# Arlo0o/StereoScene

Hardware: AMD Instinct MI355X
Metric: voxels/sec fwd+bwd, 256x256x32 grid D=192 (higher is better)
Workload: dtype f32; 1 GPU; kitti_d192: stereo pair features 2x[B,640,48,160] -> 256x256x32 occupancy, D=192, fwd+bwd incl. 4 losses; batch_per_gpu=1, global_batch=1, parallelism=dp1, train_mode=True

## Files before the change

include/ssbev.h:

```cpp
#ifndef SSBEV_H
#define SSBEV_H

#include <stddef.h>
#include <stdint.h>

#ifdef __cplusplus
extern "C" {
#endif

#define SSBEV_OK 0
#define SSBEV_EINVAL (-1)
#define SSBEV_EWORKSPACE (-2)
#define SSBEV_ELAUNCH (-3)

typedef void* ssbev_stream_t;

int ssbev_version(void);
const char* ssbev_build_arch(void);
void ssbev_env_refresh(void);

typedef struct {
  int B;
  int P;
  int C;
// ... 132 lines not shown
                         const ssbev_norm2_dims* d, void* ws, size_t ws_bytes, ssbev_stream_t stream);

typedef struct { float* running_mean_a; float* running_var_a; float momentum_a;
                 float* running_mean_b; float* running_var_b; float momentum_b; } ssbev_norm2_ext;
int ssbev_groupnorm2_fwd_ext(const float* xa, const float* gamma_a, const float* beta_a, float* mean_a, float* rstd_a,
                             const float* xb, const float* gamma_b, const float* beta_b, float* mean_b, float* rstd_b, float* y,
                             uint64_t* relu_mask, const ssbev_norm2_dims* d, const ssbev_norm2_ext* ext, void* ws, size_t ws_bytes,
                             ssbev_stream_t stream);
int ssbev_groupnorm2_bwd_ext(const float* gy, const uint64_t* relu_mask, const float* xa, const float* gamma_a, const float* mean_a,
                             const float* rstd_a, const float* xb, const float* gamma_b, const float* mean_b, const float* rstd_b,
                             float* gxa, float* gxb, float* ggamma_a, float* gbeta_a, float* ggamma_b, float* gbeta_b,
                             const ssbev_norm2_dims* d, const ssbev_norm2_ext* ext, void* ws, size_t ws_bytes,
                             ssbev_stream_t stream);

typedef struct {
  int vw;
  int slab_q;
  int slabs;
  int chunks;
  int64_t chunk_len;
  int64_t blocks;
  int fixed;
  int chunks_b;
  int64_t chunk_len_b;
  int chunks2;
  int64_t chunk_len2;
} ssbev_groupnorm_plan;
int ssbev_groupnorm_plan_query(const ssbev_norm_dims* d, const ssbev_norm2_dims* d2, int aligned16, ssbev_groupnorm_plan* out);

typedef struct { int B, D, H, W, C; } ssbev_upsample_dims;
int ssbev_trilinear2x_fwd(const float* x, float* y, const ssbev_upsample_dims* d, ssbev_stream_t stream);
int ssbev_trilinear2x_bwd(const float* gy, float* gx, const ssbev_upsample_dims* d, ssbev_stream_t stream);

typedef struct { float lr, beta1, beta2, eps, weight_decay, max_grad_norm; int step; } ssbev_adamw_cfg;
size_t ssbev_grad_norm_workspace(void);
int ssbev_grad_norm(const float* g, int64_t n, float* norm_out, void* ws, size_t ws_bytes,
                    ssbev_stream_t stream);
int ssbev_adamw_step(float* p, const float* g, float* m, float* v, int64_t n,
                     const ssbev_adamw_cfg* c, const float* grad_norm, ssbev_stream_t stream);

typedef struct { int B, D, H, W, C; } ssbev_occloss_dims;
int ssbev_occ_loss_num_sums(void);
size_t ssbev_occ_loss_workspace(const ssbev_occloss_dims* d);
int ssbev_occ_loss_fwd(const float* logits, const uint8_t* label, const float* class_weight, double* sums,
                       const ssbev_occloss_dims* d, void* ws, size_t ws_bytes, ssbev_stream_t stream);
int ssbev_bri_shell_chunks(void);
int ssbev_bri_shell_pre_fwd(const float* q, const float* kv, const float* conf, const float* wq, const float* bq,
                            const float* wk, const float* bk, const float* wv, const float* bv, float* Q, float* K, float* Vc,
                            int B, int D, int T, ssbev_stream_t stream);
int ssbev_bri_shell_post_fwd(const float* out, const float* kv, const float* gamma, float* y, int B, int D, int T,
                             ssbev_stream_t stream);
int ssbev_bri_shell_post_bwd(const float* gy, const float* out, const float* gamma, float* gout, float* delta_part, double* part,
                             int B, int D, int T, ssbev_stream_t stream);
int ssbev_bri_shell_pre_bwd(const float* gQ, const float* gK, const float* gVc, const float* q, const float* kv, const float* conf,
                            const float* gres, const float* wq, const float* wk, const float* wv, const float* bv, float* gq,
                            float* gkv, float* gconf_part, double* part, int B, int D, int T, ssbev_stream_t stream);

int ssbev_occ_loss_tail(const double* sums, float w_ce, float w_sem, float w_geo, float* out5, double* jac,
                        ssbev_stream_t stream);
size_t ssbev_occ_loss_bwd_workspace(const ssbev_occloss_dims* d);
int ssbev_occ_loss_bwd(const float* logits, const uint8_t* label, const float* class_weight,
                       const float* coef, float* grad_logits, const ssbev_occloss_dims* d, void* ws,
                       size_t ws_bytes, ssbev_stream_t stream);

size_t ssbev_occ_predict_workspace(const ssbev_upsample_dims* d);
int ssbev_occ_predict(const float* logits, const uint8_t* label, const uint16_t* remap, uint8_t* pred, uint16_t* raw,
                      int64_t* conf, int64_t* n_ignored, const ssbev_upsample_dims* d, void* ws, size_t ws_bytes,
                      ssbev_stream_t stream);

typedef struct { int B, D, H, W, C, ignore, upsample; } ssbev_lovasz_dims;
int ssbev_lovasz_num_counts(void);
size_t ssbev_lovasz_workspace(const ssbev_lovasz_dims* d);
int ssbev_lovasz_fwd(const float* logits, const uint8_t* label, float* loss, float* dj, int32_t* counts,
                     const ssbev_lovasz_dims* d, void* ws, size_t ws_bytes, ssbev_stream_t stream);
size_t ssbev_lovasz_bwd_workspace(const ssbev_lovasz_dims* d);
int ssbev_lovasz_bwd(const float* logits, const uint8_t* label, const float* dj, const int32_t* counts,
                     const float* grad_out, float* grad_logits, const ssbev_lovasz_dims* d, void* ws, size_t ws_bytes,
                     ssbev_stream_t stream);

typedef struct { int B, D, H, W, C, ignore, upsample; double top_k; } ssbev_ohem_dims;
size_t ssbev_ohem_ce_workspace(const ssbev_ohem_dims* d);
int ssbev_ohem_ce_fwd(const float* logits, const uint8_t* label, const float* class_weight, float* loss, uint8_t* mask,
                      float* inv_wsum, const ssbev_ohem_dims* d, void* ws, size_t ws_bytes, ssbev_stream_t stream);
size_t ssbev_ohem_ce_bwd_workspace(const ssbev_ohem_dims* d);
int ssbev_ohem_ce_bwd(const float* logits, const uint8_t* label, const float* class_weight, const uint8_t* mask,
                      const float* inv_wsum, const float* grad_out, float* grad_logits, const ssbev_ohem_dims* d, void* ws,
                      size_t ws_bytes, ssbev_stream_t stream);

int ssbev_bn_update_running(const float* mean, const float* rstd, float* running_mean, float* running_var, int C,
                            float momentum, float eps, int64_t n, ssbev_stream_t stream);

int ssbev_softmax_axis_fwd(const float* x, float* y, int64_t outer, int C, int64_t inner, ssbev_stream_t stream);
int ssbev_softmax_axis_bwd(const float* y, const float* gy, float* gx, int64_t outer, int C, int64_t inner,
                           ssbev_stream_t stream);
int ssbev_softmax_rows_fwd(const float* x, float* y, int64_t rows, int C, ssbev_stream_t stream);
int ssbev_softmax_rows_bwd(const float* y, const float* gy, float* gx, int64_t rows, int C, ssbev_stream_t stream);

typedef struct { int B, C, H, W, G, k, pad, dil; } ssbev_dcn_dims;
int ssbev_dcn_im2col(const float* x, const float* offset, float* cols, const ssbev_dcn_dims* d, ssbev_stream_t stream);
size_t ssbev_dcn_col2im_workspace(const ssbev_dcn_dims* d);
int ssbev_dcn_col2im(const float* x, const float* offset, const float* gcols, float* gx, float* goffset,
                     const ssbev_dcn_dims* d, void* ws, size_t ws_bytes, ssbev_stream_t stream);

int ssbev_resize_pil_u8(const uint8_t* src, int Hs, int Ws, int C, const int32_t* kk_h, const int32_t* bounds_h, int ksize_h,
                        const int32_t* kk_v, const int32_t* bounds_v, int ksize_v, uint8_t* tmp, uint8_t* dst, int Hd, int Wd,
                        ssbev_stream_t stream);
int ssbev_crop_normalize_u8(const uint8_t* src, int Hs, int Ws, float* dst, int x0, int y0, int w, int h, int flip,
                            const float* mean, const float* stdinv, int swap_rb, ssbev_stream_t stream);
int ssbev_crop_rotate_normalize_u8(const uint8_t* src, int Hs, int Ws, float* dst, int x0, int y0, int w, int h, int flip,
                                   const int32_t* affine6, const float* mean, const float* stdinv, int swap_rb,
                                   ssbev_stream_t stream);
#define SSBEV_JITTER_BRIGHTNESS 1
#define SSBEV_JITTER_CONTRAST 2
#define SSBEV_JITTER_SATURATION 4
#define SSBEV_JITTER_HUE 8
#define SSBEV_JITTER_SWAP 16
typedef struct { int flags, mode; float delta, alpha, saturation, hue; int perm[3]; } ssbev_jitter_params;
int ssbev_crop_rotate_jitter_normalize_u8(const uint8_t* src, int Hs, int Ws, float* dst, int x0, int y0, int w, int h, int flip,
                                          const int32_t* affine6, const ssbev_jitter_params* jitter, const float* mean,
                                          const float* stdinv, int swap_rb, ssbev_stream_t stream);
size_t ssbev_depth_bce_workspace(int BN, int fH, int fW);
int ssbev_depth_bce_fwd(const float* gt_depths, const float* depth_pred, float* out2, int BN, int D, int fH, int fW, int ds,
                        float c0, float dd, float weight, void* ws, size_t ws_bytes, ssbev_stream_t stream);
int ssbev_depth_bce_bwd(const float* depth_pred, const float* grad_loss, const float* out2, float* grad_pred, int BN, int D, int fH,
                        int fW, int ds, float c0, float dd, float weight, const void* ws, ssbev_stream_t stream);

size_t ssbev_depth_kld_workspace(int BN, int fH, int fW);
int ssbev_depth_kld_fwd(const float* gt_depths, const float* depth_pred, float* out2, int BN, int D, int fH, int fW, int ds,
                        double d0, double d1, double dd, float sigma, float edge_scale, float weight, void* ws, size_t ws_bytes,
                        ssbev_stream_t stream);
int ssbev_depth_kld_bwd(const float* depth_pred, const float* grad_loss, const float* out2, float* grad_pred, int BN, int D, int fH,
                        int fW, int ds, double d0, double d1, double dd, float sigma, float edge_scale, float weight, const void* ws,
                        size_t ws_bytes, ssbev_stream_t stream);

size_t ssbev_lidar_depth_workspace(int H, int W);
int ssbev_lidar_depth_map(const float* points, int n_points, const float* cam, const float* labels, float* uvd,
                          unsigned char* valid, float* depth, float* seg, int H, int W, void* ws, size_t ws_bytes,
                          ssbev_stream_t stream);

typedef struct { int B, C, Hi, Wi, Ho, Wo, k, stride, pad_t, pad_l; } ssbev_dw_dims;
int ssbev_dwconv2d_fwd(const float* x, const float* w, float* y, const ssbev_dw_dims* d, ssbev_stream_t stream);
int ssbev_dwconv2d_bwd_data(const float* gy, const float* w, float* gx, const ssbev_dw_dims* d, ssbev_stream_t stream);
size_t ssbev_dwconv2d_bwd_weight_workspace(const ssbev_dw_dims* d);
int ssbev_dwconv2d_bwd_weight(const float* x, const float* gy, float* gw, const ssbev_dw_dims* d, float* ws,
                              size_t ws_elems, ssbev_stream_t stream);
int ssbev_swish_fwd(const float* x, float* y, int64_t n, ssbev_stream_t stream);
int ssbev_swish_bwd(const float* x, const float* gy, float* gx, int64_t n, ssbev_stream_t stream);
size_t ssbev_chan_sum_workspace(int B, int64_t S, int C);
int ssbev_chan_sum(const float* a, const float* bmul, float* out, int B, int64_t S, int C, float scale, float* ws,
                   size_t ws_elems, ssbev_stream_t stream);
int ssbev_chan_scale(const float* x, const float* gate, float* y, int B, int64_t S, int C, float scale,
                     ssbev_stream_t stream);

typedef struct { int B, D, H, W, C; } ssbev_wino_dims;
int ssbev_wino_input_transform(const float* x, float* V, const ssbev_wino_dims* d, ssbev_stream_t stream);
int ssbev_wino_output_transform(const float* M, float* y, const ssbev_wino_dims* d, ssbev_stream_t stream);
int ssbev_wino_output_adjoint(const float* gy, float* Z, const ssbev_wino_dims* d, ssbev_stream_t stream);
int ssbev_wino2d_input_transform(const float* x, float* V, const ssbev_wino_dims* d, ssbev_stream_t stream);
int ssbev_wino2d_output_transform(const float* M, float* y, const ssbev_wino_dims* d, ssbev_stream_t stream);
int ssbev_wino2d_output_adjoint(const float* gy, float* Z, const ssbev_wino_dims* d, ssbev_stream_t stream);
int ssbev_wino_input_transform_bf16(const float* x, uint16_t* V, const ssbev_wino_dims* d, ssbev_stream_t stream);
int ssbev_wino_output_transform_bf16(const uint16_t* M, float* y, const ssbev_wino_dims* d, ssbev_stream_t stream);
int ssbev_wino_output_adjoint_bf16(const float* gy, uint16_t* Z, const ssbev_wino_dims* d, ssbev_stream_t stream);
int ssbev_wino2d_input_transform_bf16(const float* x, uint16_t* V, const ssbev_wino_dims* d, ssbev_stream_t stream);
int ssbev_wino2d_output_transform_bf16(const uint16_t* M, float* y, const ssbev_wino_dims* d, ssbev_stream_t stream);
int ssbev_wino2d_output_adjoint_bf16(const float* gy, uint16_t* Z, const ssbev_wino_dims* d, ssbev_stream_t stream);
int ssbev_wino_input_transform_bf16a(const uint16_t* x, uint16_t* V, const ssbev_wino_dims* d, ssbev_stream_t stream);
int ssbev_wino_output_transform_bf16a(const uint16_t* M, uint16_t* y, const ssbev_wino_dims* d, ssbev_stream_t stream);
int ssbev_wino_output_adjoint_bf16a(const uint16_t* gy, uint16_t* Z, const ssbev_wino_dims* d, ssbev_stream_t stream);
int ssbev_wino2d_input_transform_bf16a(const uint16_t* x, uint16_t* V, const ssbev_wino_dims* d, ssbev_stream_t stream);
int ssbev_wino2d_output_transform_bf16a(const uint16_t* M, uint16_t* y, const ssbev_wino_dims* d, ssbev_stream_t stream);
int ssbev_wino2d_output_adjoint_bf16a(const uint16_t* gy, uint16_t* Z, const ssbev_wino_dims* d, ssbev_stream_t stream);
int ssbev_wino43_input_transform(const float* x, float* V, const ssbev_wino_dims* d, ssbev_stream_t stream);
int ssbev_wino43_output_transform(const float* M, float* y, const ssbev_wino_dims* d, ssbev_stream_t stream);
int ssbev_wino43_output_adjoint(const float* gy, float* Z, const ssbev_wino_dims* d, ssbev_stream_t stream);
int ssbev_wino43_2d_input_transform(const float* x, float* V, const ssbev_wino_dims* d, ssbev_stream_t stream);
int ssbev_wino43_2d_output_transform(const float* M, float* y, const ssbev_wino_dims* d, ssbev_stream_t stream);
int ssbev_wino43_2d_output_transform_acc(const float* M, float* y, const ssbev_wino_dims* d, ssbev_stream_t stream);
int ssbev_wino2d_output_transform_acc(const float* M, float* y, const ssbev_wino_dims* d, ssbev_stream_t stream);
int ssbev_wino43_2d_output_adjoint(const float* gy, float* Z, const ssbev_wino_dims* d, ssbev_stream_t stream);
int ssbev_wino43_input_transform_bf16(const float* x, uint16_t* V, const ssbev_wino_dims* d, ssbev_stream_t stream);
int ssbev_wino43_output_transform_bf16(const uint16_t* M, float* y, const ssbev_wino_dims* d, ssbev_stream_t stream);
int ssbev_wino43_output_adjoint_bf16(const float* gy, uint16_t* Z, const ssbev_wino_dims* d, ssbev_stream_t stream);
int ssbev_wino43_2d_input_transform_bf16(const float* x, uint16_t* V, const ssbev_wino_dims* d, ssbev_stream_t stream);
int ssbev_wino43_2d_output_transform_bf16(const uint16_t* M, float* y, const ssbev_wino_dims* d, ssbev_stream_t stream);
int ssbev_wino43_2d_output_adjoint_bf16(const float* gy, uint16_t* Z, const ssbev_wino_dims* d, ssbev_stream_t stream);
int ssbev_wino444_input_transform(const float* x, float* V, const ssbev_wino_dims* d, ssbev_stream_t stream);
int ssbev_wino444_output_transform(const float* M, float* y, const ssbev_wino_dims* d, ssbev_stream_t stream);
int ssbev_wino444_output_adjoint(const float* gy, float* Z, const ssbev_wino_dims* d, ssbev_stream_t stream);
int ssbev_wino43_weight_transform(const float* w, float* U, int Cout, int Cin, int ndim, int mode, ssbev_stream_t stream);
int ssbev_wino43_weight_grad(const float* gU, float* gw, int Cout, int Cin, int ndim, ssbev_stream_t stream);
int ssbev_wino_weight_transform(const float* w, float* U, int Cout, int Cin, int ndim, int mode, ssbev_stream_t stream);
int ssbev_wino_weight_grad(const float* gU, float* gw, int Cout, int Cin, int ndim, ssbev_stream_t stream);
size_t ssbev_wino_dgemm_packed_elems(int Cout, int Cin);
int ssbev_wino_dgemm_pack(const float* w, float* Wp, int Cout, int Cin, int mode, ssbev_stream_t stream);
int ssbev_wino_dgemm(const float* P, const float* Wp, float* Mo, const ssbev_wino_dims* d, int N, ssbev_stream_t stream);
int ssbev_wino_bgemm(const float* A, const float* Wp, float* Cm, int64_t T, int K, int N, ssbev_stream_t stream);

typedef struct {
  int M, N, K, batch;
  int64_t lda, ldb, ldc, sa, sb, sc;
  int relu;
  int d2s_D, d2s_H, d2s_W, d2s_kd, d2s_kh, d2s_kw, d2s_Co;
  const int64_t* d2s_rowoff;
  const float* ep_mul;
  const float* ep_rowsub;
} ssbev_gemm_dims;
int ssbev_gemm_d2s_rowoff(int64_t* rowoff, int M, int D, int H, int W, int kd, int kh, int kw, int Co, ssbev_stream_t stream);
size_t ssbev_gemm_nn_workspace(const ssbev_gemm_dims* d);
size_t ssbev_gemm_nt_workspace(const ssbev_gemm_dims* d);
int ssbev_gemm_nn(const float* A, const float* B, const float* bias, float* C, const ssbev_gemm_dims* d, void* workspace,
                  size_t ws_bytes, ssbev_stream_t stream);
int ssbev_gemm_nt(const float* A, const float* W, const float* bias, float* C, const ssbev_gemm_dims* d, void* workspace,
                  size_t ws_bytes, ssbev_stream_t stream);
size_t ssbev_gemm_tn_workspace(const ssbev_gemm_dims* d);
int ssbev_gemm_tn(const float* A, const float* B, float* C, const ssbev_gemm_dims* d, void* workspace, size_t ws_bytes,
                  ssbev_stream_t stream);
typedef struct {
  int kernel;
  int bm, bn, bk;
  int nchunk;
  int per_chunk;
  int64_t grid;
  size_t workspace;
} ssbev_gemm_plan;
int ssbev_gemm_plan_query(const ssbev_gemm_dims* d, int form, ssbev_gemm_plan* out);

int ssbev_wino43_df_supported(const ssbev_wino_dims* d, int N);
int ssbev_wino43_df_instance(const ssbev_wino_dims* d, int N);
size_t ssbev_wino43_df_packed_elems(int Cout, int Cin);
int ssbev_wino43_df_pack(const float* w, float* Wp, int Cout, int Cin, int mode, ssbev_stream_t stream);
int ssbev_wino43_df_gemm(const float* P, const float* Wp, float* Mo, const ssbev_wino_dims* d, int N, ssbev_stream_t stream);
size_t ssbev_wino43_df_wgrad_workspace(const ssbev_wino_dims* d, int N);
int ssbev_wino43_df_wgrad(const float* P, const float* Z, float* gw, const ssbev_wino_dims* d, int N, void* workspace,
                          size_t ws_bytes, ssbev_stream_t stream);
typedef struct {
  int mt, nw;
  int ncolgrp, nrowgrp;
  int nst;
  int64_t grid;
  size_t lds_bytes;
  int w_kw, w_nt, w_br;
  int w_nkb, w_nnb;
  int w_nchunk;
  int w_stages_per_chunk;
  int w_total_stages;
  int64_t w_grid;
  size_t w_lds_bytes;
  size_t w_workspace;
} ssbev_wino43_df_plan;
int ssbev_wino43_df_plan_query(const ssbev_wino_dims* d, int N, ssbev_wino43_df_plan* out);

#ifdef __cplusplus
}
#endif
#endif
```

stereoscene_amd/capi.py:

```python
import ctypes as C
import os

import torch

_HERE = os.path.dirname(os.path.abspath(__file__))
LIB_PATH = os.path.join(_HERE, "_lib", "libssbev_hip.so")

OK, EINVAL, EWORKSPACE, ELAUNCH = 0, -1, -2, -3
_ERR = {EINVAL: "SSBEV_EINVAL (bad dims / null pointer / unsupported configuration)",
        EWORKSPACE: "SSBEV_EWORKSPACE (workspace too small)",
        ELAUNCH: "SSBEV_ELAUNCH (HIP launch failure)"}


class SsbevError(RuntimeError):
    pass


class PoolDims(C.Structure):
    _fields_ = [("B", C.c_int), ("P", C.c_int), ("C", C.c_int), ("nx", C.c_int), ("ny", C.c_int), ("nz", C.c_int),
                ("origin", C.c_float * 3), ("dx", C.c_float * 3)]


class LiftDims(C.Structure):
    _fields_ = [("N", C.c_int), ("D", C.c_int), ("HW", C.c_int)]


class GwcDims(C.Structure):
    _fields_ = [("B", C.c_int), ("C", C.c_int), ("G", C.c_int), ("D", C.c_int), ("H", C.c_int), ("W", C.c_int),
                ("down", C.c_float), ("align_corners", C.c_int)]


class ConvDims(C.Structure):
    _fields_ = [(n, C.c_int) for n in (
        "B", "Cin", "Cout", "Di", "Hi", "Wi", "Do", "Ho", "Wo", "kd", "kh", "kw", "sd", "sh", "sw",
        "pd", "ph", "pw", "dd", "dh", "dw", "transposed", "relu", "accumulate", "tile_hint", "precision")]


class GeomDims(C.Structure):
    _fields_ = [(n, C.c_int) for n in ("B", "N", "D", "H", "W")]


class NormDims(C.Structure):
    _fields_ = [("B", C.c_int), ("C", C.c_int), ("G", C.c_int), ("S", C.c_int64), ("eps", C.c_float),
                ("relu", C.c_int), ("stats_given", C.c_int), ("pre_act", C.c_int), ("ld_y", C.c_int64), ("ld_gy", C.c_int64),
                ("io_dtype", C.c_int)]


class Norm2Dims(C.Structure):
    _fields_ = [("B", C.c_int), ("C", C.c_int), ("Ga", C.c_int), ("Gb", C.c_int), ("S", C.c_int64), ("eps_a", C.c_float),
                ("eps_b", C.c_float), ("relu", C.c_int), ("a_batch", C.c_int), ("b_batch", C.c_int), ("io_dtype", C.c_int)]


class Gemm16Dims(C.Structure):
    _fields_ = [("M", C.c_int), ("N", C.c_int), ("K", C.c_int), ("batch", C.c_int), ("out_fp32", C.c_int)]


class NormExt(C.Structure):
    _fields_ = [("running_mean", C.c_void_p), ("running_var", C.c_void_p), ("momentum", C.c_float),
                ("n", C.c_int64)]


class Norm2Ext(C.Structure):
    _fields_ = [("running_mean_a", C.c_void_p), ("running_var_a", C.c_void_p), ("momentum_a", C.c_float),
                ("running_mean_b", C.c_void_p), ("running_var_b", C.c_void_p), ("momentum_b", C.c_float)]


class DcnDims(C.Structure):
    _fields_ = [(n, C.c_int) for n in ("B", "C", "H", "W", "G", "k", "pad", "dil")]


class DwDims(C.Structure):
    _fields_ = [(n, C.c_int) for n in ("B", "C", "Hi", "Wi", "Ho", "Wo", "k", "stride", "pad_t", "pad_l")]


class WinoDims(C.Structure):
    _fields_ = [(n, C.c_int) for n in ("B", "D", "H", "W", "C")]


class UpsampleDims(C.Structure):
    _fields_ = [("B", C.c_int), ("D", C.c_int), ("H", C.c_int), ("W", C.c_int), ("C", C.c_int)]


class LovaszDims(C.Structure):
    _fields_ = [(n, C.c_int) for n in ("B", "D", "H", "W", "C", "ignore", "upsample")]


class OhemDims(C.Structure):
    _fields_ = LovaszDims._fields_ + [("top_k", C.c_double)]


class GemmDims(C.Structure):
    _fields_ = [("M", C.c_int), ("N", C.c_int), ("K", C.c_int), ("batch", C.c_int),
                ("lda", C.c_int64), ("ldb", C.c_int64), ("ldc", C.c_int64), ("sa", C.c_int64), ("sb", C.c_int64), ("sc", C.c_int64),
                ("relu", C.c_int),
                ("d2s_D", C.c_int), ("d2s_H", C.c_int), ("d2s_W", C.c_int), ("d2s_kd", C.c_int), ("d2s_kh", C.c_int),
                ("d2s_kw", C.c_int), ("d2s_Co", C.c_int), ("d2s_rowoff", C.c_void_p),
                ("ep_mul", C.c_void_p), ("ep_rowsub", C.c_void_p)]


class GroupnormPlan(C.Structure):
    _fields_ = [("vw", C.c_int), ("slab_q", C.c_int), ("slabs", C.c_int), ("chunks", C.c_int), ("chunk_len", C.c_int64),
                ("blocks", C.c_int64), ("fixed", C.c_int), ("chunks_b", C.c_int), ("chunk_len_b", C.c_int64), ("chunks2", C.c_int),
                ("chunk_len2", C.c_int64)]


class GemmPlan(C.Structure):
    _fields_ = [("kernel", C.c_int), ("bm", C.c_int), ("bn", C.c_int), ("bk", C.c_int), ("nchunk", C.c_int), ("per_chunk", C.c_int),
                ("grid", C.c_int64), ("workspace", C.c_size_t)]


class Wino43DfPlan(C.Structure):
    _fields_ = [("mt", C.c_int), ("nw", C.c_int), ("ncolgrp", C.c_int), ("nrowgrp", C.c_int), ("nst", C.c_int), ("grid", C.c_int64),
                ("lds_bytes", C.c_size_t), ("w_kw", C.c_int), ("w_nt", C.c_int), ("w_br", C.c_int), ("w_nkb", C.c_int),
                ("w_nnb", C.c_int), ("w_nchunk", C.c_int), ("w_stages_per_chunk", C.c_int), ("w_total_stages", C.c_int),
                ("w_grid", C.c_int64), ("w_lds_bytes", C.c_size_t), ("w_workspace", C.c_size_t)]


class JitterParams(C.Structure):
    _fields_ = [("flags", C.c_int), ("mode", C.c_int), ("delta", C.c_float), ("alpha", C.c_float), ("saturation", C.c_float),
                ("hue", C.c_float), ("perm", C.c_int * 3)]


JITTER_BRIGHTNESS, JITTER_CONTRAST, JITTER_SATURATION, JITTER_HUE, JITTER_SWAP = 1, 2, 4, 8, 16


class AdamWCfg(C.Structure):
    _fields_ = [("lr", C.c_float), ("beta1", C.c_float), ("beta2", C.c_float), ("eps", C.c_float),
                ("weight_decay", C.c_float), ("max_grad_norm", C.c_float), ("step", C.c_int)]


_P = C.c_void_p
SIGNATURES = {
    "ssbev_version": (C.c_int, []),
    "ssbev_build_arch": (C.c_char_p, []),
    "ssbev_env_refresh": (None, []),
    "ssbev_voxel_index": (C.c_int, [_P, _P, _P, C.POINTER(PoolDims), _P]),
    "ssbev_coords_to_vox": (C.c_int, [_P, C.c_int, _P, C.POINTER(PoolDims), _P]),
    "ssbev_pool_prepare_workspace": (C.c_size_t, [C.c_int, C.POINTER(PoolDims)]),
    "ssbev_pool_prepare": (C.c_int, [_P, C.c_int, _P, _P, C.POINTER(PoolDims), _P, C.c_size_t, _P]),
    "ssbev_pool_long_list_elems": (C.c_size_t, [C.c_int]),
    "ssbev_pool_prepare2": (C.c_int, [_P, C.c_int, _P, _P, _P, C.POINTER(PoolDims), _P, C.c_size_t, _P]),
    "ssbev_bev_pool_fwd": (C.c_int, [_P, _P, _P, _P, C.POINTER(PoolDims), _P]),
    "ssbev_bev_pool_bwd": (C.c_int, [_P, _P, C.c_int, _P, C.POINTER(PoolDims), _P]),
    "ssbev_lift_splat_fwd": (C.c_int, [_P, _P, _P, _P, _P, C.POINTER(PoolDims), C.POINTER(LiftDims), _P]),
    "ssbev_lift_splat_fwd2": (C.c_int, [_P, _P, _P, _P, _P, _P, C.POINTER(PoolDims), C.POINTER(LiftDims), _P]),
    "ssbev_lift_splat_bwd": (C.c_int, [_P, _P, _P, _P, _P, _P, C.POINTER(PoolDims), C.POINTER(LiftDims), _P]),
    "ssbev_gwc_warp_fwd": (C.c_int, [_P, _P, _P, _P, C.POINTER(GwcDims), _P]),
    "ssbev_gwc_warp_bwd": (C.c_int, [_P, _P, _P, _P, _P, _P, C.POINTER(GwcDims), _P]),
    "ssbev_gwc_warp_bwd_workspace": (C.c_size_t, [C.POINTER(GwcDims)]),
    "ssbev_gwc_warp_bwd_fused": (C.c_int, [_P, _P, _P, _P, _P, _P, C.POINTER(GwcDims), _P, C.c_size_t, _P]),
    "ssbev_conv_packed_weight_elems": (C.c_size_t, [C.POINTER(ConvDims)]),
    "ssbev_conv_kernel_class": (C.c_int, [C.POINTER(ConvDims), C.c_int]),
    "ssbev_conv_chunk_groups": (C.c_int, [C.POINTER(ConvDims), C.c_int]),
    "ssbev_frustum_geometry": (C.c_int, [_P] * 9 + [C.POINTER(GeomDims), _P]),
    "ssbev_conv_pack_weight": (C.c_int, [_P, _P, C.POINTER(ConvDims), C.c_int, _P]),
    "ssbev_conv_thin_workspace": (C.c_size_t, [C.POINTER(ConvDims), C.c_int]),
    "ssbev_conv_thin_packed_elems": (C.c_size_t, [C.POINTER(ConvDims), C.c_int]),
    "ssbev_conv_thin_pack": (C.c_int, [_P, _P, C.POINTER(ConvDims), C.c_int, _P]),
    "ssbev_conv_thin_run": (C.c_int, [_P, _P, _P, _P, C.POINTER(ConvDims), C.c_int, _P, C.c_size_t, _P]),
    "ssbev_conv_fwd": (C.c_int, [_P, _P, _P, _P, C.POINTER(ConvDims), _P]),
    "ssbev_conv_bwd_data": (C.c_int, [_P, _P, _P, C.POINTER(ConvDims), _P]),
    "ssbev_conv_fwd_bf16": (C.c_int, [_P, _P, _P, _P, C.POINTER(ConvDims), _P]),
    "ssbev_conv_bwd_data_bf16": (C.c_int, [_P, _P, _P, C.POINTER(ConvDims), _P]),
    "ssbev_conv_bwd_weight_bf16": (C.c_int, [_P, _P, _P, C.POINTER(ConvDims), _P, C.c_size_t, _P]),
    "ssbev_conv_bwd_weight_workspace": (C.c_size_t, [C.POINTER(ConvDims)]),
    "ssbev_conv_bwd_weight": (C.c_int, [_P, _P, _P, C.POINTER(ConvDims), _P, C.c_size_t, _P]),
    "ssbev_gemm16_packed_elems": (C.c_size_t, [C.POINTER(Gemm16Dims)]),
    "ssbev_gemm16_pack": (C.c_int, [_P, _P, C.POINTER(Gemm16Dims), _P]),
    "ssbev_gemm16_nn": (C.c_int, [_P, _P, _P, C.POINTER(Gemm16Dims), _P]),
    "ssbev_gemm16_tn_workspace": (C.c_size_t, [C.POINTER(Gemm16Dims)]),
    "ssbev_gemm16_tn": (C.c_int, [_P, _P, _P, C.POINTER(Gemm16Dims), _P, C.c_size_t, _P]),
    "ssbev_groupnorm_workspace": (C.c_size_t, [C.POINTER(NormDims)]),
    "ssbev_groupnorm_fwd": (C.c_int, [_P] * 7 + [C.POINTER(NormDims), _P, C.c_size_t, _P]),
    "ssbev_groupnorm_bwd": (C.c_int, [_P] * 10 + [C.POINTER(NormDims), _P, C.c_size_t, _P]),
    "ssbev_groupnorm_mask_words": (C.c_size_t, [C.POINTER(NormDims)]),
    "ssbev_groupnorm_fwd_mask": (C.c_int, [_P] * 8 + [C.POINTER(NormDims), _P, C.c_size_t, _P]),
    "ssbev_groupnorm_bwd_mask": (C.c_int, [_P] * 10 + [C.POINTER(NormDims), _P, C.c_size_t, _P]),
    "ssbev_groupnorm_fwd_ext": (C.c_int, [_P] * 8 + [C.POINTER(NormDims), C.POINTER(NormExt), _P, C.c_size_t, _P]),
    "ssbev_groupnorm_bwd_ext": (C.c_int, [_P] * 11 + [C.POINTER(NormDims), C.POINTER(NormExt), _P, C.c_size_t, _P]),
    "ssbev_groupnorm2_fwd_ext": (C.c_int, [_P] * 12 + [C.POINTER(Norm2Dims), C.POINTER(Norm2Ext), _P, C.c_size_t, _P]),
    "ssbev_groupnorm2_bwd_ext": (C.c_int, [_P] * 16 + [C.POINTER(Norm2Dims), C.POINTER(Norm2Ext), _P, C.c_size_t, _P]),
    "ssbev_groupnorm2_workspace": (C.c_size_t, [C.POINTER(Norm2Dims)]),
    "ssbev_groupnorm2_fwd": (C.c_int, [_P] * 12 + [C.POINTER(Norm2Dims), _P, C.c_size_t, _P]),
    "ssbev_groupnorm2_bwd": (C.c_int, [_P] * 16 + [C.POINTER(Norm2Dims), _P, C.c_size_t, _P]),
    "ssbev_groupnorm_plan_query": (C.c_int, [C.POINTER(NormDims), C.POINTER(Norm2Dims), C.c_int, C.POINTER(GroupnormPlan)]),
    "ssbev_trilinear2x_fwd": (C.c_int, [_P, _P, C.POINTER(UpsampleDims), _P]),
    "ssbev_trilinear2x_bwd": (C.c_int, [_P, _P, C.POINTER(UpsampleDims), _P]),
    "ssbev_dcn_im2col": (C.c_int, [_P, _P, _P, C.POINTER(DcnDims), _P]),
    "ssbev_dcn_col2im_workspace": (C.c_size_t, [C.POINTER(DcnDims)]),
    "ssbev_dcn_col2im": (C.c_int, [_P, _P, _P, _P, _P, C.POINTER(DcnDims), _P, C.c_size_t, _P]),
    "ssbev_bn_update_running": (C.c_int, [_P, _P, _P, _P, C.c_int, C.c_float, C.c_float, C.c_int64, _P]),
    "ssbev_resize_pil_u8": (C.c_int, [_P, C.c_int, C.c_int, C.c_int, _P, _P, C.c_int, _P, _P, C.c_int, _P, _P, C.c_int, C.c_int, _P]),
    "ssbev_crop_normalize_u8": (C.c_int, [_P, C.c_int, C.c_int, _P, C.c_int, C.c_int, C.c_int, C.c_int, C.c_int, _P, _P, C.c_int, _P]),
    "ssbev_crop_rotate_normalize_u8": (C.c_int, [_P, C.c_int, C.c_int, _P, C.c_int, C.c_int, C.c_int, C.c_int, C.c_int, _P, _P, _P,
                                                C.c_int, _P]),
    "ssbev_crop_rotate_jitter_normalize_u8": (C.c_int, [_P, C.c_int, C.c_int, _P, C.c_int, C.c_int, C.c_int, C.c_int, C.c_int, _P,
                                                       C.POINTER(JitterParams), _P, _P, C.c_int, _P]),
    "ssbev_depth_bce_workspace": (C.c_size_t, [C.c_int, C.c_int, C.c_int]),
    "ssbev_depth_bce_fwd": (C.c_int, [_P, _P, _P] + [C.c_int] * 5 + [C.c_float] * 3 + [_P, C.c_size_t, _P]),
    "ssbev_depth_bce_bwd": (C.c_int, [_P, _P, _P, _P] + [C.c_int] * 5 + [C.c_float] * 3 + [_P, _P]),
    "ssbev_depth_kld_workspace": (C.c_size_t, [C.c_int, C.c_int, C.c_int]),
    "ssbev_depth_kld_fwd": (C.c_int, [_P, _P, _P] + [C.c_int] * 5 + [C.c_double] * 3 + [C.c_float] * 3 + [_P, C.c_size_t, _P]),
    "ssbev_depth_kld_bwd": (C.c_int, [_P, _P, _P, _P] + [C.c_int] * 5 + [C.c_double] * 3 + [C.c_float] * 3 + [_P, C.c_size_t, _P]),
    "ssbev_lidar_depth_workspace": (C.c_size_t, [C.c_int, C.c_int]),
    "ssbev_lidar_depth_map": (C.c_int, [_P, C.c_int, _P, _P, _P, _P, _P, _P, C.c_int, C.c_int, _P, C.c_size_t, _P]),
    "ssbev_dwconv2d_fwd": (C.c_int, [_P, _P, _P, C.POINTER(DwDims), _P]),
    "ssbev_dwconv2d_bwd_data": (C.c_int, [_P, _P, _P, C.POINTER(DwDims), _P]),
    "ssbev_dwconv2d_bwd_weight_workspace": (C.c_size_t, [C.POINTER(DwDims)]),
    "ssbev_dwconv2d_bwd_weight": (C.c_int, [_P, _P, _P, C.POINTER(DwDims), _P, C.c_size_t, _P]),
    "ssbev_swish_fwd": (C.c_int, [_P, _P, C.c_int64, _P]),
    "ssbev_swish_bwd": (C.c_int, [_P, _P, _P, C.c_int64, _P]),
    "ssbev_chan_sum_workspace": (C.c_size_t, [C.c_int, C.c_int64, C.c_int]),
    "ssbev_chan_sum": (C.c_int, [_P, _P, _P, C.c_int, C.c_int64, C.c_int, C.c_float, _P, C.c_size_t, _P]),
    "ssbev_chan_scale": (C.c_int, [_P, _P, _P, C.c_int, C.c_int64, C.c_int, C.c_float, _P]),
    "ssbev_wino_input_transform": (C.c_int, [_P, _P, C.POINTER(WinoDims), _P]),
    "ssbev_wino_output_transform": (C.c_int, [_P, _P, C.POINTER(WinoDims), _P]),
    "ssbev_wino_output_adjoint": (C.c_int, [_P, _P, C.POINTER(WinoDims), _P]),
    "ssbev_wino_weight_transform": (C.c_int, [_P, _P, C.c_int, C.c_int, C.c_int, C.c_int, _P]),
    "ssbev_wino_weight_grad": (C.c_int, [_P, _P, C.c_int, C.c_int, C.c_int, _P]),
    "ssbev_wino_dgemm_packed_elems": (C.c_size_t, [C.c_int, C.c_int]),
    "ssbev_wino_dgemm_pack": (C.c_int, [_P, _P, C.c_int, C.c_int, C.c_int, _P]),
    "ssbev_wino_dgemm": (C.c_int, [_P, _P, _P, C.POINTER(WinoDims), C.c_int, _P]),
    "ssbev_wino_bgemm": (C.c_int, [_P, _P, _P, C.c_int64, C.c_int, C.c_int, _P]),
    "ssbev_gemm_d2s_rowoff": (C.c_int, [_P, C.c_int, C.c_int, C.c_int, C.c_int, C.c_int, C.c_int, C.c_int, C.c_int, _P]),
    "ssbev_gemm_nn_workspace": (C.c_size_t, [C.POINTER(GemmDims)]),
    "ssbev_gemm_nt_workspace": (C.c_size_t, [C.POINTER(GemmDims)]),
    "ssbev_gemm_nn": (C.c_int, [_P, _P, _P, _P, C.POINTER(GemmDims), _P, C.c_size_t, _P]),
    "ssbev_gemm_nt": (C.c_int, [_P, _P, _P, _P, C.POINTER(GemmDims), _P, C.c_size_t, _P]),
    "ssbev_gemm_tn_workspace": (C.c_size_t, [C.POINTER(GemmDims)]),
    "ssbev_gemm_tn": (C.c_int, [_P, _P, _P, C.POINTER(GemmDims), _P, C.c_size_t, _P]),
    "ssbev_gemm_plan_query": (C.c_int, [C.POINTER(GemmDims), C.c_int, C.POINTER(GemmPlan)]),
    "ssbev_wino43_df_supported": (C.c_int, [C.POINTER(WinoDims), C.c_int]),
    "ssbev_wino43_df_instance": (C.c_int, [C.POINTER(WinoDims), C.c_int]),
    "ssbev_wino43_df_packed_elems": (C.c_size_t, [C.c_int, C.c_int]),
    "ssbev_wino43_df_pack": (C.c_int, [_P, _P, C.c_int, C.c_int, C.c_int, _P]),
    "ssbev_wino43_df_gemm": (C.c_int, [_P, _P, _P, C.POINTER(WinoDims), C.c_int, _P]),
    "ssbev_wino43_df_wgrad_workspace": (C.c_size_t, [C.POINTER(WinoDims), C.c_int]),
    "ssbev_wino43_df_wgrad": (C.c_int, [_P, _P, _P, C.POINTER(WinoDims), C.c_int, _P, C.c_size_t, _P]),
    "ssbev_wino43_df_plan_query": (C.c_int, [C.POINTER(WinoDims), C.c_int, C.POINTER(Wino43DfPlan)]),
    "ssbev_wino2d_input_transform": (C.c_int, [_P, _P, C.POINTER(WinoDims), _P]),
    "ssbev_wino2d_output_transform": (C.c_int, [_P, _P, C.POINTER(WinoDims), _P]),
    "ssbev_wino2d_output_adjoint": (C.c_int, [_P, _P, C.POINTER(WinoDims), _P]),
    "ssbev_wino43_input_transform": (C.c_int, [_P, _P, C.POINTER(WinoDims), _P]),
    "ssbev_wino43_input_transform_bf16": (C.c_int, [_P, _P, C.POINTER(WinoDims), _P]),
    "ssbev_wino43_output_transform": (C.c_int, [_P, _P, C.POINTER(WinoDims), _P]),
    "ssbev_wino43_output_transform_bf16": (C.c_int, [_P, _P, C.POINTER(WinoDims), _P]),
    "ssbev_wino43_output_adjoint": (C.c_int, [_P, _P, C.POINTER(WinoDims), _P]),
    "ssbev_wino43_output_adjoint_bf16": (C.c_int, [_P, _P, C.POINTER(WinoDims), _P]),
    "ssbev_wino43_2d_input_transform": (C.c_int, [_P, _P, C.POINTER(WinoDims), _P]),
    "ssbev_wino43_2d_input_transform_bf16": (C.c_int, [_P, _P, C.POINTER(WinoDims), _P]),
    "ssbev_wino43_2d_output_transform": (C.c_int, [_P, _P, C.POINTER(WinoDims), _P]),
    "ssbev_wino43_2d_output_transform_acc": (C.c_int, [_P, _P, C.POINTER(WinoDims), _P]),
    "ssbev_wino2d_output_transform_acc": (C.c_int, [_P, _P, C.POINTER(WinoDims), _P]),
    "ssbev_wino43_2d_output_transform_bf16": (C.c_int, [_P, _P, C.POINTER(WinoDims), _P]),
    "ssbev_wino43_2d_output_adjoint": (C.c_int, [_P, _P, C.POINTER(WinoDims), _P]),
    "ssbev_wino43_2d_output_adjoint_bf16": (C.c_int, [_P, _P, C.POINTER(WinoDims), _P]),
    "ssbev_wino444_input_transform": (C.c_int, [_P, _P, C.POINTER(WinoDims), _P]),
    "ssbev_wino444_output_transform": (C.c_int, [_P, _P, C.POINTER(WinoDims), _P]),
    "ssbev_wino444_output_adjoint": (C.c_int, [_P, _P, C.POINTER(WinoDims), _P]),
    "ssbev_wino43_weight_transform": (C.c_int, [_P, _P, C.c_int, C.c_int, C.c_int, C.c_int, _P]),
    "ssbev_wino43_weight_grad": (C.c_int, [_P, _P, C.c_int, C.c_int, C.c_int, _P]),
    "ssbev_wino_input_transform_bf16": (C.c_int, [_P, _P, C.POINTER(WinoDims), _P]),
    "ssbev_wino_output_transform_bf16": (C.c_int, [_P, _P, C.POINTER(WinoDims), _P]),
    "ssbev_wino_output_adjoint_bf16": (C.c_int, [_P, _P, C.POINTER(WinoDims), _P]),
    "ssbev_wino2d_input_transform_bf16": (C.c_int, [_P, _P, C.POINTER(WinoDims), _P]),
    "ssbev_wino2d_output_transform_bf16": (C.c_int, [_P, _P, C.POINTER(WinoDims), _P]),
    "ssbev_wino2d_output_adjoint_bf16": (C.c_int, [_P, _P, C.POINTER(WinoDims), _P]),
    "ssbev_wino_input_transform_bf16a": (C.c_int, [_P, _P, C.POINTER(WinoDims), _P]),
    "ssbev_wino_output_transform_bf16a": (C.c_int, [_P, _P, C.POINTER(WinoDims), _P]),
    "ssbev_wino_output_adjoint_bf16a": (C.c_int, [_P, _P, C.POINTER(WinoDims), _P]),
    "ssbev_wino2d_input_transform_bf16a": (C.c_int, [_P, _P, C.POINTER(WinoDims), _P]),
    "ssbev_wino2d_output_transform_bf16a": (C.c_int, [_P, _P, C.POINTER(WinoDims), _P]),
    "ssbev_wino2d_output_adjoint_bf16a": (C.c_int, [_P, _P, C.POINTER(WinoDims), _P]),
    "ssbev_softmax_axis_fwd": (C.c_int, [_P, _P, C.c_int64, C.c_int, C.c_int64, _P]),
    "ssbev_softmax_axis_bwd": (C.c_int, [_P, _P, _P, C.c_int64, C.c_int, C.c_int64, _P]),
    "ssbev_softmax_rows_fwd": (C.c_int, [_P, _P, C.c_int64, C.c_int, _P]),
    "ssbev_softmax_rows_bwd": (C.c_int, [_P, _P, _P, C.c_int64, C.c_int, _P]),
    "ssbev_occ_loss_num_sums": (C.c_int, []),
    "ssbev_occ_loss_workspace": (C.c_size_t, [C.POINTER(UpsampleDims)]),
    "ssbev_occ_loss_fwd": (C.c_int, [_P, _P, _P, _P, C.POINTER(UpsampleDims), _P, C.c_size_t, _P]),
    "ssbev_occ_loss_tail": (C.c_int, [_P, C.c_float, C.c_float, C.c_float, _P, _P, _P]),
    "ssbev_bri_shell_chunks": (C.c_int, []),
    "ssbev_bri_shell_pre_fwd": (C.c_int, [_P] * 12 + [C.c_int] * 3 + [_P]),
    "ssbev_bri_shell_post_fwd": (C.c_int, [_P] * 4 + [C.c_int] * 3 + [_P]),
    "ssbev_bri_shell_post_bwd": (C.c_int, [_P] * 6 + [C.c_int] * 3 + [_P]),
    "ssbev_bri_shell_pre_bwd": (C.c_int, [_P] * 15 + [C.c_int] * 3 + [_P]),
    "ssbev_occ_loss_bwd_workspace": (C.c_size_t, [C.POINTER(UpsampleDims)]),
    "ssbev_occ_loss_bwd": (C.c_int, [_P, _P, _P, _P, _P, C.POINTER(UpsampleDims), _P, C.c_size_t, _P]),
    "ssbev_occ_predict_workspace": (C.c_size_t, [C.POINTER(UpsampleDims)]),
    "ssbev_occ_predict": (C.c_int, [_P] * 7 + [C.POINTER(UpsampleDims), _P, C.c_size_t, _P]),
    "ssbev_lovasz_num_counts": (C.c_int, []),
    "ssbev_lovasz_workspace": (C.c_size_t, [C.POINTER(LovaszDims)]),
    "ssbev_lovasz_fwd": (C.c_int, [_P] * 5 + [C.POINTER(LovaszDims), _P, C.c_size_t, _P]),
    "ssbev_lovasz_bwd_workspace": (C.c_size_t, [C.POINTER(LovaszDims)]),
    "ssbev_lovasz_bwd": (C.c_int, [_P] * 6 + [C.POINTER(LovaszDims), _P, C.c_size_t, _P]),
    "ssbev_ohem_ce_workspace": (C.c_size_t, [C.POINTER(OhemDims)]),
    "ssbev_ohem_ce_fwd": (C.c_int, [_P] * 6 + [C.POINTER(OhemDims), _P, C.c_size_t, _P]),
    "ssbev_ohem_ce_bwd_workspace": (C.c_size_t, [C.POINTER(OhemDims)]),
    "ssbev_ohem_ce_bwd": (C.c_int, [_P] * 7 + [C.POINTER(OhemDims), _P, C.c_size_t, _P]),
    "ssbev_grad_norm_workspace": (C.c_size_t, []),
    "ssbev_grad_norm": (C.c_int, [_P, C.c_int64, _P, _P, C.c_size_t, _P]),
    "ssbev_adamw_step": (C.c_int, [_P, _P, _P, _P, C.c_int64, C.POINTER(AdamWCfg), _P, _P]),
}

_lib = None


def load():
    global _lib
    if _lib is None:
        if not os.path.exists(LIB_PATH):
            raise SsbevError(f"{LIB_PATH} is missing: run `python -m stereoscene_amd.build` "
                             "(there is no CPU / PyTorch fallback for the HIP operators)")
        lib = C.CDLL(LIB_PATH)
        for name, (res, args) in SIGNATURES.items():
            fn = getattr(lib, name)
            fn.restype, fn.argtypes = res, args
        _lib = lib
    return _lib


def check(code, what):
    if code != OK:
        raise SsbevError(f"{what}: {_ERR.get(code, code)}")


def ptr(t):
    if t is None:
        return None
    if not t.is_cuda:
        raise SsbevError("ssbev operators run on the MI355X only: got a CPU tensor (no CPU fallback exists)")
    if not t.is_contiguous():
        raise SsbevError("ssbev operators need contiguous buffers")
    return C.c_void_p(t.data_ptr())


_raw_stream = getattr(torch._C, "_cuda_getCurrentRawStream", None)


def stream():
    if _raw_stream is not None:
        return C.c_void_p(_raw_stream(torch.cuda.current_device()))
    return C.c_void_p(torch.cuda.current_stream().cuda_stream)
```

stereoscene_amd/csrc/capi.hip:

```cpp
#include "common.h"

#include <cstdlib>
#include <mutex>
#include <string>
#include <unordered_map>

namespace {
struct EnvTable {
  std::mutex mu;
  std::unordered_map<std::string, std::pair<bool, std::string>> seen;
};
EnvTable& env_table() {
  static EnvTable* t = new EnvTable();
  return *t;
}
}

const char* ssbev_env(const char* name) {
  EnvTable& t = env_table();
  std::lock_guard<std::mutex> lock(t.mu);
  auto it = t.seen.find(name);
  if (it == t.seen.end()) {
    const char* v = std::getenv(name);
    it = t.seen.emplace(name, std::make_pair(v != nullptr, std::string(v ? v : ""))).first;
  }
  return it->second.first ? it->second.second.c_str() : nullptr;
}

extern "C" {
int ssbev_version(void) { return 110;  }
const char* ssbev_build_arch(void) { return "gfx950"; }

void ssbev_env_refresh(void) {
  EnvTable& t = env_table();
  std::lock_guard<std::mutex> lock(t.mu);
  t.seen.clear();
}
}
```

stereoscene_amd/csrc/winograd.hip:

```cpp
#include "common.h"

#include <algorithm>
#include <cstdlib>

namespace {

struct WinoGeom { int B, D, H, W, C; int acc = 0; };
__device__ const float kWinoZeros[4] = {0.f, 0.f, 0.f, 0.f};

typedef unsigned short bf16_bits;
__device__ __forceinline__ float fload(const float* p) { return *p; }
__device__ __forceinline__ float fload(const bf16_bits* p) { return __uint_as_float((unsigned)*p << 16); }
__device__ __forceinline__ void fstore(float* p, float v) { *p = v; }
__device__ __forceinline__ void fstore(bf16_bits* p, float v) { *p = __builtin_bit_cast(bf16_bits, (__bf16)v); }

__device__ __forceinline__ void bt4(float* v, int s) {
  const float d0 = v[0], d1 = v[s], d2 = v[2 * s], d3 = v[3 * s];
  v[0] = d0 - d2; v[s] = d1 + d2; v[2 * s] = d2 - d1; v[3 * s] = d1 - d3;
}
__device__ __forceinline__ void a4(float* v, int s) {
  const float g0 = v[0], g1 = v[s];
  v[0] = g0; v[s] = g0 + g1; v[2 * s] = g0 - g1; v[3 * s] = -g1;
}

template <int NV, typename T>
__device__ __forceinline__ void ldv(const T* p, float (&o)[NV]) {
  if constexpr (NV == 1) {
    o[0] = ld1(p);
  } else if constexpr (sizeof(T) == 2) {
    const unsigned u = *reinterpret_cast<const unsigned*>(p);
    o[0] = __uint_as_float(u << 16); o[1] = __uint_as_float(u & 0xffff0000u);
  } else {
    const float2 f = *reinterpret_cast<const float2*>(p);
    o[0] = f.x; o[1] = f.y;
  }
}
template <int NV, typename T>
__device__ __forceinline__ void stv(T* p, const float (&v)[NV]) {
  if constexpr (NV == 1) {
    st1(p, v[0]);
  } else if constexpr (sizeof(T) == 2) {
    *reinterpret_cast<unsigned*>(p) = pack_bf2(v[0], v[1]);
  } else {
    *reinterpret_cast<float2*>(p) = make_float2(v[0], v[1]);
  }
}

template <int NV>
__device__ __forceinline__ void wino_decode3(long i, const WinoGeom& g, int& c, long& tile, int& tw, int& th, int& td, int& b) {
  const int cq = g.C / NV;
  c = NV * (int)(i % cq);
  long t = i / cq;
  tile = t;
  tw = (int)(t % (g.W / 2)); t /= g.W / 2;
  th = (int)(t % (g.H / 2)); t /= g.H / 2;
  td = (int)(t % (g.D / 2));
  b = (int)(t / (g.D / 2));
}
template <int NV>
__device__ __forceinline__ void wino_decode2(long i, const WinoGeom& g, int& c, long& tile, int& tw, int& th, long& bd) {
  const int cq = g.C / NV;
  c = NV * (int)(i % cq);
  long t = i / cq;
  tile = t;
  tw = (int)(t % (g.W / 2)); t /= g.W / 2;
  th = (int)(t % (g.H / 2));
  bd = t / (g.H / 2);
}

template <typename TF, typename TA = float, int NV = 1>
__global__ void __launch_bounds__(256)
wino_input_kernel(const TA* __restrict__ x, TF* __restrict__ V, WinoGeom g, long total) {
  const long i = (long)blockIdx.x * 256 + threadIdx.x;
  if (i >= total) return;
  int c, tw, th, td, b;
  long tile;
  wino_decode3<NV>(i, g, c, tile, tw, th, td, b);
  float v[NV][64];
#pragma unroll
  for (int a = 0; a < 4; ++a) {
    const int d = 2 * td - 1 + a;
#pragma unroll
    for (int e = 0; e < 4; ++e) {
      const int h = 2 * th - 1 + e;
#pragma unroll
      for (int f = 0; f < 4; ++f) {
        const int w = 2 * tw - 1 + f;
        const bool ok = d >= 0 && d < g.D && h >= 0 && h < g.H && w >= 0 && w < g.W;
        float t[NV];
#pragma unroll
        for (int n = 0; n < NV; ++n) t[n] = 0.0f;
        if (ok) ldv<NV>(x + ((((long)b * g.D + d) * g.H + h) * g.W + w) * g.C + c, t);
#pragma unroll
        for (int n = 0; n < NV; ++n) v[n][(a * 4 + e) * 4 + f] = t[n];
      }
    }
  }
#pragma unroll
  for (int n = 0; n < NV; ++n) {
#pragma unroll
    for (int p = 0; p < 16; ++p) bt4(v[n] + p * 4, 1);
#pragma unroll
    for (int a = 0; a < 4; ++a)
#pragma unroll
      for (int f = 0; f < 4; ++f) bt4(v[n] + a * 16 + f, 4);
#pragma unroll
    for (int p = 0; p < 16; ++p) bt4(v[n] + p, 16);
  }
  const long T = total / (g.C / NV);
#pragma unroll
  for (int xi = 0; xi < 64; ++xi) {
    float t[NV];
#pragma unroll
    for (int n = 0; n < NV; ++n) t[n] = v[n][xi];
    stv<NV>(V + ((long)xi * T + tile) * g.C + c, t);
  }
}

template <typename TF, typename TA = float, int NV = 1>
__global__ void __launch_bounds__(256)
wino_output_kernel(const TF* __restrict__ M, TA* __restrict__ y, WinoGeom g, long total) {
  const long i = (long)blockIdx.x * 256 + threadIdx.x;
  if (i >= total) return;
  int c, tw, th, td, b;
  long tile;
  wino_decode3<NV>(i, g, c, tile, tw, th, td, b);
  const long T = total / (g.C / NV);
  float m[NV][64];
#pragma unroll
  for (int xi = 0; xi < 64; ++xi) {
    float t[NV];
    ldv<NV>(M + ((long)xi * T + tile) * g.C + c, t);
#pragma unroll
    for (int n = 0; n < NV; ++n) m[n][xi] = t[n];
  }
  float out[NV][8];
#pragma unroll
  for (int n = 0; n < NV; ++n) {
    float r1[32];
#pragma unroll
    for (int p = 0; p < 16; ++p) {
      r1[p * 2 + 0] = m[n][p * 4] + m[n][p * 4 + 1] + m[n][p * 4 + 2];
      r1[p * 2 + 1] = m[n][p * 4 + 1] - m[n][p * 4 + 2] - m[n][p * 4 + 3];
    }
    float r2[16];
#pragma unroll
    for (int a = 0; a < 4; ++a)
#pragma unroll
      for (int f = 0; f < 2; ++f) {
        const float m0 = r1[(a * 4 + 0) * 2 + f], m1 = r1[(a * 4 + 1) * 2 + f], m2 = r1[(a * 4 + 2) * 2 + f],
                    m3 = r1[(a * 4 + 3) * 2 + f];
        r2[(a * 2 + 0) * 2 + f] = m0 + m1 + m2;
        r2[(a * 2 + 1) * 2 + f] = m1 - m2 - m3;
      }
#pragma unroll
    for (int e = 0; e < 2; ++e)
#pragma unroll
      for (int f = 0; f < 2; ++f) {
        const float m0 = r2[(0 * 2 + e) * 2 + f], m1 = r2[(1 * 2 + e) * 2 + f], m2 = r2[(2 * 2 + e) * 2 + f],
                    m3 = r2[(3 * 2 + e) * 2 + f];
        out[n][(0 * 2 + e) * 2 + f] = m0 + m1 + m2;
        out[n][(1 * 2 + e) * 2 + f] = m1 - m2 - m3;
      }
  }
#pragma unroll
  for (int dz = 0; dz < 2; ++dz)
#pragma unroll
    for (int e = 0; e < 2; ++e)
#pragma unroll
      for (int f = 0; f < 2; ++f) {
        float t[NV];
#pragma unroll
        for (int n = 0; n < NV; ++n) t[n] = out[n][(dz * 2 + e) * 2 + f];
        stv<NV>(y + ((((long)b * g.D + 2 * td + dz) * g.H + 2 * th + e) * g.W + 2 * tw + f) * g.C + c, t);
      }
}

template <typename TF, typename TA = float, int NV = 1>
__global__ void __launch_bounds__(256)
wino_output_adjoint_kernel(const TA* __restrict__ gy, TF* __restrict__ Z, WinoGeom g, long total) {
  const long i = (long)blockIdx.x * 256 + threadIdx.x;
  if (i >= total) return;
  int c, tw, th, td, b;
  long tile;
  wino_decode3<NV>(i, g, c, tile, tw, th, td, b);
  float v[NV][64];
#pragma unroll
  for (int a = 0; a < 2; ++a)
#pragma unroll
    for (int e = 0; e < 2; ++e)
#pragma unroll
      for (int f = 0; f < 2; ++f) {
        float t[NV];
        ldv<NV>(gy + ((((long)b * g.D + 2 * td + a) * g.H + 2 * th + e) * g.W + 2 * tw + f) * g.C + c, t);
#pragma unroll
        for (int n = 0; n < NV; ++n) v[n][(a * 4 + e) * 4 + f] = t[n];
      }
#pragma unroll
  for (int n = 0; n < NV; ++n) {
#pragma unroll
    for (int a = 0; a < 2; ++a)
#pragma unroll
      for (int e = 0; e < 2; ++e) a4(v[n] + (a * 4 + e) * 4, 1);
#pragma unroll
    for (int a = 0; a < 2; ++a)
#pragma unroll
      for (int f = 0; f < 4; ++f) a4(v[n] + a * 16 + f, 4);
#pragma unroll
    for (int p = 0; p < 16; ++p) a4(v[n] + p, 16);
  }
  const long T = total / (g.C / NV);
#pragma unroll
  for (int xi = 0; xi < 64; ++xi) {
    float t[NV];
#pragma unroll
    for (int n = 0; n < NV; ++n) t[n] = v[n][xi];
    stv<NV>(Z + ((long)xi * T + tile) * g.C + c, t);
  }
}

template <typename TF, typename TA = float, int NV = 1>
__global__ void __launch_bounds__(256)
wino2d_input_kernel(const TA* __restrict__ x, TF* __restrict__ V, WinoGeom g, long total) {
  const long i = (long)blockIdx.x * 256 + threadIdx.x;
  if (i >= total) return;
  int c, tw, th;
  long tile, bd;
  wino_decode2<NV>(i, g, c, tile, tw, th, bd);
  float v[NV][16];
#pragma unroll
  for (int e = 0; e < 4; ++e) {
    const int h = 2 * th - 1 + e;
#pragma unroll
    for (int f = 0; f < 4; ++f) {
      const int w = 2 * tw - 1 + f;
      const bool ok = h >= 0 && h < g.H && w >= 0 && w < g.W;
      float t[NV];
#pragma unroll
      for (int n = 0; n < NV; ++n) t[n] = 0.0f;
      if (ok) ldv<NV>(x + ((bd * g.H + h) * g.W + w) * g.C + c, t);
#pragma unroll
      for (int n = 0; n < NV; ++n) v[n][e * 4 + f] = t[n];
    }
  }
#pragma unroll
  for (int n = 0; n < NV; ++n) {
#pragma unroll
    for (int e = 0; e < 4; ++e) bt4(v[n] + e * 4, 1);
#pragma unroll
    for (int f = 0; f < 4; ++f) bt4(v[n] + f, 4);
  }
  const long T = total / (g.C / NV);
#pragma unroll
  for (int xi = 0; xi < 16; ++xi) {
    float t[NV];
#pragma unroll
    for (int n = 0; n < NV; ++n) t[n] = v[n][xi];
    stv<NV>(V + ((long)xi * T + tile) * g.C + c, t);
  }
}

template <typename TF, typename TA = float, int NV = 1>
__global__ void __launch_bounds__(256)
wino2d_output_kernel(const TF* __restrict__ M, TA* __restrict__ y, WinoGeom g, long total) {
  const long i = (long)blockIdx.x * 256 + threadIdx.x;
  if (i >= total) return;
  int c, tw, th;
  long tile, bd;
  wino_decode2<NV>(i, g, c, tile, tw, th, bd);
  const long T = total / (g.C / NV);
  float m[NV][16];
#pragma unroll
  for (int xi = 0; xi < 16; ++xi) {
    float t[NV];
    ldv<NV>(M + ((long)xi * T + tile) * g.C + c, t);
#pragma unroll
    for (int n = 0; n < NV; ++n) m[n][xi] = t[n];
  }
  float oldv[NV][4];
#pragma unroll
  for (int n = 0; n < NV; ++n)
#pragma unroll
    for (int k = 0; k < 4; ++k) oldv[n][k] = 0.0f;
  if (g.acc) {
#pragma unroll
    for (int f = 0; f < 2; ++f) {
      const long base = ((bd * g.H + 2 * th) * g.W + 2 * tw + f) * g.C + c;
      float t0[NV], t1[NV];
      ldv<NV>(y + base, t0);
      ldv<NV>(y + base + (long)g.W * g.C, t1);
#pragma unroll
      for (int n = 0; n < NV; ++n) { oldv[n][2 * f] = t0[n]; oldv[n][2 * f + 1] = t1[n]; }
    }
  }
#pragma unroll
  for (int f = 0; f < 2; ++f) {
    float y0[NV], y1[NV];
#pragma unroll
    for (int n = 0; n < NV; ++n) {
      float r[8];
#pragma unroll
      for (int e = 0; e < 4; ++e) {
        r[e * 2 + 0] = m[n][e * 4] + m[n][e * 4 + 1] + m[n][e * 4 + 2];
        r[e * 2 + 1] = m[n][e * 4 + 1] - m[n][e * 4 + 2] - m[n][e * 4 + 3];
      }
      y0[n] = r[0 * 2 + f] + r[1 * 2 + f] + r[2 * 2 + f] + oldv[n][2 * f];
      y1[n] = r[1 * 2 + f] - r[2 * 2 + f] - r[3 * 2 + f] + oldv[n][2 * f + 1];
    }
    const long base = ((bd * g.H + 2 * th) * g.W + 2 * tw + f) * g.C + c;
    stv<NV>(y + base, y0);
    stv<NV>(y + base + (long)g.W * g.C, y1);
  }
}

template <typename TF, typename TA = float, int NV = 1>
__global__ void __launch_bounds__(256)
wino2d_output_adjoint_kernel(const TA* __restrict__ gy, TF* __restrict__ Z, WinoGeom g, long total) {
  const long i = (long)blockIdx.x * 256 + threadIdx.x;
  if (i >= total) return;
  int c, tw, th;
  long tile, bd;
  wino_decode2<NV>(i, g, c, tile, tw, th, bd);
  float v[NV][16];
#pragma unroll
  for (int e = 0; e < 2; ++e)
#pragma unroll
    for (int f = 0; f < 2; ++f) {
      float t[NV];
      ldv<NV>(gy + ((bd * g.H + 2 * th + e) * g.W + 2 * tw + f) * g.C + c, t);
#pragma unroll
      for (int n = 0; n < NV; ++n) v[n][e * 4 + f] = t[n];
    }
#pragma unroll
  for (int n = 0; n < NV; ++n) {
#pragma unroll
    for (int e = 0; e < 2; ++e) a4(v[n] + e * 4, 1);
#pragma unroll
    for (int f = 0; f < 4; ++f) a4(v[n] + f, 4);
  }
  const long T = total / (g.C / NV);
#pragma unroll
  for (int xi = 0; xi < 16; ++xi) {
    float t[NV];
#pragma unroll
    for (int n = 0; n < NV; ++n) t[n] = v[n][xi];
    stv<NV>(Z + ((long)xi * T + tile) * g.C + c, t);
  }
}

bool wino2d_ok(const ssbev_wino_dims* d) {
  return d && d->B > 0 && d->C > 0 && d->D > 0 && d->H > 0 && d->W > 0 && d->H % 2 == 0 && d->W % 2 == 0;
}

__device__ __forceinline__ void g4(const float* g, int s, float* o, int so) {
  const float g0 = g[0], g1 = g[s], g2 = g[2 * s];
  o[0] = g0; o[so] = 0.5f * (g0 + g1 + g2); o[2 * so] = 0.5f * (g0 - g1 + g2); o[3 * so] = g2;
}
__device__ __forceinline__ void gt3(const float* u, int s, float* o, int so) {
  const float u0 = u[0], u1 = u[s], u2 = u[2 * s], u3 = u[3 * s];
  o[0] = u0 + 0.5f * (u1 + u2); o[so] = 0.5f * (u1 - u2); o[2 * so] = 0.5f * (u1 + u2) + u3;
}

template <int ND>
__global__ void __launch_bounds__(256)
wino_weight_kernel(const float* __restrict__ w, float* __restrict__ U, int Cout, int Cin, int mode) {
  constexpr int TAPS = ND == 3 ? 27 : 9, NF = ND == 3 ? 64 : 16;
  const int i = blockIdx.x * 256 + threadIdx.x;
  if (i >= Cout * Cin) return;
  const int co = mode == 0 ? i % Cout : i / Cin, ci = mode == 0 ? i / Cout : i % Cin;
  float g[TAPS];
#pragma unroll
  for (int t = 0; t < TAPS; ++t) g[t] = w[((size_t)co * Cin + ci) * TAPS + (mode == 0 ? t : TAPS - 1 - t)];
  float u[NF];
  if (ND == 3) {
    float a[36], b[48];
#pragma unroll
    for (int p = 0; p < 9; ++p) g4(g + p * 3, 1, a + p * 4, 1);
#pragma unroll
    for (int d = 0; d < 3; ++d)
#pragma unroll
      for (int f = 0; f < 4; ++f) g4(a + d * 12 + f, 4, b + d * 16 + f, 4);
#pragma unroll
    for (int p = 0; p < 16; ++p) g4(b + p, 16, u + p, 16);
  } else {
    float a[12];
#pragma unroll
    for (int p = 0; p < 3; ++p) g4(g + p * 3, 1, a + p * 4, 1);
#pragma unroll
    for (int f = 0; f < 4; ++f) g4(a + f, 4, u + f, 4);
  }
  const size_t plane = (size_t)Cout * Cin;
  const size_t pos = mode == 0 ? (size_t)ci * Cout + co : (size_t)co * Cin + ci;
#pragma unroll
  for (int xi = 0; xi < NF; ++xi) U[xi * plane + pos] = u[xi];
}

template <int ND>
__global__ void __launch_bounds__(256)
wino_weight_grad_kernel(const float* __restrict__ gU, float* __restrict__ gw, int Cout, int Cin) {
  constexpr int TAPS = ND == 3 ? 27 : 9, NF = ND == 3 ? 64 : 16;
  const int i = blockIdx.x * 256 + threadIdx.x;
  if (i >= Cout * Cin) return;
  const int co = i % Cout, ci = i / Cout;
  const size_t plane = (size_t)Cout * Cin;
  float u[NF];
#pragma unroll
  for (int xi = 0; xi < NF; ++xi) u[xi] = gU[xi * plane + (size_t)ci * Cout + co];
  float g[TAPS];
  if (ND == 3) {
    float a[48], b[36];
#pragma unroll
    for (int p = 0; p < 16; ++p) gt3(u + p * 4, 1, a + p * 3, 1);
#pragma unroll
    for (int d = 0; d < 4; ++d)
#pragma unroll
      for (int f = 0; f < 3; ++f) gt3(a + d * 12 + f, 3, b + d * 9 + f, 3);
#pragma unroll
    for (int p = 0; p < 9; ++p) gt3(b + p, 9, g + p, 9);
  } else {
    float a[12];
#pragma unroll
    for (int p = 0; p < 4; ++p) gt3(u + p * 4, 1, a + p * 3, 1);
#pragma unroll
    for (int f = 0; f < 3; ++f) gt3(a + f, 3, g + f, 3);
  }
#pragma unroll
  for (int t = 0; t < TAPS; ++t) gw[((size_t)co * Cin + ci) * TAPS + t] = g[t];
}

__device__ __forceinline__ void bt6(float* v, int s) {
  const float d0 = v[0], d1 = v[s], d2 = v[2 * s], d3 = v[3 * s], d4 = v[4 * s], d5 = v[5 * s];
  v[0] = 4.0f * d0 - 5.0f * d2 + d4;
  v[s] = -4.0f * d1 - 4.0f * d2 + d3 + d4;
  v[2 * s] = 4.0f * d1 - 4.0f * d2 - d3 + d4;
  v[3 * s] = -2.0f * d1 - d2 + 2.0f * d3 + d4;
  v[4 * s] = 2.0f * d1 - d2 - 2.0f * d3 + d4;
  v[5 * s] = 4.0f * d1 - 5.0f * d3 + d5;
}
__device__ __forceinline__ void at6(const float* m, int s, float* o, int so) {
  const float m0 = m[0], m1 = m[s], m2 = m[2 * s], m3 = m[3 * s], m4 = m[4 * s], m5 = m[5 * s];
  const float p = m1 + m2, q = m1 - m2, r = m3 + m4, t = m3 - m4;
  o[0] = m0 + p + r;
  o[so] = q + 2.0f * t;
  o[2 * so] = p + 4.0f * r;
  o[3 * so] = q + 8.0f * t + m5;
}
__device__ __forceinline__ void a6(const float* g, int s, float* o, int so) {
  const float g0 = g[0], g1 = g[s], g2 = g[2 * s], g3 = g[3 * s];
  o[0] = g0;
  o[so] = g0 + g1 + g2 + g3;
  o[2 * so] = g0 - g1 + g2 - g3;
  o[3 * so] = g0 + 2.0f * g1 + 4.0f * g2 + 8.0f * g3;
  o[4 * so] = g0 - 2.0f * g1 + 4.0f * g2 - 8.0f * g3;
  o[5 * so] = g3;
}
__device__ __forceinline__ void g6(const float* g, int s, float* o, int so) {
  const float g0 = g[0], g1 = g[s], g2 = g[2 * s];
  o[0] = 0.25f * g0;
  o[so] = -(g0 + g1 + g2) * (1.0f / 6.0f);
  o[2 * so] = -(g0 - g1 + g2) * (1.0f / 6.0f);
  o[3 * so] = g0 * (1.0f / 24.0f) + g1 * (1.0f / 12.0f) + g2 * (1.0f / 6.0f);
  o[4 * so] = g0 * (1.0f / 24.0f) - g1 * (1.0f / 12.0f) + g2 * (1.0f / 6.0f);
  o[5 * so] = g2;
}
__device__ __forceinline__ void gt6(const float* u, int s, float* o, int so) {
  const float u0 = u[0], u1 = u[s], u2 = u[2 * s], u3 = u[3 * s], u4 = u[4 * s], u5 = u[5 * s];
  o[0] = 0.25f * u0 - (u1 + u2) * (1.0f / 6.0f) + (u3 + u4) * (1.0f / 24.0f);
  o[so] = (u2 - u1) * (1.0f / 6.0f) + (u3 - u4) * (1.0f / 12.0f);
  o[2 * so] = -(u1 + u2) * (1.0f / 6.0f) + (u3 + u4) * (1.0f / 6.0f) + u5;
}

template <int DA>
__device__ __forceinline__ void tile43(long t, const WinoGeom& g, int& b_or_bd, int& td, int& th, int& tw) {
  tw = (int)(t % (g.W / 4)); t /= g.W / 4;
  th = (int)(t % (g.H / 4)); t /= g.H / 4;
  if (DA) { td = (int)(t % (g.D / DA)); b_or_bd = (int)(t / (g.D / DA)); }
  else { td = 0; b_or_bd = (int)t; }
}

template <int DA, typename TF>
__global__ void __launch_bounds__(256) __attribute__((amdgpu_waves_per_eu(1, DA == 4 ? 1 : (DA == 2 ? 2 : 8))))
wino43_input_kernel(const float* __restrict__ x, TF* __restrict__ V, WinoGeom g, long total) {
  constexpr int NA = DA ? DA + 2 : 1, NF = NA * 36;
  const long i = (long)blockIdx.x * 256 + threadIdx.x;
  if (i >= total) return;
  const int c = (int)(i % g.C);
  const long tile = i / g.C;
  int b, td, th, tw;
  tile43<DA>(tile, g, b, td, th, tw);
  float v[NF];
#pragma unroll
  for (int a = 0; a < NA; ++a) {
    const int d = DA ? DA * td - 1 + a : 0;
    const long plane = DA ? (long)b * g.D + d : (long)b;
    const bool dok = !DA || (d >= 0 && d < g.D);
#pragma unroll
    for (int e = 0; e < 6; ++e) {
      const int h = 4 * th - 1 + e;
#pragma unroll
      for (int f = 0; f < 6; ++f) {
        const int w = 4 * tw - 1 + f;
        const bool ok = dok && h >= 0 && h < g.H && w >= 0 && w < g.W;
        v[(a * 6 + e) * 6 + f] = ok ? x[((plane * g.H + h) * g.W + w) * g.C + c] : 0.0f;
      }
// ... 34 lines not shown
  float r1[NA * 6 * 4];
#pragma unroll
  for (int p = 0; p < NA * 6; ++p) at6(m + p * 6, 1, r1 + p * 4, 1);
  float r2[NA * 4 * 4];
#pragma unroll
  for (int a = 0; a < NA; ++a)
#pragma unroll
    for (int f = 0; f < 4; ++f) at6(r1 + a * 24 + f, 4, r2 + a * 16 + f, 4);
  if (DA == 0 && g.acc) {
    float oldv[16];
#pragma unroll
    for (int e = 0; e < 4; ++e)
#pragma unroll
      for (int f = 0; f < 4; ++f) oldv[e * 4 + f] = y[(((long)b * g.H + 4 * th + e) * g.W + 4 * tw + f) * g.C + c];
#pragma unroll
    for (int k = 0; k < 16; ++k) r2[k] += oldv[k];
  }
#pragma unroll
  for (int e = 0; e < 4; ++e)
#pragma unroll
    for (int f = 0; f < 4; ++f) {
      if (DA == 2) {
        const float m0 = r2[0 * 16 + e * 4 + f], m1 = r2[1 * 16 + e * 4 + f], m2 = r2[2 * 16 + e * 4 + f], m3 = r2[3 * 16 + e * 4 + f];
        const long base = ((((long)b * g.D + 2 * td) * g.H + 4 * th + e) * g.W + 4 * tw + f) * g.C + c;
        y[base] = m0 + m1 + m2;
        y[base + (long)g.H * g.W * g.C] = m1 - m2 - m3;
      } else if (DA == 4) {
        float o[4];
        at6(r2 + e * 4 + f, 16, o, 1);
        const long base = ((((long)b * g.D + 4 * td) * g.H + 4 * th + e) * g.W + 4 * tw + f) * g.C + c;
#pragma unroll
        for (int a = 0; a < 4; ++a) y[base + (long)a * g.H * g.W * g.C] = o[a];
      } else {
        y[(((long)b * g.H + 4 * th + e) * g.W + 4 * tw + f) * g.C + c] = r2[e * 4 + f];
      }
    }
}

template <int DA, typename TF>
__global__ void __launch_bounds__(256) __attribute__((amdgpu_waves_per_eu(1, DA == 4 ? 1 : (DA == 2 ? 2 : 8))))
wino43_output_adjoint_kernel(const float* __restrict__ gy, TF* __restrict__ Z, WinoGeom g, long total) {
  constexpr int NA = DA ? DA + 2 : 1, NG = DA ? DA : 1, NF = NA * 36;
  const long i = (long)blockIdx.x * 256 + threadIdx.x;
  if (i >= total) return;
  const int c = (int)(i % g.C);
  const long tile = i / g.C;
  int b, td, th, tw;
  tile43<DA>(tile, g, b, td, th, tw);
  float gin[NG * 16];
#pragma unroll
  for (int a = 0; a < NG; ++a) {
    const long plane = DA ? (long)b * g.D + DA * td + a : (long)b;
#pragma unroll
    for (int e = 0; e < 4; ++e)
#pragma unroll
      for (int f = 0; f < 4; ++f) gin[(a * 4 + e) * 4 + f] = gy[((plane * g.H + 4 * th + e) * g.W + 4 * tw + f) * g.C + c];
  }
  float r1[NG * 4 * 6];
#pragma unroll
  for (int p = 0; p < NG * 4; ++p) a6(gin + p * 4, 1, r1 + p * 6, 1);
  float v[NF];
#pragma unroll
  for (int a = 0; a < NG; ++a)
#pragma unroll
    for (int f = 0; f < 6; ++f) a6(r1 + a * 24 + f, 6, v + a * 36 + f, 6);
  if (DA == 2) {
#pragma unroll
    for (int p = 0; p < 36; ++p) a4(v + p, 36);
  } else if (DA == 4) {
#pragma unroll
    for (int p = 0; p < 36; ++p) {
      float t6[6];
      a6(v + p, 36, t6, 1);
#pragma unroll
      for (int a = 0; a < 6; ++a) v[a * 36 + p] = t6[a];
    }
  }
  const long T = total / g.C;
#pragma unroll
  for (int xi = 0; xi < NF; ++xi) fstore(Z + ((long)xi * T + tile) * g.C + c, v[xi]);
}

template <int DA>
__global__ void __launch_bounds__(256)
wino43_weight_kernel(const float* __restrict__ w, float* __restrict__ U, int Cout, int Cin, int mode) {
  constexpr int ND_ = DA ? 3 : 1, TAPS = ND_ * 9, NA = DA ? DA + 2 : 1, NF = NA * 36;
  const int i = blockIdx.x * 256 + threadIdx.x;
  if (i >= Cout * Cin) return;
  const int co = mode == 0 ? i % Cout : i / Cin, ci = mode == 0 ? i / Cout : i % Cin;
  float g[TAPS];
#pragma unroll
  for (int t = 0; t < TAPS; ++t) g[t] = w[((size_t)co * Cin + ci) * TAPS + (mode == 0 ? t : TAPS - 1 - t)];
  float a1[ND_ * 3 * 6];
#pragma unroll
  for (int p = 0; p < ND_ * 3; ++p) g6(g + p * 3, 1, a1 + p * 6, 1);
  float a2[ND_ * 36];
#pragma unroll
  for (int d = 0; d < ND_; ++d)
#pragma unroll
    for (int f = 0; f < 6; ++f) g6(a1 + d * 18 + f, 6, a2 + d * 36 + f, 6);
  float u[NF];
  if (DA == 2) {
#pragma unroll
    for (int p = 0; p < 36; ++p) g4(a2 + p, 36, u + p, 36);
  } else if (DA == 4) {
#pragma unroll
    for (int p = 0; p < 36; ++p) g6(a2 + p, 36, u + p, 36);
  } else {
#pragma unroll
    for (int p = 0; p < 36; ++p) u[p] = a2[p];
  }
  const size_t plane = (size_t)Cout * Cin;
  const size_t pos = mode == 0 ? (size_t)ci * Cout + co : (size_t)co * Cin + ci;
#pragma unroll
  for (int xi = 0; xi < NF; ++xi) U[xi * plane + pos] = u[xi];
}

template <int DA>
__global__ void __launch_bounds__(256)
wino43_weight_grad_kernel(const float* __restrict__ gU, float* __restrict__ gw, int Cout, int Cin) {
  constexpr int ND_ = DA ? 3 : 1, TAPS = ND_ * 9, NA = DA ? DA + 2 : 1, NF = NA * 36;
  const int i = blockIdx.x * 256 + threadIdx.x;
  if (i >= Cout * Cin) return;
  const int co = i % Cout, ci = i / Cout;
  const size_t plane = (size_t)Cout * Cin;
  float u[NF];
#pragma unroll
  for (int xi = 0; xi < NF; ++xi) u[xi] = gU[xi * plane + (size_t)ci * Cout + co];
  float a1[NA * 6 * 3];
#pragma unroll
  for (int p = 0; p < NA * 6; ++p) gt6(u + p * 6, 1, a1 + p * 3, 1);
  float a2[NA * 9];
#pragma unroll
  for (int a = 0; a < NA; ++a)
#pragma unroll
    for (int f = 0; f < 3; ++f) gt6(a1 + a * 18 + f, 3, a2 + a * 9 + f, 3);
  float g[TAPS];
  if (DA == 2) {
#pragma unroll
    for (int p = 0; p < 9; ++p) gt3(a2 + p, 9, g + p, 9);
  } else if (DA == 4) {
#pragma unroll
    for (int p = 0; p < 9; ++p) gt6(a2 + p, 9, g + p, 9);
  } else {
#pragma unroll
    for (int p = 0; p < 9; ++p) g[p] = a2[p];
  }
#pragma unroll
  for (int t = 0; t < TAPS; ++t) gw[((size_t)co * Cin + ci) * TAPS + t] = g[t];
}

bool wino43_ok(const ssbev_wino_dims* d, int da) {
  return d && d->B > 0 && d->C > 0 && d->D > 0 && d->H > 0 && d->W > 0 && d->H % 4 == 0 && d->W % 4 == 0 &&
         (da == 0 || d->D % da == 0);
}

typedef float wf32x16 __attribute__((ext_vector_type(16)));

struct WinoGemmGeom { int B, D, Thw, Cin, Cout, CoutPad; };

template <int MT, int NT>
__global__ void __launch_bounds__(256)
wino_dgemm_kernel(const float* __restrict__ P, const float* __restrict__ Wp, float* __restrict__ Mo, WinoGemmGeom g) {
  const int lane = threadIdx.x & 63, wave = threadIdx.x >> 6;
  const int li = lane & 31, lk = lane >> 5;
  const int tgroups = (g.Thw + 32 * MT - 1) / (32 * MT), tg4 = ((tgroups + 3) >> 2) << 2;
  const int tg = (blockIdx.x * 4 + wave) % tg4;
  const int bi = (blockIdx.x * 4 + wave) / tg4;
  if (tg >= tgroups) return;
  const int i = bi % (g.D / 2), b = bi / (g.D / 2);
  const int xhw = blockIdx.z, n0 = blockIdx.y * (NT * 32);
  const long R = (long)g.B * g.D * g.Thw;
  const float* pa[4][MT];
#pragma unroll
  for (int mt = 0; mt < MT; ++mt) {
    const int tq = (tg * MT + mt) * 32 + li;
#pragma unroll
    for (int a = 0; a < 4; ++a) {
      const int d = 2 * i - 1 + a;
      pa[a][mt] = (tq < g.Thw && d >= 0 && d < g.D)
                      ? P + ((long)xhw * R + ((long)b * g.D + d) * g.Thw + tq) * g.Cin + 4 * lk : nullptr;
    }
  }
  wf32x16 acc[4][MT][NT];
#pragma unroll
  for (int f = 0; f < 4; ++f)
#pragma unroll
    for (int mt = 0; mt < MT; ++mt)
#pragma unroll
      for (int nt = 0; nt < NT; ++nt)
#pragma unroll
        for (int r = 0; r < 16; ++r) acc[f][mt][nt][r] = 0.0f;
  const int Q = (g.Cin + 7) >> 3;
  const size_t fstride = (size_t)Q * 2 * g.CoutPad * 4;
  const float* wl = Wp + ((size_t)lk * g.CoutPad + n0 + li) * 4 + (size_t)xhw * fstride;
  for (int q = 0; q < Q; ++q) {
    const bool cok = (8 * q + 4 * lk) < g.Cin;
    float4 v[4][MT];
#pragma unroll
    for (int mt = 0; mt < MT; ++mt) {
      float4 p[4];
#pragma unroll
      for (int a = 0; a < 4; ++a)
        p[a] = (pa[a][mt] && cok) ? *reinterpret_cast<const float4*>(pa[a][mt] + 8 * q) : make_float4(0.f, 0.f, 0.f, 0.f);
      v[0][mt] = make_float4(p[0].x - p[2].x, p[0].y - p[2].y, p[0].z - p[2].z, p[0].w - p[2].w);
      v[1][mt] = make_float4(p[1].x + p[2].x, p[1].y + p[2].y, p[1].z + p[2].z, p[1].w + p[2].w);
      v[2][mt] = make_float4(p[2].x - p[1].x, p[2].y - p[1].y, p[2].z - p[1].z, p[2].w - p[1].w);
      v[3][mt] = make_float4(p[1].x - p[3].x, p[1].y - p[3].y, p[1].z - p[3].z, p[1].w - p[3].w);
    }
    float4 wv[4][NT];
#pragma unroll
    for (int f = 0; f < 4; ++f)
#pragma unroll
      for (int nt = 0; nt < NT; ++nt)
        wv[f][nt] = (n0 + nt * 32 < g.CoutPad)
                        ? *reinterpret_cast<const float4*>(wl + (size_t)f * 16 * fstride + ((size_t)q * 2 * g.CoutPad + nt * 32) * 4)
                        : make_float4(0.f, 0.f, 0.f, 0.f);
#define SSBEV_WG_COMP(COMP)                                                                   \
    _Pragma("unroll") for (int f = 0; f < 4; ++f)                                             \
    _Pragma("unroll") for (int mt = 0; mt < MT; ++mt)                                         \
    _Pragma("unroll") for (int nt = 0; nt < NT; ++nt)                                         \
      acc[f][mt][nt] = __builtin_amdgcn_mfma_f32_32x32x2f32(v[f][mt].COMP, wv[f][nt].COMP, acc[f][mt][nt], 0, 0, 0);
    SSBEV_WG_COMP(x) SSBEV_WG_COMP(y) SSBEV_WG_COMP(z) SSBEV_WG_COMP(w)
#undef SSBEV_WG_COMP
  }
#pragma unroll
  for (int mt = 0; mt < MT; ++mt) {
    const int t0 = (tg * MT + mt) * 32;
    float* o0 = Mo + ((long)xhw * R + ((long)b * g.D + 2 * i) * g.Thw + t0) * g.Cout;
    float* o1 = o0 + (long)g.Thw * g.Cout;
#pragma unroll
    for (int nt = 0; nt < NT; ++nt) {
      const int co = n0 + nt * 32 + li;
      if (co >= g.Cout) continue;
#pragma unroll
      for (int r = 0; r < 16; ++r) {
        const int row = (r & 3) + 8 * (r >> 2) + 4 * lk;
        if (t0 + row < g.Thw) {
          const float m0 = acc[0][mt][nt][r], m1 = acc[1][mt][nt][r], m2 = acc[2][mt][nt][r], m3 = acc[3][mt][nt][r];
          o0[(long)row * g.Cout + co] = m0 + m1 + m2;
          o1[(long)row * g.Cout + co] = m1 - m2 - m3;
        }
      }
    }
  }
}

struct WinoBgemmGeom { long T; int K, N, NPad; };

constexpr int kBgBM = 64, kBgBK = 64, kBgStages = 3;

template <int NT>
__global__ void __launch_bounds__(256)
wino_bgemm_kernel(const float* __restrict__ A, const float* __restrict__ Wp, float* __restrict__ Cm, WinoBgemmGeom g) {
  extern __shared__ __align__(16) float al[];
  const int tid = threadIdx.x, lane = tid & 63, wave = tid >> 6;
  const int li = lane & 31, lk = lane >> 5;
  const int xi = blockIdx.z;
  const int n0 = (blockIdx.y * 4 + wave) * (NT * 32);
  const bool col_active = n0 < g.N;
  const float* Ax = A + (long)xi * g.T * g.K;
  float* Cx = Cm + (long)xi * g.T * g.N;
  const int Q = (g.K + 7) >> 3, nstage = (g.K + kBgBK - 1) / kBgBK;
  const size_t fstride = (size_t)Q * 2 * g.NPad * 4;
  const float* wl = Wp + (size_t)xi * fstride + ((size_t)lk * g.NPad + n0 + li) * 4;
  const long nrb = (g.T + kBgBM - 1) / kBgBM;
  const long rb_per = (nrb + gridDim.x - 1) / gridDim.x;
  const long rb_begin = (long)blockIdx.x * rb_per, rb_end = min(nrb, rb_begin + rb_per);
  const long total = (rb_end - rb_begin) * nstage;
  if (total <= 0) return;

  auto issue = [&](long s) {
    const long rb = rb_begin + s / nstage;
    const int k0 = (int)(s % nstage) * kBgBK, buf = (int)(s % kBgStages);
#pragma unroll
    for (int e = 0; e < 4; ++e) {
      const int jbase = (wave + 4 * e) * 64;
      const int j = jbase + lane, row = j >> 4, slot = j & 15;
      const int src_slot = (slot & 8) | ((slot & 7) ^ (row & 7));
      const long r = rb * kBgBM + row;
      const int k = k0 + src_slot * 4;
      const float* src = (r < g.T && k < g.K) ? Ax + r * g.K + k : kWinoZeros;
      __builtin_amdgcn_global_load_lds(src, al + buf * (kBgBM * kBgBK) + jbase * 4, 16, 0, 0);
    }
  };
  wf32x16 acc[2][NT];
  float4 bvA[kBgBK / 8][NT], bvB[kBgBK / 8][NT];
  auto load_b = [&](long s, float4 (&bv)[kBgBK / 8][NT]) {
    const int st = (int)(s % nstage);
#pragma unroll
    for (int qq = 0; qq < kBgBK / 8; ++qq) {
      const int q = st * (kBgBK / 8) + qq;
#pragma unroll
      for (int nt = 0; nt < NT; ++nt)
        bv[qq][nt] = (col_active && q < Q && n0 + nt * 32 < g.NPad)
                         ? *reinterpret_cast<const float4*>(wl + ((size_t)q * 2 * g.NPad + nt * 32) * 4)
                         : make_float4(0.f, 0.f, 0.f, 0.f);
    }
  };
  issue(0);
  load_b(0, bvA);
  if (total > 1) issue(1);
  for (long s = 0; s < total; ++s) {
    const int st = (int)(s % nstage), buf = (int)(s % kBgStages);
    float4 (&bv)[kBgBK / 8][NT] = (s & 1) ? bvB : bvA;
    if (st == 0) {
#pragma unroll
      for (int mt = 0; mt < 2; ++mt)
#pragma unroll
        for (int nt = 0; nt < NT; ++nt)
#pragma unroll
          for (int r = 0; r < 16; ++r) acc[mt][nt][r] = 0.0f;
    }
    if (s + 1 < total) asm volatile("s_waitcnt vmcnt(4)" ::: "memory");
    else asm volatile("s_waitcnt vmcnt(0)" ::: "memory");
    __syncthreads();
    if (s + 1 < total) { if (s & 1) load_b(s + 1, bvA); else load_b(s + 1, bvB); }
    if (s + 2 < total) issue(s + 2);
    if (col_active) {
      const float* ab = al + buf * (kBgBM * kBgBK);
#pragma unroll
      for (int qq = 0; qq < kBgBK / 8; ++qq) {
        float4 av[2];
#pragma unroll
        for (int mt = 0; mt < 2; ++mt) {
          const int row = mt * 32 + li;
          const int slot = 2 * qq + lk;
          av[mt] = *reinterpret_cast<const float4*>(ab + row * kBgBK + (((slot & 8) | ((slot & 7) ^ (row & 7))) << 2));
        }
#define SSBEV_BG_COMP(COMP)                                                                 \
        _Pragma("unroll") for (int mt = 0; mt < 2; ++mt)                                    \
        _Pragma("unroll") for (int nt = 0; nt < NT; ++nt)                                   \
          acc[mt][nt] = __builtin_amdgcn_mfma_f32_32x32x2f32(av[mt].COMP, bv[qq][nt].COMP, acc[mt][nt], 0, 0, 0);
        SSBEV_BG_COMP(x) SSBEV_BG_COMP(y) SSBEV_BG_COMP(z) SSBEV_BG_COMP(w)
#undef SSBEV_BG_COMP
      }
      if (st == nstage - 1) {
        const long r0 = (rb_begin + s / nstage) * kBgBM;
#pragma unroll
        for (int mt = 0; mt < 2; ++mt)
#pragma unroll
          for (int nt = 0; nt < NT; ++nt) {
            const int co = n0 + nt * 32 + li;
            if (co >= g.N) continue;
#pragma unroll
            for (int r = 0; r < 16; ++r) {
              const long row = r0 + mt * 32 + (r & 3) + 8 * (r >> 2) + 4 * lk;
              if (row < g.T) Cx[row * g.N + co] = acc[mt][nt][r];
            }
          }
      }
    }
  }
}

__global__ void __launch_bounds__(256)
wino_weight_packed_kernel(const float* __restrict__ w, float* __restrict__ Wp, int Cout, int Cin, int mode) {
  const int K = mode == 0 ? Cin : Cout, N = mode == 0 ? Cout : Cin;
  const int KPad = (K + 7) & ~7, NPad = (N + 31) & ~31;
  const int i = blockIdx.x * 256 + threadIdx.x;
  if (i >= KPad * NPad) return;
  const int n = i % NPad, k = i / NPad;
  float u[64];
  if (k < K && n < N) {
    float gk[27];
    const int co = mode == 0 ? n : k, ci = mode == 0 ? k : n;
#pragma unroll
    for (int t = 0; t < 27; ++t) gk[t] = w[((size_t)co * Cin + ci) * 27 + (mode == 0 ? t : 26 - t)];
    float a[36], bb[48];
#pragma unroll
    for (int p = 0; p < 9; ++p) g4(gk + p * 3, 1, a + p * 4, 1);
#pragma unroll
    for (int d = 0; d < 3; ++d)
#pragma unroll
      for (int f = 0; f < 4; ++f) g4(a + d * 12 + f, 4, bb + d * 16 + f, 4);
#pragma unroll
    for (int p = 0; p < 16; ++p) g4(bb + p, 16, u + p, 16);
  } else {
#pragma unroll
    for (int xi = 0; xi < 64; ++xi) u[xi] = 0.0f;
  }
  const int Q = KPad >> 3, q = k >> 3, kh = (k >> 2) & 1, t = k & 3;
#pragma unroll
  for (int xi = 0; xi < 64; ++xi) Wp[((((size_t)xi * Q + q) * 2 + kh) * NPad + n) * 4 + t] = u[xi];
}

bool wino_ok(const ssbev_wino_dims* d) {
  return d && d->B > 0 && d->C > 0 && d->D > 0 && d->H > 0 && d->W > 0 && d->D % 2 == 0 && d->H % 2 == 0 && d->W % 2 == 0;
}

}

extern "C" {

#define SSBEV_WINO_ENTRY(NAME, KERNEL, TSRC, TDST)                                                                 \
  int NAME(const TSRC* src, TDST* dst, const ssbev_wino_dims* d, ssbev_stream_t stream) {                         \
    if (!wino_ok(d) || !src || !dst) return SSBEV_EINVAL;                                                          \
    const long total = (long)d->B * (d->D / 2) * (d->H / 2) * (d->W / 2) * d->C;                                   \
    const WinoGeom g{d->B, d->D, d->H, d->W, d->C};                                                                \
    hipLaunchKernelGGL(KERNEL, dim3(cdiv((size_t)total, 256)), dim3(256), 0, as_stream(stream), src, dst, g, total); \
    return ssbev_launch_status();                                                                                  \
  }

#define SSBEV_WINO2D_ENTRY(NAME, KERNEL, TSRC, TDST)                                                               \
  int NAME(const TSRC* src, TDST* dst, const ssbev_wino_dims* d, ssbev_stream_t stream) {                         \
    if (!wino2d_ok(d) || !src || !dst) return SSBEV_EINVAL;                                                        \
    const long total = (long)d->B * d->D * (d->H / 2) * (d->W / 2) * d->C;                                         \
    const WinoGeom g{d->B, d->D, d->H, d->W, d->C};                                                                \
    hipLaunchKernelGGL(KERNEL, dim3(cdiv((size_t)total, 256)), dim3(256), 0, as_stream(stream), src, dst, g, total); \
    return ssbev_launch_status();                                                                                  \
  }

int ssbev_wino_weight_transform(const float* w, float* U, int Cout, int Cin, int ndim, int mode, ssbev_stream_t stream) {
  if (!w || !U || Cout <= 0 || Cin <= 0 || (ndim != 2 && ndim != 3) || (mode != 0 && mode != 1)) return SSBEV_EINVAL;
  const dim3 grid(cdiv((size_t)Cout * Cin, 256)), block(256);
  if (ndim == 3) hipLaunchKernelGGL(wino_weight_kernel<3>, grid, block, 0, as_stream(stream), w, U, Cout, Cin, mode);
  else hipLaunchKernelGGL(wino_weight_kernel<2>, grid, block, 0, as_stream(stream), w, U, Cout, Cin, mode);
  return ssbev_launch_status();
}

int ssbev_wino_weight_grad(const float* gU, float* gw, int Cout, int Cin, int ndim, ssbev_stream_t stream) {
  if (!gU || !gw || Cout <= 0 || Cin <= 0 || (ndim != 2 && ndim != 3)) return SSBEV_EINVAL;
  const dim3 grid(cdiv((size_t)Cout * Cin, 256)), block(256);
  if (ndim == 3) hipLaunchKernelGGL(wino_weight_grad_kernel<3>, grid, block, 0, as_stream(stream), gU, gw, Cout, Cin);
  else hipLaunchKernelGGL(wino_weight_grad_kernel<2>, grid, block, 0, as_stream(stream), gU, gw, Cout, Cin);
  return ssbev_launch_status();
}

size_t ssbev_wino_dgemm_packed_elems(int Cout, int Cin) {
  const size_t a = (size_t)((Cin + 7) & ~7) * ((Cout + 31) & ~31), b = (size_t)((Cout + 7) & ~7) * ((Cin + 31) & ~31);
  return 64 * (a > b ? a : b);
}

int ssbev_wino_dgemm_pack(const float* w, float* Wp, int Cout, int Cin, int mode, ssbev_stream_t stream) {
  if (!w || !Wp || Cout <= 0 || Cin <= 0 || (mode != 0 && mode != 1)) return SSBEV_EINVAL;
  const int K = mode == 0 ? Cin : Cout, N = mode == 0 ? Cout : Cin;
  const size_t total = (size_t)((K + 7) & ~7) * ((N + 31) & ~31);
  hipLaunchKernelGGL(wino_weight_packed_kernel, dim3(cdiv(total, 256)), dim3(256), 0, as_stream(stream), w, Wp, Cout, Cin,
                     mode);
  return ssbev_launch_status();
}

int ssbev_wino_dgemm(const float* P, const float* Wp, float* Mo, const ssbev_wino_dims* d, int N, ssbev_stream_t stream) {
  if (!wino_ok(d) || !P || !Wp || !Mo || N <= 0 || d->C % 4 != 0) return SSBEV_EINVAL;
  const WinoGemmGeom g{d->B, d->D, (d->H / 2) * (d->W / 2), d->C, N, (N + 31) & ~31};
  static const int forced = [] { const char* e = ssbev_tune("SSBEV_WINO_TILE"); return e ? atoi(e) : 0; }();
  int mt = 1, nt = 2;
  if (forced) { mt = forced / 10; nt = forced % 10; }
  const int tgroups = (g.Thw + 32 * mt - 1) / (32 * mt), tg4 = (tgroups + 3) >> 2;
  dim3 grid((unsigned)((long)g.B * (g.D / 2) * tg4), cdiv(N, nt * 32), 16), block(256);
  hipStream_t st = as_stream(stream);
#define SSBEV_WG_LAUNCH(M_, N_) hipLaunchKernelGGL((wino_dgemm_kernel<M_, N_>), grid, block, 0, st, P, Wp, Mo, g)
  switch (mt * 10 + nt) {
    case 14: SSBEV_WG_LAUNCH(1, 4); break;
    case 13: SSBEV_WG_LAUNCH(1, 3); break;
    case 12: SSBEV_WG_LAUNCH(1, 2); break;
    case 22: SSBEV_WG_LAUNCH(2, 2); break;
    case 21: SSBEV_WG_LAUNCH(2, 1); break;
    case 11: SSBEV_WG_LAUNCH(1, 1); break;
    default: return SSBEV_EINVAL;
  }
#undef SSBEV_WG_LAUNCH
  return ssbev_launch_status();
}

int ssbev_wino_bgemm(const float* A, const float* Wp, float* Cm, int64_t T, int K, int N, ssbev_stream_t stream) {
  if (!A || !Wp || !Cm || T <= 0 || K <= 0 || N <= 0 || K % 4 != 0) return SSBEV_EINVAL;
  const WinoBgemmGeom g{(long)T, K, N, (N + 31) & ~31};
  const int nt = N > 128 ? 2 : 1;
  const long nrb = ((long)T + kBgBM - 1) / kBgBM;
  const int ycols = cdiv(N, 4 * nt * 32);
  long gx = std::max(1L, (768L + 64 * ycols - 1) / (64 * ycols));
  gx = std::min(gx, std::max(1L, nrb / 4));
  dim3 grid((unsigned)gx, ycols, 64), block(256);
  const size_t lds = (size_t)kBgStages * kBgBM * kBgBK * sizeof(float);
  hipStream_t st = as_stream(stream);
  if (nt == 2) hipLaunchKernelGGL(wino_bgemm_kernel<2>, grid, block, lds, st, A, Wp, Cm, g);
  else hipLaunchKernelGGL(wino_bgemm_kernel<1>, grid, block, lds, st, A, Wp, Cm, g);
  return ssbev_launch_status();
}

SSBEV_WINO2D_ENTRY(ssbev_wino2d_input_transform, wino2d_input_kernel<float>, float, float)
SSBEV_WINO2D_ENTRY(ssbev_wino2d_output_transform, wino2d_output_kernel<float>, float, float)
SSBEV_WINO2D_ENTRY(ssbev_wino2d_output_adjoint, wino2d_output_adjoint_kernel<float>, float, float)

SSBEV_WINO_ENTRY(ssbev_wino_input_transform, wino_input_kernel<float>, float, float)
SSBEV_WINO_ENTRY(ssbev_wino_output_transform, wino_output_kernel<float>, float, float)
SSBEV_WINO_ENTRY(ssbev_wino_output_adjoint, wino_output_adjoint_kernel<float>, float, float)

#define SSBEV_WINO43_ENTRY(NAME, KERNEL, DA, TF, TSRC, TDST)                                                        \
  int NAME(const TSRC* src, TDST* dst, const ssbev_wino_dims* d, ssbev_stream_t stream) {                         \
    if (!wino43_ok(d, DA) || !src || !dst) return SSBEV_EINVAL;                                                     \
    const long total = (long)d->B * (DA ? d->D / DA : d->D) * (d->H / 4) * (d->W / 4) * d->C;                      \
    const WinoGeom g{d->B, d->D, d->H, d->W, d->C};                                                                \
    hipLaunchKernelGGL((KERNEL<DA, TF>), dim3(cdiv((size_t)total, 256)), dim3(256), 0, as_stream(stream), src, dst, g, \
                       total);                                                                                     \
    return ssbev_launch_status();                                                                                  \
  }

SSBEV_WINO43_ENTRY(ssbev_wino43_input_transform, wino43_input_kernel, 2, float, float, float)
SSBEV_WINO43_ENTRY(ssbev_wino43_output_transform, wino43_output_kernel, 2, float, float, float)
SSBEV_WINO43_ENTRY(ssbev_wino43_output_adjoint, wino43_output_adjoint_kernel, 2, float, float, float)
SSBEV_WINO43_ENTRY(ssbev_wino43_2d_input_transform, wino43_input_kernel, 0, float, float, float)
SSBEV_WINO43_ENTRY(ssbev_wino43_2d_output_transform, wino43_output_kernel, 0, float, float, float)
SSBEV_WINO43_ENTRY(ssbev_wino43_2d_output_adjoint, wino43_output_adjoint_kernel, 0, float, float, float)
SSBEV_WINO43_ENTRY(ssbev_wino43_input_transform_bf16, wino43_input_kernel, 2, bf16_bits, float, uint16_t)
SSBEV_WINO43_ENTRY(ssbev_wino43_output_transform_bf16, wino43_output_kernel, 2, bf16_bits, uint16_t, float)
SSBEV_WINO43_ENTRY(ssbev_wino43_output_adjoint_bf16, wino43_output_adjoint_kernel, 2, bf16_bits, float, uint16_t)
SSBEV_WINO43_ENTRY(ssbev_wino43_2d_input_transform_bf16, wino43_input_kernel, 0, bf16_bits, float, uint16_t)
SSBEV_WINO43_ENTRY(ssbev_wino43_2d_output_transform_bf16, wino43_output_kernel, 0, bf16_bits, uint16_t, float)
SSBEV_WINO43_ENTRY(ssbev_wino43_2d_output_adjoint_bf16, wino43_output_adjoint_kernel, 0, bf16_bits, float, uint16_t)

SSBEV_WINO43_ENTRY(ssbev_wino444_input_transform, wino43_input_kernel, 4, float, float, float)
SSBEV_WINO43_ENTRY(ssbev_wino444_output_transform, wino43_output_kernel, 4, float, float, float)
SSBEV_WINO43_ENTRY(ssbev_wino444_output_adjoint, wino43_output_adjoint_kernel, 4, float, float, float)

int ssbev_wino43_2d_output_transform_acc(const float* src, float* dst, const ssbev_wino_dims* d, ssbev_stream_t stream) {
  if (!wino43_ok(d, 0) || !src || !dst) return SSBEV_EINVAL;
  const long total = (long)d->B * d->D * (d->H / 4) * (d->W / 4) * d->C;
  WinoGeom g{d->B, d->D, d->H, d->W, d->C};
  g.acc = 1;
  hipLaunchKernelGGL((wino43_output_kernel<0, float>), dim3(cdiv((size_t)total, 256)), dim3(256), 0, as_stream(stream), src, dst, g, total);
  return ssbev_launch_status();
}

int ssbev_wino2d_output_transform_acc(const float* src, float* dst, const ssbev_wino_dims* d, ssbev_stream_t stream) {
  if (!wino2d_ok(d) || !src || !dst) return SSBEV_EINVAL;
  const long total = (long)d->B * d->D * (d->H / 2) * (d->W / 2) * d->C;
  WinoGeom g{d->B, d->D, d->H, d->W, d->C};
  g.acc = 1;
  hipLaunchKernelGGL(wino2d_output_kernel<float>, dim3(cdiv((size_t)total, 256)), dim3(256), 0, as_stream(stream), src, dst, g, total);
  return ssbev_launch_status();
}

int ssbev_wino43_weight_transform(const float* w, float* U, int Cout, int Cin, int ndim, int mode, ssbev_stream_t stream) {
  if (!w || !U || Cout <= 0 || Cin <= 0 || (ndim != 2 && ndim != 3 && ndim != 4) || (mode != 0 && mode != 1)) return SSBEV_EINVAL;
  const dim3 grid(cdiv((size_t)Cout * Cin, 256)), block(256);
  if (ndim == 4) hipLaunchKernelGGL(wino43_weight_kernel<4>, grid, block, 0, as_stream(stream), w, U, Cout, Cin, mode);
  else if (ndim == 3) hipLaunchKernelGGL(wino43_weight_kernel<2>, grid, block, 0, as_stream(stream), w, U, Cout, Cin, mode);
  else hipLaunchKernelGGL(wino43_weight_kernel<0>, grid, block, 0, as_stream(stream), w, U, Cout, Cin, mode);
  return ssbev_launch_status();
}

int ssbev_wino43_weight_grad(const float* gU, float* gw, int Cout, int Cin, int ndim, ssbev_stream_t stream) {
  if (!gU || !gw || Cout <= 0 || Cin <= 0 || (ndim != 2 && ndim != 3 && ndim != 4)) return SSBEV_EINVAL;
  const dim3 grid(cdiv((size_t)Cout * Cin, 256)), block(256);
  if (ndim == 4) hipLaunchKernelGGL(wino43_weight_grad_kernel<4>, grid, block, 0, as_stream(stream), gU, gw, Cout, Cin);
  else if (ndim == 3) hipLaunchKernelGGL(wino43_weight_grad_kernel<2>, grid, block, 0, as_stream(stream), gU, gw, Cout, Cin);
  else hipLaunchKernelGGL(wino43_weight_grad_kernel<0>, grid, block, 0, as_stream(stream), gU, gw, Cout, Cin);
  return ssbev_launch_status();
}

SSBEV_WINO2D_ENTRY(ssbev_wino2d_input_transform_bf16, wino2d_input_kernel<bf16_bits>, float, uint16_t)
SSBEV_WINO2D_ENTRY(ssbev_wino2d_output_transform_bf16, wino2d_output_kernel<bf16_bits>, uint16_t, float)
SSBEV_WINO2D_ENTRY(ssbev_wino2d_output_adjoint_bf16, wino2d_output_adjoint_kernel<bf16_bits>, float, uint16_t)

#define SSBEV_WINO16_ENTRY(NAME, KERNEL, DIV_D, OK)                                                                   \
  int NAME(const uint16_t* src, uint16_t* dst, const ssbev_wino_dims* d, ssbev_stream_t stream) {                    \
    if (!OK(d) || !src || !dst) return SSBEV_EINVAL;                                                                  \
    const int nv = d->C % 2 == 0 ? 2 : 1;                                                                             \
    const long total = (long)d->B * (d->D / DIV_D) * (d->H / 2) * (d->W / 2) * (d->C / nv);                           \
    const WinoGeom g{d->B, d->D, d->H, d->W, d->C};                                                                   \
    if (nv == 2)                                                                                                      \
      hipLaunchKernelGGL((KERNEL<bf16_bits, bf16_bits, 2>), dim3(cdiv((size_t)total, 256)), dim3(256), 0, as_stream(stream), src, dst, g, total); \
    else                                                                                                              \
      hipLaunchKernelGGL((KERNEL<bf16_bits, bf16_bits, 1>), dim3(cdiv((size_t)total, 256)), dim3(256), 0, as_stream(stream), src, dst, g, total); \
    return ssbev_launch_status();                                                                                     \
  }
SSBEV_WINO16_ENTRY(ssbev_wino_input_transform_bf16a, wino_input_kernel, 2, wino_ok)
SSBEV_WINO16_ENTRY(ssbev_wino_output_transform_bf16a, wino_output_kernel, 2, wino_ok)
SSBEV_WINO16_ENTRY(ssbev_wino_output_adjoint_bf16a, wino_output_adjoint_kernel, 2, wino_ok)
SSBEV_WINO16_ENTRY(ssbev_wino2d_input_transform_bf16a, wino2d_input_kernel, 1, wino2d_ok)
SSBEV_WINO16_ENTRY(ssbev_wino2d_output_transform_bf16a, wino2d_output_kernel, 1, wino2d_ok)
SSBEV_WINO16_ENTRY(ssbev_wino2d_output_adjoint_bf16a, wino2d_output_adjoint_kernel, 1, wino2d_ok)

SSBEV_WINO_ENTRY(ssbev_wino_input_transform_bf16, wino_input_kernel<bf16_bits>, float, uint16_t)
SSBEV_WINO_ENTRY(ssbev_wino_output_transform_bf16, wino_output_kernel<bf16_bits>, uint16_t, float)
SSBEV_WINO_ENTRY(ssbev_wino_output_adjoint_bf16, wino_output_adjoint_kernel<bf16_bits>, float, uint16_t)

}
```

stereoscene_amd/csrc/winograd_fused.hip:

```cpp
#include "common.h"

#include <cstdio>
#include <vector>

#include <algorithm>
#include <cstdlib>
#include <type_traits>

namespace {

typedef float wf32x16 __attribute__((ext_vector_type(16)));
__device__ const float kDfZeros[4] = {0.f, 0.f, 0.f, 0.f};

constexpr int DF_BK = 32;

struct DfGeom {
  int B, D, Thw, K, N, NPad;
  int ND;
  int nrowgrp;
  int ncolgrp;
  int NU;
  int nxi;
  unsigned long long* dbg = nullptr;
};
// ... 248 lines not shown
  const int total_stages = g.B * g.ND * g.nrowstage;
  const int s_begin = chunk * g.stages_per_chunk, s_end = min(total_stages, s_begin + g.stages_per_chunk);

  auto issue = [&](int sidx, int buf) {
    const int i = sidx % g.ND, br = sidx / g.ND;
    const int rs = br % g.nrowstage, b = br / g.nrowstage;
    const int t0 = rs * DFW_BR;
#pragma unroll
    for (int e = 0; e < (PI + 3) / 4; ++e) {
      const int j = wave + 4 * e;
      if (PI % 4 != 0 && j >= PI) break;
      const int a = j / PIP, jj = j % PIP, item = jj * 64 + lane;
      const int row = item / PSL, slot = item % PSL;
      const int d = 2 * i - 1 + a, t = t0 + row;
      const int kk = k0 + slot * 4;
      const bool ok = d >= 0 && d < g.D && t < g.Thw && kk < g.K;
      const int off = ((b * g.D + d) * g.Thw + t) * g.K + kk;
      const float* src = ok ? Px + off : kDfZeros;
      __builtin_amdgcn_global_load_lds(src, lds + buf * SF + a * (DFW_BR * PC) + jj * 256, 16, 0, 0);
    }
#pragma unroll
    for (int e = 0; e < (ZI + 3) / 4; ++e) {
      const int j = wave + 4 * e;
      if (ZI % 4 != 0 && j >= ZI) break;
      const int a = j / ZIP, jj = j % ZIP, item = jj * 64 + lane;
      const int row = item / ZSL, slot = item % ZSL;
      const int t = t0 + row, nn = n0 + slot * 4;
      const bool ok = t < g.Thw && nn < g.N;
      const int off = ((b * g.D + 2 * i + a) * g.Thw + t) * g.N + nn;
      const float* src = ok ? Zx + off : kDfZeros;
      __builtin_amdgcn_global_load_lds(src, lds + buf * SF + PF + a * (DFW_BR * ZC) + jj * 256, 16, 0, 0);
    }
  };

  wf32x16 acc[4][NT];
#pragma unroll
  for (int f = 0; f < 4; ++f)
#pragma unroll
    for (int nt = 0; nt < NT; ++nt)
#pragma unroll
      for (int rr = 0; rr < 16; ++rr) acc[f][nt][rr] = 0.0f;

  const bool tile_active = k0 + kw * 32 < g.K && n0 + nw * NT * 32 < g.N;
  if (s_begin < s_end) issue(s_begin, 0);
  for (int sidx = s_begin; sidx < s_end; ++sidx) {
    const int buf = (sidx - s_begin) & 1;
    asm volatile("s_waitcnt vmcnt(0)" ::: "memory");
    __builtin_amdgcn_s_barrier();
    const float* pb = lds + buf * SF;
    const float* zb = pb + PF;
    if (sidx + 1 < s_end) issue(sidx + 1, buf ^ 1);
    if (tile_active) {
      float pc[4], gc[NT][2], pn[4], gn[NT][2];
      auto fetch = [&](int rp, float (&pv)[4], float (&gz)[NT][2]) {
        const int row = 2 * rp + lk;
#pragma unroll
        for (int a = 0; a < 4; ++a) pv[a] = pb[a * (DFW_BR * PC) + row * PC + kw * 32 + li];
#pragma unroll
        for (int nt = 0; nt < NT; ++nt) {
          gz[nt][0] = zb[row * ZC + (nw * NT + nt) * 32 + li];
          gz[nt][1] = zb[DFW_BR * ZC + row * ZC + (nw * NT + nt) * 32 + li];
        }
      };
      fetch(0, pc, gc);
#pragma unroll
      for (int rp = 0; rp < DFW_BR / 2; ++rp) {
        if (rp + 1 < DFW_BR / 2) fetch(rp + 1, pn, gn);
        __builtin_amdgcn_sched_barrier(0);
        const float v0 = pc[0] - pc[2], v1 = pc[1] + pc[2], v2 = pc[2] - pc[1], v3 = pc[1] - pc[3];
#pragma unroll
        for (int nt = 0; nt < NT; ++nt) {
          const float g0 = gc[nt][0], g1 = gc[nt][1];
          acc[0][nt] = __builtin_amdgcn_mfma_f32_32x32x2f32(v0, g0, acc[0][nt], 0, 0, 0);
          acc[1][nt] = __builtin_amdgcn_mfma_f32_32x32x2f32(v1, g0 + g1, acc[1][nt], 0, 0, 0);
          acc[2][nt] = __builtin_amdgcn_mfma_f32_32x32x2f32(v2, g0 - g1, acc[2][nt], 0, 0, 0);
          acc[3][nt] = __builtin_amdgcn_mfma_f32_32x32x2f32(v3, -g1, acc[3][nt], 0, 0, 0);
        }
#pragma unroll
        for (int a = 0; a < 4; ++a) pc[a] = pn[a];
#pragma unroll
        for (int nt = 0; nt < NT; ++nt) { gc[nt][0] = gn[nt][0]; gc[nt][1] = gn[nt][1]; }
      }
    }
    asm volatile("s_waitcnt lgkmcnt(0)" ::: "memory");
  }
  const int kt = k0 + kw * 32;
#pragma unroll
  for (int f = 0; f < 4; ++f) {
    float* dst = part + ((((size_t)chunk * 4 + f) * g.nxi + xhw) * g.K) * g.N;
#pragma unroll
    for (int nt = 0; nt < NT; ++nt) {
      const int n = n0 + (nw * NT + nt) * 32 + li;
      if (n >= g.N) continue;
#pragma unroll
      for (int rr = 0; rr < 16; ++rr) {
        const int k = kt + (rr & 3) + 8 * (rr >> 2) + 4 * lk;
        if (k < g.K) dst[(size_t)k * g.N + n] = acc[f][nt][rr];
      }
    }
  }
}

__device__ __forceinline__ void g43t(const float* u, int s, float* o, int so) {
  const float u0 = u[0], u1 = u[s], u2 = u[2 * s], u3 = u[3 * s], u4 = u[4 * s], u5 = u[5 * s];
  o[0] = 0.25f * u0 - (u1 + u2) * (1.0f / 6.0f) + (u3 + u4) * (1.0f / 24.0f);
  o[so] = (u2 - u1) * (1.0f / 6.0f) + (u3 - u4) * (1.0f / 12.0f);
  o[2 * so] = -(u1 + u2) * (1.0f / 6.0f) + (u3 + u4) * (1.0f / 6.0f) + u5;
}
__device__ __forceinline__ void g23t(const float* u, int s, float* o, int so) {
  const float u0 = u[0], u1 = u[s], u2 = u[2 * s], u3 = u[3 * s];
  o[0] = u0 + 0.5f * (u1 + u2);
  o[so] = 0.5f * (u1 - u2);
  o[2 * so] = 0.5f * (u1 + u2) + u3;
}

__global__ void __launch_bounds__(256)
wino_dfw_sum_kernel(float* __restrict__ part, size_t n4, int nchunk) {
  const size_t i = (size_t)blockIdx.x * 256 + threadIdx.x;
  if (i >= n4) return;
  float4 a = reinterpret_cast<const float4*>(part)[i];
  for (int c = 1; c < nchunk; ++c) {
    const float4 o = reinterpret_cast<const float4*>(part)[(size_t)c * n4 + i];
    a.x += o.x; a.y += o.y; a.z += o.z; a.w += o.w;
  }
  reinterpret_cast<float4*>(part)[i] = a;
}

__global__ void __launch_bounds__(256)
wino_dfw_reduce_kernel(const float* __restrict__ gU, float* __restrict__ gw, int Cout, int Cin) {
  const int idx = blockIdx.x * 256 + threadIdx.x;
  if (idx >= Cin * Cout) return;
  const int co = idx % Cout, ci = idx / Cout;
  float u[144];
  const size_t slab = (size_t)Cin * Cout;
#pragma unroll
  for (int x = 0; x < 144; ++x) u[x] = gU[(size_t)x * slab + idx];
  float a1[72];
#pragma unroll
  for (int p = 0; p < 24; ++p) g43t(u + p * 6, 1, a1 + p * 3, 1);
  float a2[36];
#pragma unroll
  for (int fd = 0; fd < 4; ++fd)
#pragma unroll
    for (int f = 0; f < 3; ++f) g43t(a1 + fd * 18 + f, 3, a2 + fd * 9 + f, 3);
  float gk[27];
#pragma unroll
  for (int p = 0; p < 9; ++p) g23t(a2 + p, 9, gk + p, 9);
#pragma unroll
  for (int t = 0; t < 27; ++t) gw[((size_t)co * Cin + ci) * 27 + t] = gk[t];
}

bool df_dims_ok(const ssbev_wino_dims* d, int N) {
  return d && d->B > 0 && d->C > 0 && d->D > 0 && d->H > 0 && d->W > 0 && d->H % 4 == 0 && d->W % 4 == 0 && d->D % 2 == 0 &&
         d->C % DF_BK == 0 && N > 0 && N % 4 == 0;
}

int env_int(const char* name, int dflt) {
  const char* v = ssbev_tune(name);
  return v ? atoi(v) : dflt;
}

}

extern "C" {

int ssbev_wino43_df_supported(const ssbev_wino_dims* d, int N) { return df_dims_ok(d, N) ? 1 : 0; }

size_t ssbev_wino43_df_packed_elems(int Cout, int Cin) {
  const size_t a = (size_t)((Cin + 7) & ~7) * ((Cout + 31) & ~31), b = (size_t)((Cout + 7) & ~7) * ((Cin + 31) & ~31);
  return 144 * (a > b ? a : b);
}

int ssbev_wino43_df_pack(const float* w, float* Wp, int Cout, int Cin, int mode, ssbev_stream_t stream) {
  if (!w || !Wp || Cout <= 0 || Cin <= 0 || (mode != 0 && mode != 1)) return SSBEV_EINVAL;
  const int K = mode == 0 ? Cin : Cout, N = mode == 0 ? Cout : Cin;
  const int KPad = (K + 7) & ~7, NPad = (N + 31) & ~31;
  hipLaunchKernelGGL(wino_df_pack_kernel, dim3((unsigned)((KPad / 4) * ((NPad + 63) / 64))), dim3(256), 0, as_stream(stream), w,
                     Wp, Cout, Cin, mode);
  return ssbev_launch_status();
}

struct DfPlan { int mt, nw, ncolgrp, nrowgrp, nst; long grid; size_t lds; };

static DfPlan df_instance(const ssbev_wino_dims* d, int N) {
  int mt, nw;
  const int ntile = ((N + 31) & ~31) / 32, Thw = (d->H / 4) * (d->W / 4), ND = d->D / 2;
  static const int forced_nw = env_int("SSBEV_DF_NW", 0), forced_mt = env_int("SSBEV_DF_MT", 0);
  nw = ntile % 4 == 0 ? 4 : (ntile % 3 == 0 ? 3 : (ntile % 2 == 0 ? 2 : 4));
  if (forced_nw >= 2 && forced_nw <= 4) nw = forced_nw;
  const int ncolgrp = (ntile + nw - 1) / nw;
  mt = 2;
  if ((long)36 * d->B * ND * ((Thw + 63) / 64) * ncolgrp < 2048) mt = 1;
  if (((Thw + 63) / 64) * 64 * 10 > ((Thw + 31) / 32) * 32 * 11) mt = 1;
  if (nw == 3) mt = 1;
  static const int nw2_mt = env_int("SSBEV_DF_NW2_MT", 1);
  if (nw == 2) mt = nw2_mt == 2 ? 2 : 1;
  if (forced_mt == 1 || forced_mt == 2) mt = forced_mt;
  const int key = mt * 10 + nw;
  if (key != 24 && key != 23 && key != 22 && key != 14 && key != 13 && key != 12) { mt = 1; nw = 2; }
  DfPlan p;
  p.mt = mt; p.nw = nw;
  p.ncolgrp = (ntile + nw - 1) / nw;
  p.nrowgrp = (Thw + 32 * mt - 1) / (32 * mt);
  p.nst = d->C / DF_BK;
  p.grid = (long)36 * d->B * ND * p.nrowgrp * p.ncolgrp;
  p.lds = (size_t)2 * 4 * 32 * mt * DF_BK * sizeof(float);
  return p;
}

int ssbev_wino43_df_instance(const ssbev_wino_dims* d, int N) {
  if (!df_dims_ok(d, N)) return 0;
  const DfPlan p = df_instance(d, N);
  return p.mt * 10 + p.nw;
}

int ssbev_wino43_df_gemm(const float* P, const float* Wp, float* Mo, const ssbev_wino_dims* d, int N, ssbev_stream_t stream) {
  if (!df_dims_ok(d, N) || !P || !Wp || !Mo) return SSBEV_EINVAL;
  DfGeom g;
  g.B = d->B; g.D = d->D; g.Thw = (d->H / 4) * (d->W / 4); g.K = d->C; g.N = N; g.NPad = (N + 31) & ~31;
  g.ND = d->D / 2;
  const DfPlan pl = df_instance(d, N);
  const int mt = pl.mt, nw = pl.nw;
  g.ncolgrp = pl.ncolgrp;
  g.nrowgrp = pl.nrowgrp;
  g.NU = g.B * g.ND * g.nrowgrp;
  g.nxi = 36;
  const size_t lds = pl.lds;
  const long nwg = pl.grid;
  hipStream_t st = as_stream(stream);
#ifdef SSBEV_DF_CLOCKS
#define DF_CLOCKS_BEGIN(NW_)                                                                                               \
  unsigned long long* dbg_dev = nullptr;                                                                                   \
  const bool dbg_on = ssbev_tune("SSBEV_DF_TIMES") != nullptr;                                                                \
  if (dbg_on) { if (hipMalloc(&dbg_dev, (size_t)nwg * NW_ * 32) != hipSuccess) return SSBEV_ELAUNCH; g.dbg = dbg_dev; }
#define DF_CLOCKS_END(NW_)                                                                                                 \
  if (dbg_on) {                                                                                                            \
    std::vector<unsigned long long> h((size_t)nwg * NW_ * 4);                                                              \
    (void)hipStreamSynchronize(st); (void)hipMemcpy(h.data(), dbg_dev, h.size() * 8, hipMemcpyDeviceToHost); (void)hipFree(dbg_dev); \
    double ph[3] = {0, 0, 0}; unsigned long long t0 = ~0ull, t1 = 0;                                                       \
    for (size_t w = 0; w < (size_t)nwg * NW_; ++w) { for (int i = 0; i < 3; ++i) ph[i] += (double)h[w * 4 + i];            \
      t0 = std::min(t0, h[w * 4 + 3]); t1 = std::max(t1, h[w * 4 + 3] + h[w * 4] + h[w * 4 + 1] + h[w * 4 + 2]); }         \
    const double nw_ = (double)nwg * NW_;                                                                                  \
    fprintf(stderr, "wino_df<mt %d, %d> K=%d N=%d: clocks per wave: prologue %.0f stages %.0f (%d stages) epilogue %.0f | span %.0f, %ld workgroups\n", \
            mt, NW_, g.K, g.N, ph[0] / nw_, ph[1] / nw_, g.K / DF_BK, ph[2] / nw_, (double)(t1 - t0), nwg);                \
  }
#else
#define DF_CLOCKS_BEGIN(NW_)
#define DF_CLOCKS_END(NW_)
#endif
#define SSBEV_DF_LAUNCH(MT_, NW_)                                                                                          \
  do {                                                                                                                     \
    auto kern = wino_df_kernel<MT_, NW_>;                                                                                  \
    if (lds > 64 * 1024 - 1 &&                                                                                             \
        hipFuncSetAttribute(reinterpret_cast<const void*>(kern), hipFuncAttributeMaxDynamicSharedMemorySize, (int)lds) !=  \
            hipSuccess)                                                                                                    \
      return SSBEV_ELAUNCH;                                                                                                \
    DF_CLOCKS_BEGIN(NW_)                                                                                                    \
    hipLaunchKernelGGL(kern, dim3((unsigned)nwg), dim3(64 * NW_), lds, st, P, Wp, Mo, g);                                  \
    DF_CLOCKS_END(NW_)                                                                                                      \
  } while (0)
  switch (mt * 10 + nw) {
    case 24: SSBEV_DF_LAUNCH(2, 4); break;
    case 23: SSBEV_DF_LAUNCH(2, 3); break;
    case 22: SSBEV_DF_LAUNCH(2, 2); break;
    case 14: SSBEV_DF_LAUNCH(1, 4); break;
    case 13: SSBEV_DF_LAUNCH(1, 3); break;
    default: SSBEV_DF_LAUNCH(1, 2); break;
  }
#undef SSBEV_DF_LAUNCH
  return ssbev_launch_status();
}

struct DfwPlan { int kw, nt, br, pc, zc, nkb, nnb, nchunk, stages_per_chunk, total_stages; long grid; size_t lds, workspace; };

static DfwPlan dfw_plan(const ssbev_wino_dims* d, int N) {
  DfwPlan p;
  const int K = d->C;
  if (K <= 64) { p.kw = 2; p.nt = 1; p.br = 16; }
  else if (N % 96 == 0) { p.kw = 4; p.nt = 3; p.br = 8; }
  else { p.kw = 4; p.nt = 2; p.br = 16; }
  p.pc = p.kw * 32;
  p.zc = (4 / p.kw) * p.nt * 32;
  p.nkb = (K + p.pc - 1) / p.pc;
  p.nnb = (N + p.zc - 1) / p.zc;
  const int Thw = (d->H / 4) * (d->W / 4);
  p.total_stages = d->B * (d->D / 2) * ((Thw + p.br - 1) / p.br);
  static const int target = env_int("SSBEV_DFW_WGS", 1024);
  const int per = 36 * p.nkb * p.nnb;
  int nchunk = std::max(1, target / per);
  {
    double best = -1.0;
    int best_n = nchunk;
    for (int n = std::max(1, nchunk * 2 / 3); n <= nchunk * 2; ++n) {
      const long tot = (long)per * n, rounds = (tot + 511) / 512;
      const double eff = (double)tot / (double)(rounds * 512) - 0.002 * std::abs(n - nchunk);
      if (eff > best) { best = eff; best_n = n; }
    }
    nchunk = best_n;
  }
  p.nchunk = std::min(nchunk, std::max(1, p.total_stages / 8));
  p.stages_per_chunk = (p.total_stages + p.nchunk - 1) / p.nchunk;
  p.grid = (long)per * p.nchunk;
  p.lds = (size_t)2 * (4 * p.br * p.pc + 2 * p.br * p.zc) * sizeof(float);
  p.workspace = (size_t)p.nchunk * 144 * K * N * sizeof(float);
  return p;
}

// ... 56 lines not shown
```

stereoscene_amd/functional.py:

```python
import ctypes as C
import math

import os

import numpy as np
import torch

from . import capi, streams



class KernelTimer:

    def __init__(self, families=None):
        self.records = []
        self.counts = {}
        self.families = families

    def span(self, family, flops, nbytes=0.0, tag=None, executed=None):
        c = self.counts.setdefault(family, dict(launches=0, flops=0.0, bytes=0.0, executed=0.0))
        c["launches"] += 1
        c["flops"] += flops
        c["bytes"] += nbytes
        c["executed"] += flops if executed is None else executed
# ... 846 lines not shown
    R, K, N = a.shape[-2], a.shape[-1], b.shape[-1]
    out = torch.empty(*a.shape[:-2], K, N, dtype=torch.float32, device=a.device)
    g = _gdims(R, N, K, batch, lda, ldb, N, sa, sb, K * N)
    if ep_mul is not None:
        ep_mul, ep_rowsub = ep_mul.contiguous(), ep_rowsub.contiguous().float()
        if tuple(ep_mul.shape) != tuple(out.shape) or ep_rowsub.numel() != batch * K:
            raise capi.SsbevError("gemm_tn: epilogue operand shapes")
        g.ep_mul, g.ep_rowsub = ep_mul.data_ptr(), ep_rowsub.data_ptr()
    lib = capi.load()
    ws = _ws(lib.ssbev_gemm_tn_workspace(C.byref(g)), a.device)
    fl = 2.0 * batch * R * N * K
    with _span("gemm_own", fl, 4.0 * (a.numel() + b.numel() + out.numel() * (2 if ep_mul is not None else 1)),
               tag or f"tn {batch}x{R}x{K}x{N}"):
        capi.check(lib.ssbev_gemm_tn(_rawptr(a), _rawptr(b), capi.ptr(out), C.byref(g), capi.ptr(ws), ws.numel(), capi.stream()),
                   "ssbev_gemm_tn")
    return out


class _LinearCL(torch.autograd.Function):

    @staticmethod
    def forward(ctx, x2, w2, bias):
        ctx.save_for_backward(x2, w2)
        ctx.has_bias = bias is not None
        return gemm_nt(x2, w2, bias, tag=f"linear fwd {w2.shape[1]}->{w2.shape[0]} rows={x2.shape[0]}")

    @staticmethod
    def backward(ctx, gy):
        x2, w2 = ctx.saved_tensors
        gy = gy.contiguous()
        gx = gw = gb = None
        if ctx.needs_input_grad[0]:
            gx = gemm_nn(gy, w2, tag=f"linear dgrad {w2.shape[1]}->{w2.shape[0]} rows={x2.shape[0]}")
        if ctx.needs_input_grad[1]:
            gw = gemm_tn(gy, x2, tag=f"linear wgrad {w2.shape[1]}->{w2.shape[0]} rows={x2.shape[0]}")
        if ctx.has_bias and ctx.needs_input_grad[2]:
            gb = gy.sum(0)
        return gx, gw, gb


_D2S_TABLES = {}


def _d2s_table(B, D, H, W, k, Co, device):
    key = (B, D, H, W, k, Co, str(device))
    t = _D2S_TABLES.get(key)
    if t is None:
        t = torch.empty(B * D * H * W, dtype=torch.int64, device=device)
        capi.check(capi.load().ssbev_gemm_d2s_rowoff(capi.ptr(t), B * D * H * W, D, H, W, k[0], k[1], k[2], Co, capi.stream()),
                   "ssbev_gemm_d2s_rowoff")
        _D2S_TABLES[key] = t
    return t


class _DeconvKS(torch.autograd.Function):

    @staticmethod
    def forward(ctx, xcl, weight, bias, k):
        B, D, H, W, Ci = xcl.shape
        Co = weight.shape[1]
        kd, kh, kw = k
        taps = kd * kh * kw
        wk = weight.detach().permute(0, 2, 3, 4, 1).reshape(Ci, taps * Co).contiguous()
        table = _d2s_table(B, D, H, W, k, Co, xcl.device)
        y = torch.empty(B, D * kd, H * kh, W * kw, Co, dtype=torch.float32, device=xcl.device)
        x2 = xcl.reshape(-1, Ci)
        R = x2.shape[0]
        g = _gdims(R, taps * Co, Ci, 1, Ci, taps * Co, 0, 0, 0, 0, 0, ((D, H, W, kd, kh, kw, Co), table))
        fl = 2.0 * R * Ci * taps * Co
        with _span("gemm_own", fl, 4.0 * (x2.numel() + wk.numel() + y.numel()), f"deconv k=s fwd {Ci}->{Co} k{kd}{kh}{kw}"):
            capi.check(capi.load().ssbev_gemm_nn(capi.ptr(x2), capi.ptr(wk), capi.ptr(bias.detach().contiguous() if bias is not None else None),
                                                 capi.ptr(y), C.byref(g), None, 0, capi.stream()), "ssbev_gemm_nn")
        ctx.save_for_backward(x2, wk)
        ctx.meta = (B, D, H, W, Ci, Co, k, bias is not None)
        return y

    @staticmethod
    def backward(ctx, gy):
        x2, wk = ctx.saved_tensors
        B, D, H, W, Ci, Co, k, has_bias = ctx.meta
        kd, kh, kw = k
        taps = kd * kh * kw
        gy = gy.contiguous()
        table = _d2s_table(B, D, H, W, k, Co, gy.device)
        d2s = ((D, H, W, kd, kh, kw, Co), table)
        R = x2.shape[0]
        lib = capi.load()
        gx = gw = gb = None
        fl = 2.0 * R * Ci * taps * Co
        if ctx.needs_input_grad[0]:
            gx2 = torch.empty(R, Ci, dtype=torch.float32, device=gy.device)
            g = _gdims(R, Ci, taps * Co, 1, 0, taps * Co, Ci, 0, 0, 0, 0, d2s)
            ws = _ws(lib.ssbev_gemm_nt_workspace(C.byref(g)), gy.device)
            with _span("gemm_own", fl, 4.0 * (gy.numel() + wk.numel() + gx2.numel()), f"deconv k=s dgrad {Ci}->{Co} k{kd}{kh}{kw}"):
                capi.check(lib.ssbev_gemm_nt(capi.ptr(gy), capi.ptr(wk), None, capi.ptr(gx2), C.byref(g), capi.ptr(ws), ws.numel(),
                                             capi.stream()), "ssbev_gemm_nt")
            gx = gx2.view(B, D, H, W, Ci)
        if ctx.needs_input_grad[1]:
            gwk = torch.empty(Ci, taps * Co, dtype=torch.float32, device=gy.device)
            g = _gdims(R, taps * Co, Ci, 1, Ci, 0, taps * Co, 0, 0, Ci * taps * Co, 0, d2s)
            ws = _ws(lib.ssbev_gemm_tn_workspace(C.byref(g)), gy.device)
            with _span("gemm_own", fl, 4.0 * (gy.numel() + x2.numel() + gwk.numel()), f"deconv k=s wgrad {Ci}->{Co} k{kd}{kh}{kw}"):
                capi.check(lib.ssbev_gemm_tn(capi.ptr(x2), capi.ptr(gy), capi.ptr(gwk), C.byref(g), capi.ptr(ws), ws.numel(),
                                             capi.stream()), "ssbev_gemm_tn")
            gw = gwk.view(Ci, kd, kh, kw, Co).permute(0, 4, 1, 2, 3).contiguous()
        if has_bias and ctx.needs_input_grad[2]:
            gb = gy.reshape(-1, Co).sum(0)
        return gx, gw, gb, None


GEMM_LAYERS = os.environ.get("SSBEV_GEMM_LAYERS", "1") != "0"
GEMM_MIN_CIN = int(os.environ.get("SSBEV_GEMM_MIN_CIN", "512"))


def _deconv_k_eq_s_gemm(x, weight, bias, k):
    if tuple(k) == (1, 1, 1) and own_gemm_site("deconv") and own_gemm_site("linear") and weight.shape[1] % 4 == 0:
        return linear_cl(x, weight.reshape(weight.shape[0], weight.shape[1]).t(), bias)
    xcl = to_cl(_f32(x, "deconv_gemm"))
    B, D, H, W, Ci = xcl.shape
    Co = weight.shape[1]
    kd, kh, kw = k
    if own_gemm_site("deconv") and Co % 64 == 0 and Ci % 4 == 0:
        return from_cl(_DeconvKS.apply(xcl, weight, bias, (int(kd), int(kh), int(kw))))
    w2 = weight.permute(0, 2, 3, 4, 1).reshape(Ci, kd * kh * kw * Co)
    fl = 2.0 * B * D * H * W * Ci * kd * kh * kw * Co
    nby = 4.0 * (xcl.numel() + w2.numel() + B * D * H * W * kd * kh * kw * Co)
    mult = 3.0 if (torch.is_grad_enabled() and (x.requires_grad or weight.requires_grad)) else 1.0
    with _span("gemm_lib", fl * mult, nby * mult, f"fwd   deconv k=s {Ci}->{Co} k{kd}{kh}{kw}"):
        g = torch.mm(xcl.reshape(-1, Ci), w2).view(B, D, H, W, kd, kh, kw, Co)
    y = g.permute(0, 1, 4, 2, 5, 3, 6, 7).reshape(B, D * kd, H * kh, W * kw, Co)
    if bias is not None:
        y = y + bias
    return from_cl(y)


def conv_transpose3d(x, weight, bias=None, stride=1, padding=0, output_padding=0):
    st, pd, op = _triple(stride, 3), _triple(padding, 3), _triple(output_padding, 3)
    if storage_bf16() and x.is_cuda and TILE_HINT in (0, 9):
        y = _conv16_route(x, weight, bias, st, pd, (1, 1, 1), True, op)
        if y is not None:
            return y
        return _to_act(_ConvNd.apply(x, weight, bias, st, pd, (1, 1, 1), True, op))
    if (GEMM_LAYERS and TILE_HINT == 0 and PRECISION == "fp32" and x.is_cuda and tuple(weight.shape[2:]) == tuple(st)
            and pd == (0, 0, 0) and op == (0, 0, 0) and weight.shape[0] >= 128):
        return _deconv_k_eq_s_gemm(x, weight, bias, tuple(st))
    return _ConvNd.apply(x, weight, bias, _triple(stride, 3), _triple(padding, 3), (1, 1, 1), True,
                         _triple(output_padding, 3))


DILATED_POLYPHASE = os.environ.get("SSBEV_DILATED_POLYPHASE", "1") != "0"
POLYPHASE_MAX_PAD = float(os.environ.get("SSBEV_POLYPHASE_MAX_PAD", "1.35"))


def _dilated_polyphase(x, weight, d):
    B, Cc, H, W = x.shape
    Hp, Wp = -(-H // (2 * d)) * 2 * d, -(-W // (2 * d)) * 2 * d
    if Hp * Wp > POLYPHASE_MAX_PAD * H * W:
        return None
    xp = torch.nn.functional.pad(x, [0, Wp - W, 0, Hp - H]) if (Hp != H or Wp != W) else x
    xs = xp.reshape(B, Cc, Hp // d, d, Wp // d, d).permute(0, 3, 5, 1, 2, 4).reshape(B * d * d, Cc, Hp // d, Wp // d)
    ys = conv2d(xs, weight, None, 1, 1, 1)
    Co = weight.shape[0]
    y = ys.reshape(B, d, d, Co, Hp // d, Wp // d).permute(0, 3, 4, 1, 5, 2).reshape(B, Co, Hp, Wp)
    return y[:, :, :H, :W]


def conv2d(x, weight, bias=None, stride=1, padding=0, dilation=1):
    s, p, dl = _triple(stride, 2), _triple(padding, 2), _triple(dilation, 2)
    if storage_bf16() and x.is_cuda and TILE_HINT in (0, 9):
        x5, w5 = x.unsqueeze(2), weight.unsqueeze(2)
        if (DILATED_POLYPHASE and WINOGRAD and WINO_BF16S and tuple(weight.shape[2:]) == (3, 3) and s == (1, 1) and dl[0] == dl[1]
                and dl[0] > 1 and p == dl and min(weight.shape[0], weight.shape[1]) >= 64):
            y = _dilated_polyphase(x, weight, dl[0])
            if y is not None:
                return y if bias is None else y + _like_act(bias, y).view(1, -1, 1, 1)
        if WINOGRAD and WINO_BF16S and wino_conv3d_applicable(x5, w5, (1,) + s, (0,) + p, (1,) + dl):
            y = _WinoConv.apply(x5, w5, _slot_of(x)).squeeze(2)
            return y if bias is None else y + _like_act(bias, y).view(1, -1, 1, 1)
        y = _conv16_route(x5, w5, bias, (1,) + s, (0,) + p, (1,) + dl, False, (0, 0, 0))
        if y is None:
            y = _to_act(_ConvNd.apply(x5, w5, bias, (1,) + s, (0,) + p, (1,) + dl, False, (0, 0, 0)))
        return y.squeeze(2)
    if (GEMM_LAYERS and TILE_HINT == 0 and PRECISION == "fp32" and x.is_cuda and tuple(weight.shape[2:]) == (1, 1)
            and s == (1, 1) and p == (0, 0) and weight.shape[1] >= GEMM_MIN_CIN):
        return linear_cl(x, weight, bias)
    if (DILATED_POLYPHASE and WINOGRAD and TILE_HINT == 0 and x.is_cuda and tuple(weight.shape[2:]) == (3, 3) and s == (1, 1)
            and dl[0] == dl[1] and dl[0] > 1 and p == dl and min(weight.shape[0], weight.shape[1]) >= 64):
        y = _dilated_polyphase(x, weight, dl[0])
        if y is not None:
            return y if bias is None else y + bias.view(1, -1, 1, 1)
    x5, w5 = x.unsqueeze(2), weight.unsqueeze(2)
    if WINOGRAD and TILE_HINT == 0 and wino_conv3d_applicable(x5, w5, (1,) + s, (0,) + p, (1,) + dl):
        y = _WinoConv.apply(x5, w5, _slot_of(x)).squeeze(2)
        return y if bias is None else y + bias.view(1, -1, 1, 1)
    y = _ConvNd.apply(x5, w5, bias, (1,) + s, (0,) + p, (1,) + dl, False, (0, 0, 0), _slot_of(x))
    return y.squeeze(2)



_WINO_G = None


def _wino_g(device):
    global _WINO_G
    if _WINO_G is None or _WINO_G.device != device:
        _WINO_G = torch.tensor([[1.0, 0.0, 0.0], [0.5, 0.5, 0.5], [0.5, -0.5, 0.5], [0.0, 0.0, 1.0]], device=device)
    return _WINO_G


PRECISION = os.environ.get("SSBEV_PRECISION", "fp32")
_MODES = ("fp32", "bf16", "bf16_operands")


def set_precision(mode):
    global PRECISION
    if mode not in _MODES:
        raise ValueError(f"precision must be one of {_MODES}, got {mode!r}")
    PRECISION = mode


def storage_bf16():
    return PRECISION == "bf16"


def act_dtype():
    return torch.bfloat16 if PRECISION == "bf16" else torch.float32


def _like_act(y, ref):
    return y if y.dtype == ref.dtype else y.to(ref.dtype)


def _wino_call(name, src, dims, out_shape, dtype=torch.float32):
    lib = capi.load()
    dst = torch.empty(out_shape, dtype=dtype, device=src.device)
    capi.check(getattr(lib, name)(capi.ptr(src), capi.ptr(dst), C.byref(dims), capi.stream()), name)
    return dst


WINO_DEPTH_FUSED = os.environ.get("SSBEV_WINO_DEPTH_FUSED", "0") != "0"


WINO_OWN_GEMM = os.environ.get("SSBEV_WINO_OWN_GEMM", "0") != "0"


def gemm16_nn(a16, b32, out_fp32=False, tag=None):
    lib = capi.load()
    Bt, M, K = a16.shape
    N = b32.shape[2]
    d = capi.Gemm16Dims(M, N, K, Bt, int(out_fp32))
    n = lib.ssbev_gemm16_packed_elems(C.byref(d))
    if n == 0 or a16.dtype != torch.bfloat16 or b32.dtype != torch.float32 or tuple(b32.shape[:2]) != (Bt, K):
        return None
    a16, b32 = a16.contiguous(), b32.contiguous()
    packed = torch.empty(n, dtype=torch.int16, device=a16.device)
    out = torch.empty(Bt, M, N, dtype=torch.float32 if out_fp32 else torch.bfloat16, device=a16.device)
    with _span("gemm16", 2.0 * Bt * M * K * N, 2.0 * (a16.numel() + out.numel()) + 4.0 * b32.numel(), tag or f"gemm16 {Bt}x[{M}x{K}x{N}]"):
        capi.check(lib.ssbev_gemm16_pack(capi.ptr(b32), capi.ptr(packed), C.byref(d), capi.stream()), "ssbev_gemm16_pack")
        capi.check(lib.ssbev_gemm16_nn(capi.ptr(a16), capi.ptr(packed), capi.ptr(out), C.byref(d), capi.stream()), "ssbev_gemm16_nn")
    return out


GEMM16_OWN = os.environ.get("SSBEV_GEMM16_OWN", "1") != "0"


def _bmm16(V, U):
    if GEMM16_OWN and V.is_cuda:
        M = gemm16_nn(V, U, tag=f"wino16 gemm {V.shape[0]}x[{V.shape[1]}x{V.shape[2]}x{U.shape[2]}]")
        if M is not None:
            return M
    return torch.bmm(V, U.to(torch.bfloat16))


def gemm16_tn(a16, b16, tag=None):
    lib = capi.load()
    Bt, M, K = a16.shape
    N = b16.shape[2]
    d = capi.Gemm16Dims(M, N, K, Bt, 1)
    if (K % 8 or N % 8 or a16.dtype != torch.bfloat16 or b16.dtype != torch.bfloat16 or tuple(b16.shape[:2]) != (Bt, M)
            or Bt >= 65536):
        return None
    a16, b16 = a16.contiguous(), b16.contiguous()
    out = torch.empty(Bt, K, N, dtype=torch.float32, device=a16.device)
    ws = torch.empty(max(int(lib.ssbev_gemm16_tn_workspace(C.byref(d))), 4), dtype=torch.float32, device=a16.device)
    with _span("gemm16", 2.0 * Bt * M * K * N, 2.0 * (a16.numel() + b16.numel()) + 4.0 * out.numel(), tag or f"gemm16 tn {Bt}x[{K}x{M}x{N}]"):
        capi.check(lib.ssbev_gemm16_tn(capi.ptr(a16), capi.ptr(b16), capi.ptr(out), C.byref(d), capi.ptr(ws), ws.numel(),
                                       capi.stream()), "ssbev_gemm16_tn")
    return out


def _bmm16_tn(V, Z):
    if GEMM16_OWN and V.is_cuda:
        g = gemm16_tn(V, Z, tag=f"wino16 wgrad gemm {V.shape[0]}x[{V.shape[2]}x{V.shape[1]}x{Z.shape[2]}]")
        if g is not None:
            return g
    return torch.bmm(V.transpose(1, 2), Z, out_dtype=torch.float32)


def _wino_bgemm(V, w, Cout, Cin, mode):
    lib = capi.load()
    T, K = V.shape[1], V.shape[2]
    N = Cout if mode == 0 else Cin
    Wp = torch.empty(lib.ssbev_wino_dgemm_packed_elems(Cout, Cin), dtype=torch.float32, device=V.device)
    capi.check(lib.ssbev_wino_dgemm_pack(capi.ptr(w), capi.ptr(Wp), Cout, Cin, mode, capi.stream()), "ssbev_wino_dgemm_pack")
    M = torch.empty(64, T, N, dtype=torch.float32, device=V.device)
    capi.check(lib.ssbev_wino_bgemm(capi.ptr(V), capi.ptr(Wp), capi.ptr(M), T, K, N, capi.stream()), "ssbev_wino_bgemm")
    return M


def _wino_depth_fused(xcl, w, B, D, H, W, K, N, mode):
    lib = capi.load()
    Cout, Cin = (N, K) if mode == 0 else (K, N)
    R = B * D * (H // 2) * (W // 2)
    P = _wino_call("ssbev_wino2d_input_transform", xcl, capi.WinoDims(B, D, H, W, K), (16, R, K))
    Wp = torch.empty(lib.ssbev_wino_dgemm_packed_elems(Cout, Cin), dtype=torch.float32, device=xcl.device)
    capi.check(lib.ssbev_wino_dgemm_pack(capi.ptr(w), capi.ptr(Wp), Cout, Cin, mode, capi.stream()), "ssbev_wino_dgemm_pack")
    Mo = torch.empty(16, R, N, dtype=torch.float32, device=xcl.device)
    dims = capi.WinoDims(B, D, H, W, K)
    capi.check(lib.ssbev_wino_dgemm(capi.ptr(P), capi.ptr(Wp), capi.ptr(Mo), C.byref(dims), N, capi.stream()),
               "ssbev_wino_dgemm")
    del P
    return _wino_call("ssbev_wino2d_output_transform", Mo, capi.WinoDims(B, D, H, W, N), (B, D, H, W, N))


WINO_F43 = os.environ.get("SSBEV_WINO_F43", "1") != "0"
WINO_F43_2D = os.environ.get("SSBEV_WINO_F43_2D", "0") != "0"
WINO_F43_2D_DEPTHNET = os.environ.get("SSBEV_WINO_F43_2D_DEPTHNET", "0") != "0"
_F43_2D_SCOPE = 0


class wino_f43_2d_scope:

    def __enter__(self):
        global _F43_2D_SCOPE
        _F43_2D_SCOPE += 1 if WINO_F43_2D_DEPTHNET else 0
        return self

    def __exit__(self, *exc):
        global _F43_2D_SCOPE
        _F43_2D_SCOPE -= 1 if WINO_F43_2D_DEPTHNET else 0
        return False
WINO_F444 = os.environ.get("SSBEV_WINO_F444", "0") != "0"
WINO_F444_MIN_CIN = int(os.environ.get("SSBEV_WINO_F444_MIN_CIN", "0"))


WINO_DF = os.environ.get("SSBEV_WINO_DF", "1") != "0"
WINO_DF_MIN_ROWS = int(os.environ.get("SSBEV_WINO_DF_MIN_ROWS", "1024"))


def _wino_df_applicable(B, D, H, W, Cin, Cout):
    if not (WINO_DF and WINO_F43 and PRECISION == "fp32" and not (WINO_DEPTH_FUSED or WINO_OWN_GEMM or WINO_F444)):
        return False
    if B * D * (H // 4) * (W // 4) < WINO_DF_MIN_ROWS:
        return False
    lib = capi.load()
    return bool(lib.ssbev_wino43_df_supported(C.byref(capi.WinoDims(B, D, H, W, Cin)), Cout)) and \
        bool(lib.ssbev_wino43_df_supported(C.byref(capi.WinoDims(B, D, H, W, Cout)), Cin)) and Cout % 4 == 0


def _wino_df_gemm(xcl, w, B, D, H, W, K, N, mode, tag, fl, into=None):
    lib = capi.load()
    Cout, Cin = (N, K) if mode == 0 else (K, N)
    R = B * D * (H // 4) * (W // 4)
    with _span("wino_transform", 0.0, 4.0 * xcl.numel() * 3.25, tag + " in"):
        P = _wino_call("ssbev_wino43_2d_input_transform", xcl, capi.WinoDims(B, D, H, W, K), (36, R, K))
    Wp = torch.empty(lib.ssbev_wino43_df_packed_elems(Cout, Cin), dtype=torch.float32, device=xcl.device)
    capi.check(lib.ssbev_wino43_df_pack(capi.ptr(w), capi.ptr(Wp), Cout, Cin, mode, capi.stream()), "ssbev_wino43_df_pack")
    Mo = torch.empty(36, R, N, dtype=torch.float32, device=xcl.device)
    dims = capi.WinoDims(B, D, H, W, K)
    nby = 4.0 * (P.numel() + Mo.numel() + Wp.numel())
    with _span(f"conv_wino_fused:{lib.ssbev_wino43_df_instance(C.byref(dims), N)}" if KERNEL_TIMER is not None else "conv_wino_fused",
               fl, nby, tag, fl / 6.0):
        capi.check(lib.ssbev_wino43_df_gemm(capi.ptr(P), capi.ptr(Wp), capi.ptr(Mo), C.byref(dims), N, capi.stream()),
                   "ssbev_wino43_df_gemm")
    with _span("wino_transform", 0.0, 4.0 * B * D * H * W * N * (3.25 + (into is not None)), tag + " out"):
        if into is not None:
            odims = capi.WinoDims(B, D, H, W, N)
            capi.check(lib.ssbev_wino43_2d_output_transform_acc(capi.ptr(Mo), capi.ptr(into), C.byref(odims), capi.stream()),
                       "ssbev_wino43_2d_output_transform_acc")
            y = into
        else:
            y = _wino_call("ssbev_wino43_2d_output_transform", Mo, capi.WinoDims(B, D, H, W, N), (B, D, H, W, N))
    return y, P


class _WinoConvDF(torch.autograd.Function):

    @staticmethod
    def forward(ctx, x, weight, slot=None):
        ctx.slot = slot
        if ctx.needs_input_grad[1]:
            streams.note_use(weight)
        xcl = to_cl(_f32(x, "wino_conv"))
        B, D, H, W, Cin = xcl.shape
        Cout = weight.shape[0]
        fl = 2.0 * B * D * H * W * Cin * Cout * 27
        w = weight.detach().contiguous()
        y, P = _wino_df_gemm(xcl, w, B, D, H, W, Cin, Cout, 0, f"winoDF fwd {Cin}->{Cout} {D}x{H}x{W}", fl)
        ctx.save_for_backward(P if weight.requires_grad else None, weight)
        ctx.geom = (B, D, H, W, Cin, Cout, fl)
        return from_cl(y)

    @staticmethod
    def backward(ctx, gy):
        P, weight = ctx.saved_tensors
        B, D, H, W, Cin, Cout, fl = ctx.geom
        gcl = to_cl(gy)
        lib = capi.load()
        w = weight.detach().contiguous()
        gx = gw = None

        def weight_gradient():
            R = B * D * (H // 4) * (W // 4)
            with _span("wino_transform", 0.0, 4.0 * gcl.numel() * 3.25, "winoDF wgrad adjoint"):
                Z = _wino_call("ssbev_wino43_2d_output_adjoint", gcl, capi.WinoDims(B, D, H, W, Cout), (36, R, Cout))
            dims = capi.WinoDims(B, D, H, W, Cin)
            ws = _ws(lib.ssbev_wino43_df_wgrad_workspace(C.byref(dims), Cout), gy.device)
            gwt = torch.empty_like(w)
            nby = 4.0 * (P.numel() + Z.numel() + 144 * Cin * Cout)
            with _span("conv_wino_fused_wgrad", fl, nby, f"winoDF wgrad {Cin}->{Cout} {D}x{H}x{W}", fl / 6.0):
                capi.check(lib.ssbev_wino43_df_wgrad(capi.ptr(P), capi.ptr(Z), capi.ptr(gwt), C.byref(dims), Cout, capi.ptr(ws),
                                                     ws.numel(), capi.stream()), "ssbev_wino43_df_wgrad")
            return gwt

        gw_side = ctx.needs_input_grad[1] and streams.wgrad_on_side(weight)
        if gw_side:
            with streams.on_side(gy.device, gcl, P) as side:
                gw = weight_gradient()
                side.publish(gw)
        if ctx.needs_input_grad[0]:
            into = _slot_target(ctx.slot, torch.empty((B, D, H, W, Cin), device="meta"))
            gxcl, _ = _wino_df_gemm(gcl, w, B, D, H, W, Cout, Cin, 1, f"winoDF dgrad {Cin}->{Cout} {D}x{H}x{W}", fl, into=into)
            if ctx.slot is not None:
                ctx.slot.buf = gxcl
            gx = from_cl(gxcl)
        if ctx.needs_input_grad[1] and not gw_side:
            gw = weight_gradient()
        return gx, gw, None


class _WinoConv(torch.autograd.Function):

    @staticmethod
    def _plan(three_d, D, H, W, bf, cin=1 << 30):
        f43 = WINO_F43 and (three_d or WINO_F43_2D or _F43_2D_SCOPE > 0) and not bf and H % 4 == 0 and W % 4 == 0 and \
            not (three_d and (WINO_DEPTH_FUSED or WINO_OWN_GEMM))
        if f43 and three_d and WINO_F444 and D % 4 == 0 and cin >= WINO_F444_MIN_CIN:
            return 4, "ssbev_wino444_", 216, 4, 8.0
        if f43:
            pre = "ssbev_wino43_" if three_d else "ssbev_wino43_2d_"
            nf, th, reduction = (144, 4, 6.0) if three_d else (36, 4, 4.0)
        else:
            pre = "ssbev_wino_" if three_d else "ssbev_wino2d_"
            nf, th, reduction = (64, 2, 3.375) if three_d else (16, 2, 2.25)
        return (1 if f43 else 0), pre, nf, th, reduction

    @staticmethod
    def forward(ctx, x, weight, slot=None):
        ctx.slot = slot
        if ctx.needs_input_grad[1]:
            streams.note_use(weight)
        bf = PRECISION != "fp32"
        a16 = storage_bf16()
        xcl = to_cl(x if x.dtype == torch.bfloat16 else x.to(torch.bfloat16)) if a16 else to_cl(_f32(x, "wino_conv"))
        B, D, H, W, Cin = xcl.shape
        Cout, three_d = weight.shape[0], weight.shape[2] == 3
        f43, pre, nf, th, red = _WinoConv._plan(three_d, D, H, W, bf, Cin)
        T = B * (D // (4 if f43 == 4 else 2) if three_d else D) * (H // th) * (W // th)
        lib = capi.load()
        w = weight.detach().contiguous()
        fl = 2.0 * B * D * H * W * Cin * Cout * (27 if three_d else 9)
        fused = three_d and WINO_DEPTH_FUSED and not bf and not f43
        wt = lib.ssbev_wino43_weight_transform if f43 else lib.ssbev_wino_weight_transform
        wdim = 4 if f43 == 4 else (3 if three_d else 2)
        if not fused:
            U = torch.empty(nf, Cin, Cout, dtype=torch.float32, device=x.device)
            capi.check(wt(capi.ptr(w), capi.ptr(U), Cout, Cin, wdim, 0, capi.stream()), "ssbev_wino_weight_transform")
        tag = f"wino{ {0: '', 1: '43', 4: '444'}[f43]} fwd {Cin}->{Cout} {D}x{H}x{W}"
        nby = 4.0 * (B * D * H * W * (Cin + Cout) + (27 if three_d else 9) * Cin * Cout)
        with _span("conv_winograd", fl, nby, tag, fl / red):
            if fused:
                y = _wino_depth_fused(xcl, w, B, D, H, W, Cin, Cout, 0)
                V = None
            elif bf:
                sfx = "_bf16a" if a16 else "_bf16"
                V = _wino_call(pre + "input_transform" + sfx, xcl, capi.WinoDims(B, D, H, W, Cin), (nf, T, Cin), torch.bfloat16)
                M = _bmm16(V, U)
                y = _wino_call(pre + "output_transform" + sfx, M, capi.WinoDims(B, D, H, W, Cout), (B, D, H, W, Cout),
                               torch.bfloat16 if a16 else torch.float32)
            else:
                V = _wino_call(pre + "input_transform", xcl, capi.WinoDims(B, D, H, W, Cin), (nf, T, Cin))
                M = _wino_bgemm(V, w, Cout, Cin, 0) if (three_d and WINO_OWN_GEMM and not f43) else (gemm_nn(V, U, tag=tag + " gemm") if own_gemm_site("wino") else torch.bmm(V, U))
                y = _wino_call(pre + "output_transform", M, capi.WinoDims(B, D, H, W, Cout), (B, D, H, W, Cout))
        ctx.save_for_backward(xcl if fused else V, weight)
        ctx.geom = (B, D, H, W, Cin, Cout, T, three_d, fl, fused, bf, f43, pre, nf, red, a16)
        return from_cl(y)

    @staticmethod
    def backward(ctx, gy):
        V, weight = ctx.saved_tensors
        B, D, H, W, Cin, Cout, T, three_d, fl, fused, bf, f43, pre, nf, red, a16 = ctx.geom
        sfx, fdt = (("_bf16a" if a16 else "_bf16"), torch.bfloat16) if bf else ("", torch.float32)
        gcl = to_cl(gy)
        if a16 and gcl.dtype != torch.bfloat16:
            gcl = gcl.to(torch.bfloat16)
        adt = torch.bfloat16 if a16 else torch.float32
        lib = capi.load()
        w = weight.detach().contiguous()
        nd = 4 if f43 == 4 else (3 if three_d else 2)
        gx = gw = None
        vtag = {0: "", 1: "43", 4: "444"}[f43]
        nby = 4.0 * (B * D * H * W * (Cin + Cout) + (27 if three_d else 9) * Cin * Cout)
        if ctx.needs_input_grad[0] and fused:
            with _span("conv_winograd", fl, nby, f"wino dgrad {Cin}->{Cout} {D}x{H}x{W}", fl / red):
                gx = from_cl(_wino_depth_fused(gcl, w, B, D, H, W, Cout, Cin, 1))
        elif ctx.needs_input_grad[0]:
            Ut = torch.empty(nf, Cout, Cin, dtype=torch.float32, device=gy.device)
            wt = lib.ssbev_wino43_weight_transform if f43 else lib.ssbev_wino_weight_transform
            capi.check(wt(capi.ptr(w), capi.ptr(Ut), Cout, Cin, nd, 1, capi.stream()), "ssbev_wino_weight_transform")
            with _span("conv_winograd", fl, nby, f"wino{vtag} dgrad {Cin}->{Cout} {D}x{H}x{W}", fl / red):
                Vg = _wino_call(pre + "input_transform" + sfx, gcl, capi.WinoDims(B, D, H, W, Cout), (nf, T, Cout), fdt)
                Mx = _wino_bgemm(Vg, w, Cout, Cin, 1) if (three_d and WINO_OWN_GEMM and not bf and not f43) \
                    else ((_bmm16(Vg, Ut) if fdt == torch.bfloat16 else torch.bmm(Vg, Ut.to(fdt))) if (bf or not own_gemm_site("wino")) else gemm_nn(Vg, Ut, tag="wino dgrad gemm"))
                del Vg
                acc_fn = {"ssbev_wino2d_": "ssbev_wino2d_output_transform_acc",
                          "ssbev_wino43_2d_": "ssbev_wino43_2d_output_transform_acc"}.get(pre) if not bf else None
                into = _slot_target(ctx.slot, torch.empty((B, D, H, W, Cin), device="meta")) if acc_fn else None
                if into is not None:
                    odims = capi.WinoDims(B, D, H, W, Cin)
                    capi.check(getattr(lib, acc_fn)(capi.ptr(Mx), capi.ptr(into), C.byref(odims), capi.stream()), acc_fn)
                    gxcl = into
                else:
                    gxcl = _wino_call(pre + "output_transform" + sfx, Mx, capi.WinoDims(B, D, H, W, Cin), (B, D, H, W, Cin), adt)
                if ctx.slot is not None:
                    ctx.slot.buf = gxcl
            gx = from_cl(gxcl)
        if ctx.needs_input_grad[1]:
            def weight_gradient(V=V):
                with _span("conv_winograd_wgrad", fl, nby, f"wino{vtag} wgrad {Cin}->{Cout} {D}x{H}x{W}", fl / red):
                    if fused:
                        V = _wino_call(pre + "input_transform", V, capi.WinoDims(B, D, H, W, Cin), (nf, T, Cin))
                    Z = _wino_call(pre + "output_adjoint" + sfx, gcl, capi.WinoDims(B, D, H, W, Cout), (nf, T, Cout), fdt)
                    gU = _bmm16_tn(V, Z) if bf else (gemm_tn(V, Z, tag="wino wgrad gemm") if own_gemm_site("wino") else torch.bmm(V.transpose(1, 2), Z))
                gwt = torch.empty_like(w)
                wg = lib.ssbev_wino43_weight_grad if f43 else lib.ssbev_wino_weight_grad
                capi.check(wg(capi.ptr(gU), capi.ptr(gwt), Cout, Cin, nd, capi.stream()), "ssbev_wino_weight_grad")
                return gwt

            if streams.wgrad_on_side(weight):
                with streams.on_side(gy.device, gcl, V) as side:
                    gw = weight_gradient()
                    side.publish(gw)
            else:
                gw = weight_gradient()
        return gx, gw, None


def conv_flops_3x3(B, D, H, W, Cin, Cout):
    return 2.0 * B * D * H * W * Cin * Cout * 27


def wino_conv3d_applicable(x, weight, stride, padding, dilation):
    k = tuple(weight.shape[2:])
    if not (x.is_cuda and tuple(stride) == (1, 1, 1) and tuple(dilation) == (1, 1, 1) and weight.shape[0] >= 64
            and weight.shape[1] >= 64 and weight.shape[1] % 4 == 0):
        return False
    if k == (3, 3, 3):
        return tuple(padding) == (1, 1, 1) and all(int(n) % 2 == 0 for n in x.shape[2:])
    if k == (1, 3, 3):
        return tuple(padding) == (0, 1, 1) and all(int(n) % 2 == 0 for n in x.shape[3:])
    return False




class _DcnIm2col(torch.autograd.Function):

    @staticmethod
    def forward(ctx, x, offset, groups, k, pad, dil):
        lib = capi.load()
        xcl, ocl = to_cl(_f32(x, "dcn")), to_cl(_f32(offset, "dcn"))
        B, H, W, Cch = xcl.shape
        d = capi.DcnDims(B, Cch, H, W, groups, k, pad, dil)
        cols = torch.empty(groups, B * H * W, k * k * (Cch // groups), dtype=torch.float32, device=x.device)
        with _span("dcn_sample", 0.0, 4.0 * (xcl.numel() + ocl.numel() + cols.numel()), "fwd   dcn_im2col"):
            capi.check(lib.ssbev_dcn_im2col(capi.ptr(xcl), capi.ptr(ocl), capi.ptr(cols), C.byref(d), capi.stream()),
                       "ssbev_dcn_im2col")
        ctx.save_for_backward(xcl, ocl)
        ctx.d = d
        return cols

    @staticmethod
    def backward(ctx, gcols):
        lib = capi.load()
        xcl, ocl = ctx.saved_tensors
        gx, goff = torch.empty_like(xcl), torch.empty_like(ocl)
        ws = _ws(lib.ssbev_dcn_col2im_workspace(C.byref(ctx.d)), xcl.device)
        with _span("dcn_sample", 0.0, 4.0 * (2 * xcl.numel() + 2 * ocl.numel() + gcols.numel()), "bwd   dcn_col2im"):
            capi.check(lib.ssbev_dcn_col2im(capi.ptr(xcl), capi.ptr(ocl), capi.ptr(gcols.contiguous()), capi.ptr(gx),
                                            capi.ptr(goff), C.byref(ctx.d), capi.ptr(ws), ws.numel(), capi.stream()),
                       "ssbev_dcn_col2im")
        return from_cl(gx), from_cl(goff), None, None, None, None


def deform_conv2d(x, offset, weight, groups=1, padding=1, dilation=1):
    Cout, Cg, k, _ = weight.shape
    B, _, H, W = x.shape
    cols = _DcnIm2col.apply(x, offset, int(groups), int(k), int(padding), int(dilation))
    Cog = Cout // groups
    Kc = k * k * Cg
    if (x.is_cuda and own_gemm_site("linear") and _gemm_supported(cols) and PRECISION == "fp32" and Cog % 4 == 0 and Kc % 4 == 0):
        w3 = weight.view(groups, Cog, Cg, k, k).permute(0, 1, 3, 4, 2).reshape(groups, Cog, Kc)
        y2 = _GroupedLinearCL.apply(cols, w3)
        return from_cl(y2.view(B, H, W, Cout))
    outs = []
    for g, cg in enumerate(cols.unbind(0)):
        colg = cg.view(B, H, W, Kc).permute(0, 3, 1, 2)
        wg = weight[g * Cog:(g + 1) * Cog].permute(0, 2, 3, 1).reshape(Cog, Kc, 1, 1)
        outs.append(conv2d(colg, wg, None, 1, 0, 1))
    return torch.cat(outs, dim=1) if groups > 1 else outs[0]


class _GroupedLinearCL(torch.autograd.Function):

    @staticmethod
    def forward(ctx, cols, w3):
        lib = capi.load()
        cols, w3 = cols.contiguous(), w3.contiguous()
        G, R, K = cols.shape
        N = w3.shape[1]
        y = torch.empty(R, G * N, dtype=torch.float32, device=cols.device)
        g = _gdims(R, N, K, G, K, K, G * N, R * K, N * K, N)
        ws = _ws(lib.ssbev_gemm_nt_workspace(C.byref(g)), cols.device)
        with _span("gemm_own", 2.0 * G * R * N * K, 4.0 * (cols.numel() + w3.numel() + y.numel()), f"linear fwd grouped {G}x[{K}->{N}] rows={R}"):
            capi.check(lib.ssbev_gemm_nt(capi.ptr(cols), capi.ptr(w3), None, capi.ptr(y), C.byref(g), capi.ptr(ws), ws.numel(),
                                         capi.stream()), "ssbev_gemm_nt")
        ctx.save_for_backward(cols, w3)
        return y

    @staticmethod
    def backward(ctx, gy):
        lib = capi.load()
        cols, w3 = ctx.saved_tensors
        G, R, K = cols.shape
        N = w3.shape[1]
        gy = gy.contiguous()
        gcols = gw = None
        fl = 2.0 * G * R * N * K
        if ctx.needs_input_grad[0]:
            gcols = torch.empty_like(cols)
            g = _gdims(R, K, N, G, G * N, K, K, N, N * K, R * K)
            ws = _ws(lib.ssbev_gemm_nn_workspace(C.byref(g)), gy.device)
            with _span("gemm_own", fl, 4.0 * (gy.numel() + w3.numel() + gcols.numel()), f"linear dgrad grouped {G}x[{K}->{N}] rows={R}"):
                capi.check(lib.ssbev_gemm_nn(capi.ptr(gy), capi.ptr(w3), None, capi.ptr(gcols), C.byref(g), capi.ptr(ws), ws.numel(),
                                             capi.stream()), "ssbev_gemm_nn")
        if ctx.needs_input_grad[1]:
            gw = torch.empty_like(w3)
            g = _gdims(R, K, N, G, G * N, K, K, N, R * K, N * K)
            ws = _ws(lib.ssbev_gemm_tn_workspace(C.byref(g)), gy.device)
            with _span("gemm_own", fl, 4.0 * (gy.numel() + cols.numel() + gw.numel()), f"linear wgrad grouped {G}x[{K}->{N}] rows={R}"):
                capi.check(lib.ssbev_gemm_tn(capi.ptr(gy), capi.ptr(cols), capi.ptr(gw), C.byref(g), capi.ptr(ws), ws.numel(),
                                             capi.stream()), "ssbev_gemm_tn")
        return gcols, gw




GN_RELU_MASK = os.environ.get("SSBEV_GN_RELU_MASK", "1") != "0"


def _norm_ext(device, running=None, n=0):
    e = capi.NormExt(None, None, 0.0, int(n))
    if running is not None:
        e.running_mean, e.running_var, e.momentum = running[0].data_ptr(), running[1].data_ptr(), float(running[2])
    return e


class _GroupNorm(torch.autograd.Function):

    @staticmethod
    def forward(ctx, x, weight, bias, residual, groups, eps, relu, as_batch, given_mean, given_rstd, pre_act=0, res_slot=None,
                running=None):
        lib = capi.load()
        ctx.res_slot = res_slot
        ctx.set_materialize_grads(False)
        xcl, io = _act(to_cl(x), "group_norm")
        Cch = xcl.shape[-1]
        B = 1 if as_batch else xcl.shape[0]
        S = xcl.numel() // (B * Cch)
        rcl = to_cl(residual if residual.dtype == xcl.dtype else residual.to(xcl.dtype)) if residual is not None else None
        given = given_mean is not None
        d = capi.NormDims(B, Cch, groups, S, float(eps), int(relu), int(given), int(pre_act), 0, 0, io)
        y = torch.empty_like(xcl)
        mean = given_mean.contiguous() if given else torch.empty(B * groups, dtype=torch.float32, device=x.device)
        rstd = given_rstd.contiguous() if given else torch.empty(B * groups, dtype=torch.float32, device=x.device)
        ws = _ws(lib.ssbev_groupnorm_workspace(C.byref(d)), x.device)
        w, b = weight.detach().contiguous(), bias.detach().contiguous()
        nb = float(xcl.element_size()) * xcl.numel() * (3 + (residual is not None) - 2 * given)
        use_mask = bool(relu) and GN_RELU_MASK and not given and any(ctx.needs_input_grad[:4])
        mask = torch.empty(lib.ssbev_groupnorm_mask_words(C.byref(d)), dtype=torch.int64, device=x.device) if use_mask else None
        ext = _norm_ext(x.device, running, B * S)
        with _span("groupnorm", 0.0, nb, f"fwd   N C={Cch} G={groups} S={S} res={int(residual is not None)}"):
            capi.check(lib.ssbev_groupnorm_fwd_ext(capi.ptr(xcl), capi.ptr(w), capi.ptr(b), capi.ptr(rcl), capi.ptr(y),
                                                   capi.ptr(mean), capi.ptr(rstd), capi.ptr(mask) if use_mask else None,
                                                   C.byref(d), C.byref(ext), capi.ptr(ws), ws.numel(), capi.stream()),
                       "ssbev_groupnorm_fwd_ext")
        ctx.save_for_backward(xcl, (mask if use_mask else y) if relu else None, w, mean, rstd)
        ctx.use_mask = use_mask
# ... 874 lines not shown
```

Measured before the change: 30.32 million voxels/s.

## Add native dilated 2-D Winograd F(2,3) path via per-axis phase tile tables

Adds direct Winograd support for dilated 3x3 2-D convolutions. Per-axis tile start tables cover each dilation phase, so the input, output and adjoint kernels gather taps at stride dil, with bounds guards for ragged edges. The dilated conv path now goes to this route before the polyphase path, which padded and reshuffled the input. The intent is to drop polyphase padding and rearrangement copies, at the cost of extra tile overhead on uneven phases, a 128-tile cap per axis, and a wider WinoDims struct.

```diff
diff --git a/include/ssbev.h b/include/ssbev.h
--- a/include/ssbev.h
+++ b/include/ssbev.h
@@ -308,10 +308,12 @@
 int ssbev_chan_scale(const float* x, const float* gate, float* y, int B, int64_t S, int C, float scale,
                      ssbev_stream_t stream);
 
-typedef struct { int B, D, H, W, C; } ssbev_wino_dims;
+typedef struct { int B, D, H, W, C; int dil; } ssbev_wino_dims;
 int ssbev_wino_input_transform(const float* x, float* V, const ssbev_wino_dims* d, ssbev_stream_t stream);
 int ssbev_wino_output_transform(const float* M, float* y, const ssbev_wino_dims* d, ssbev_stream_t stream);
 int ssbev_wino_output_adjoint(const float* gy, float* Z, const ssbev_wino_dims* d, ssbev_stream_t stream);
+#define SSBEV_WINO2D_MAX_AXIS_TILES 128
+int ssbev_wino2d_axis_tiles(int extent, int dil, uint16_t* first, int cap);
 int ssbev_wino2d_input_transform(const float* x, float* V, const ssbev_wino_dims* d, ssbev_stream_t stream);
 int ssbev_wino2d_output_transform(const float* M, float* y, const ssbev_wino_dims* d, ssbev_stream_t stream);
 int ssbev_wino2d_output_adjoint(const float* gy, float* Z, const ssbev_wino_dims* d, ssbev_stream_t stream);
diff --git a/stereoscene_amd/capi.py b/stereoscene_amd/capi.py
--- a/stereoscene_amd/capi.py
+++ b/stereoscene_amd/capi.py
@@ -74,7 +74,7 @@
 
 
 class WinoDims(C.Structure):
-    _fields_ = [(n, C.c_int) for n in ("B", "D", "H", "W", "C")]
+    _fields_ = [(n, C.c_int) for n in ("B", "D", "H", "W", "C", "dil")]
 
 
 class UpsampleDims(C.Structure):
@@ -238,6 +238,7 @@
     "ssbev_wino43_df_wgrad_workspace": (C.c_size_t, [C.POINTER(WinoDims), C.c_int]),
     "ssbev_wino43_df_wgrad": (C.c_int, [_P, _P, _P, C.POINTER(WinoDims), C.c_int, _P, C.c_size_t, _P]),
     "ssbev_wino43_df_plan_query": (C.c_int, [C.POINTER(WinoDims), C.c_int, C.POINTER(Wino43DfPlan)]),
+    "ssbev_wino2d_axis_tiles": (C.c_int, [C.c_int, C.c_int, C.POINTER(C.c_uint16), C.c_int]),
     "ssbev_wino2d_input_transform": (C.c_int, [_P, _P, C.POINTER(WinoDims), _P]),
     "ssbev_wino2d_output_transform": (C.c_int, [_P, _P, C.POINTER(WinoDims), _P]),
     "ssbev_wino2d_output_adjoint": (C.c_int, [_P, _P, C.POINTER(WinoDims), _P]),
diff --git a/stereoscene_amd/csrc/capi.hip b/stereoscene_amd/csrc/capi.hip
--- a/stereoscene_amd/csrc/capi.hip
+++ b/stereoscene_amd/csrc/capi.hip
@@ -28,7 +28,7 @@
 }
 
 extern "C" {
-int ssbev_version(void) { return 110;  }
+int ssbev_version(void) { return 111;  }
 const char* ssbev_build_arch(void) { return "gfx950"; }
 
 void ssbev_env_refresh(void) {
diff --git a/stereoscene_amd/csrc/winograd.hip b/stereoscene_amd/csrc/winograd.hip
--- a/stereoscene_amd/csrc/winograd.hip
+++ b/stereoscene_amd/csrc/winograd.hip
@@ -5,7 +5,16 @@
 
 namespace {
 
-struct WinoGeom { int B, D, H, W, C; int acc = 0; };
+struct WinoGeom {
+  int B, D, H, W, C; int acc = 0;
+  static constexpr bool kDil = false;
+};
+constexpr int kWinoMaxAxisTiles = SSBEV_WINO2D_MAX_AXIS_TILES;
+struct WinoGeomDil : WinoGeom {
+  int dil, TH, TW;
+  unsigned short h0[kWinoMaxAxisTiles], w0[kWinoMaxAxisTiles];
+  static constexpr bool kDil = true;
+};
 __device__ const float kWinoZeros[4] = {0.f, 0.f, 0.f, 0.f};
 
 typedef unsigned short bf16_bits;
@@ -68,6 +77,24 @@
   bd = t / (g.H / 2);
 }
 
+template <int NV>
+__device__ __forceinline__ void wino_tile2(long i, const WinoGeom& g, int& c, long& tile, int& h0, int& w0, int& dl, long& bd) {
+  int tw, th;
+  wino_decode2<NV>(i, g, c, tile, tw, th, bd);
+  h0 = 2 * th; w0 = 2 * tw; dl = 1;
+}
+template <int NV>
+__device__ __forceinline__ void wino_tile2(long i, const WinoGeomDil& g, int& c, long& tile, int& h0, int& w0, int& dl, long& bd) {
+  const int cq = g.C / NV;
+  c = NV * (int)(i % cq);
+  long t = i / cq;
+  tile = t;
+  w0 = g.w0[(int)(t % g.TW)]; t /= g.TW;
+  h0 = g.h0[(int)(t % g.TH)];
+  bd = t / g.TH;
+  dl = g.dil;
+}
+
 template <typename TF, typename TA = float, int NV = 1>
 __global__ void __launch_bounds__(256)
 wino_input_kernel(const TA* __restrict__ x, TF* __restrict__ V, WinoGeom g, long total) {
@@ -219,21 +246,21 @@
   }
 }
 
-template <typename TF, typename TA = float, int NV = 1>
-__global__ void __launch_bounds__(256)
-wino2d_input_kernel(const TA* __restrict__ x, TF* __restrict__ V, WinoGeom g, long total) {
+template <typename TF, typename TA = float, int NV = 1, typename G = WinoGeom>
+__global__ void __launch_bounds__(256)
+wino2d_input_kernel(const TA* __restrict__ x, TF* __restrict__ V, G g, long total) {
   const long i = (long)blockIdx.x * 256 + threadIdx.x;
   if (i >= total) return;
-  int c, tw, th;
+  int c, h0, w0, dl;
   long tile, bd;
-  wino_decode2<NV>(i, g, c, tile, tw, th, bd);
+  wino_tile2<NV>(i, g, c, tile, h0, w0, dl, bd);
   float v[NV][16];
 #pragma unroll
   for (int e = 0; e < 4; ++e) {
-    const int h = 2 * th - 1 + e;
+    const int h = h0 + (e - 1) * dl;
 #pragma unroll
     for (int f = 0; f < 4; ++f) {
-      const int w = 2 * tw - 1 + f;
+      const int w = w0 + (f - 1) * dl;
       const bool ok = h >= 0 && h < g.H && w >= 0 && w < g.W;
       float t[NV];
 #pragma unroll
@@ -260,14 +287,16 @@
   }
 }
 
-template <typename TF, typename TA = float, int NV = 1>
-__global__ void __launch_bounds__(256)
-wino2d_output_kernel(const TF* __restrict__ M, TA* __restrict__ y, WinoGeom g, long total) {
+template <typename TF, typename TA = float, int NV = 1, typename G = WinoGeom>
+__global__ void __launch_bounds__(256)
+wino2d_output_kernel(const TF* __restrict__ M, TA* __restrict__ y, G g, long total) {
   const long i = (long)blockIdx.x * 256 + threadIdx.x;
   if (i >= total) return;
-  int c, tw, th;
+  int c, h0, w0, dl;
   long tile, bd;
-  wino_decode2<NV>(i, g, c, tile, tw, th, bd);
+  wino_tile2<NV>(i, g, c, tile, h0, w0, dl, bd);
+  const long rstep = (long)dl * g.W * g.C;
+  const bool row1 = !G::kDil || h0 + dl < g.H;
   const long T = total / (g.C / NV);
   float m[NV][16];
 #pragma unroll
@@ -285,10 +314,13 @@
   if (g.acc) {
 #pragma unroll
     for (int f = 0; f < 2; ++f) {
-      const long base = ((bd * g.H + 2 * th) * g.W + 2 * tw + f) * g.C + c;
+      if (G::kDil && w0 + f * dl >= g.W) continue;
+      const long base = ((bd * g.H + h0) * g.W + w0 + f * dl) * g.C + c;
       float t0[NV], t1[NV];
       ldv<NV>(y + base, t0);
-      ldv<NV>(y + base + (long)g.W * g.C, t1);
+#pragma unroll
+      for (int n = 0; n < NV; ++n) t1[n] = 0.0f;
+      if (row1) ldv<NV>(y + base + rstep, t1);
 #pragma unroll
       for (int n = 0; n < NV; ++n) { oldv[n][2 * f] = t0[n]; oldv[n][2 * f + 1] = t1[n]; }
     }
@@ -307,27 +339,31 @@
       y0[n] = r[0 * 2 + f] + r[1 * 2 + f] + r[2 * 2 + f] + oldv[n][2 * f];
       y1[n] = r[1 * 2 + f] - r[2 * 2 + f] - r[3 * 2 + f] + oldv[n][2 * f + 1];
     }
-    const long base = ((bd * g.H + 2 * th) * g.W + 2 * tw + f) * g.C + c;
+    if (G::kDil && w0 + f * dl >= g.W) continue;
+    const long base = ((bd * g.H + h0) * g.W + w0 + f * dl) * g.C + c;
     stv<NV>(y + base, y0);
-    stv<NV>(y + base + (long)g.W * g.C, y1);
-  }
-}
-
-template <typename TF, typename TA = float, int NV = 1>
-__global__ void __launch_bounds__(256)
-wino2d_output_adjoint_kernel(const TA* __restrict__ gy, TF* __restrict__ Z, WinoGeom g, long total) {
+    if (row1) stv<NV>(y + base + rstep, y1);
+  }
+}
+
+template <typename TF, typename TA = float, int NV = 1, typename G = WinoGeom>
+__global__ void __launch_bounds__(256)
+wino2d_output_adjoint_kernel(const TA* __restrict__ gy, TF* __restrict__ Z, G g, long total) {
   const long i = (long)blockIdx.x * 256 + threadIdx.x;
   if (i >= total) return;
-  int c, tw, th;
+  int c, h0, w0, dl;
   long tile, bd;
-  wino_decode2<NV>(i, g, c, tile, tw, th, bd);
+  wino_tile2<NV>(i, g, c, tile, h0, w0, dl, bd);
   float v[NV][16];
 #pragma unroll
   for (int e = 0; e < 2; ++e)
 #pragma unroll
     for (int f = 0; f < 2; ++f) {
+      const int h = h0 + e * dl, w = w0 + f * dl;
       float t[NV];
-      ldv<NV>(gy + ((bd * g.H + 2 * th + e) * g.W + 2 * tw + f) * g.C + c, t);
+#pragma unroll
+      for (int n = 0; n < NV; ++n) t[n] = 0.0f;
+      if (!G::kDil || (h < g.H && w < g.W)) ldv<NV>(gy + ((bd * g.H + h) * g.W + w) * g.C + c, t);
 #pragma unroll
       for (int n = 0; n < NV; ++n) v[n][e * 4 + f] = t[n];
     }
@@ -349,7 +385,31 @@
 }
 
 bool wino2d_ok(const ssbev_wino_dims* d) {
-  return d && d->B > 0 && d->C > 0 && d->D > 0 && d->H > 0 && d->W > 0 && d->H % 2 == 0 && d->W % 2 == 0;
+  return d && d->B > 0 && d->C > 0 && d->D > 0 && d->H > 0 && d->W > 0 && d->H % 2 == 0 && d->W % 2 == 0 && d->dil <= 1;
+}
+
+int wino2d_axis_table(int n, int dil, unsigned short* first, int cap) {
+  if (n <= 0 || dil <= 0) return 0;
+  int cnt = 0;
+  for (int ph = 0; ph < dil && ph < n; ++ph) {
+    const int nt = ((n - ph + dil - 1) / dil + 1) / 2;
+    for (int t = 0; t < nt; ++t, ++cnt)
+      if (first && cnt < cap) first[cnt] = (unsigned short)(ph + 2 * t * dil);
+  }
+  return cnt;
+}
+
+bool wino2d_dil_geom(const ssbev_wino_dims* d, WinoGeomDil& g, long& total) {
+  if (!d || d->B <= 0 || d->C <= 0 || d->D <= 0 || d->H <= 0 || d->W <= 0 || d->dil <= 1 || d->H > 65535 || d->W > 65535) return false;
+  g.B = d->B; g.D = d->D; g.H = d->H; g.W = d->W; g.C = d->C; g.acc = 0;
+  g.dil = d->dil;
+  g.TH = wino2d_axis_table(d->H, d->dil, g.h0, kWinoMaxAxisTiles);
+  g.TW = wino2d_axis_table(d->W, d->dil, g.w0, kWinoMaxAxisTiles);
+  if (g.TH > kWinoMaxAxisTiles || g.TW > kWinoMaxAxisTiles) return false;
+  for (int i = g.TH; i < kWinoMaxAxisTiles; ++i) g.h0[i] = 0;
+  for (int i = g.TW; i < kWinoMaxAxisTiles; ++i) g.w0[i] = 0;
+  total = (long)d->B * d->D * g.TH * g.TW * d->C;
+  return true;
 }
 
 __device__ __forceinline__ void g4(const float* g, int s, float* o, int so) {
@@ -690,7 +750,7 @@
 
 bool wino43_ok(const ssbev_wino_dims* d, int da) {
   return d && d->B > 0 && d->C > 0 && d->D > 0 && d->H > 0 && d->W > 0 && d->H % 4 == 0 && d->W % 4 == 0 &&
-         (da == 0 || d->D % da == 0);
+         (da == 0 || d->D % da == 0) && d->dil <= 1;
 }
 
 typedef float wf32x16 __attribute__((ext_vector_type(16)));
@@ -924,7 +984,7 @@
 }
 
 bool wino_ok(const ssbev_wino_dims* d) {
-  return d && d->B > 0 && d->C > 0 && d->D > 0 && d->H > 0 && d->W > 0 && d->D % 2 == 0 && d->H % 2 == 0 && d->W % 2 == 0;
+  return d && d->B > 0 && d->C > 0 && d->D > 0 && d->H > 0 && d->W > 0 && d->D % 2 == 0 && d->H % 2 == 0 && d->W % 2 == 0 && d->dil <= 1;
 }
 
 }
@@ -948,6 +1008,30 @@
     hipLaunchKernelGGL(KERNEL, dim3(cdiv((size_t)total, 256)), dim3(256), 0, as_stream(stream), src, dst, g, total); \
     return ssbev_launch_status();                                                                                  \
   }
+
+#define SSBEV_WINO2D_DIL_ENTRY(NAME, KERNEL, ACC)                                                                  \
+  int NAME(const float* src, float* dst, const ssbev_wino_dims* d, ssbev_stream_t stream) {                       \
+    if (!src || !dst || !d) return SSBEV_EINVAL;                                                                   \
+    if (d->dil > 1) {                                                                                              \
+      WinoGeomDil g;                                                                                               \
+      long total;                                                                                                  \
+      if (!wino2d_dil_geom(d, g, total)) return SSBEV_EINVAL;                                                      \
+      g.acc = ACC;                                                                                                 \
+      hipLaunchKernelGGL((KERNEL<float, float, 1, WinoGeomDil>), dim3(cdiv((size_t)total, 256)), dim3(256), 0,     \
+                         as_stream(stream), src, dst, g, total);                                                   \
+      return ssbev_launch_status();                                                                                \
+    }                                                                                                              \
+    if (!wino2d_ok(d)) return SSBEV_EINVAL;                                                                        \
+    const long total = (long)d->B * d->D * (d->H / 2) * (d->W / 2) * d->C;                                         \
+    WinoGeom g{d->B, d->D, d->H, d->W, d->C};                                                                      \
+    g.acc = ACC;                                                                                                   \
+    hipLaunchKernelGGL(KERNEL<float>, dim3(cdiv((size_t)total, 256)), dim3(256), 0, as_stream(stream), src, dst, g, total); \
+    return ssbev_launch_status();                                                                                  \
+  }
+
+int ssbev_wino2d_axis_tiles(int extent, int dil, uint16_t* first, int cap) {
+  return wino2d_axis_table(extent, dil, first, first ? cap : 0);
+}
 
 int ssbev_wino_weight_transform(const float* w, float* U, int Cout, int Cin, int ndim, int mode, ssbev_stream_t stream) {
   if (!w || !U || Cout <= 0 || Cin <= 0 || (ndim != 2 && ndim != 3) || (mode != 0 && mode != 1)) return SSBEV_EINVAL;
@@ -1018,9 +1102,9 @@
   return ssbev_launch_status();
 }
 
-SSBEV_WINO2D_ENTRY(ssbev_wino2d_input_transform, wino2d_input_kernel<float>, float, float)
-SSBEV_WINO2D_ENTRY(ssbev_wino2d_output_transform, wino2d_output_kernel<float>, float, float)
-SSBEV_WINO2D_ENTRY(ssbev_wino2d_output_adjoint, wino2d_output_adjoint_kernel<float>, float, float)
+SSBEV_WINO2D_DIL_ENTRY(ssbev_wino2d_input_transform, wino2d_input_kernel, 0)
+SSBEV_WINO2D_DIL_ENTRY(ssbev_wino2d_output_transform, wino2d_output_kernel, 0)
+SSBEV_WINO2D_DIL_ENTRY(ssbev_wino2d_output_adjoint, wino2d_output_adjoint_kernel, 0)
 
 SSBEV_WINO_ENTRY(ssbev_wino_input_transform, wino_input_kernel<float>, float, float)
 SSBEV_WINO_ENTRY(ssbev_wino_output_transform, wino_output_kernel<float>, float, float)
@@ -1062,14 +1146,7 @@
   return ssbev_launch_status();
 }
 
-int ssbev_wino2d_output_transform_acc(const float* src, float* dst, const ssbev_wino_dims* d, ssbev_stream_t stream) {
-  if (!wino2d_ok(d) || !src || !dst) return SSBEV_EINVAL;
-  const long total = (long)d->B * d->D * (d->H / 2) * (d->W / 2) * d->C;
-  WinoGeom g{d->B, d->D, d->H, d->W, d->C};
-  g.acc = 1;
-  hipLaunchKernelGGL(wino2d_output_kernel<float>, dim3(cdiv((size_t)total, 256)), dim3(256), 0, as_stream(stream), src, dst, g, total);
-  return ssbev_launch_status();
-}
+SSBEV_WINO2D_DIL_ENTRY(ssbev_wino2d_output_transform_acc, wino2d_output_kernel, 1)
 
 int ssbev_wino43_weight_transform(const float* w, float* U, int Cout, int Cin, int ndim, int mode, ssbev_stream_t stream) {
   if (!w || !U || Cout <= 0 || Cin <= 0 || (ndim != 2 && ndim != 3 && ndim != 4) || (mode != 0 && mode != 1)) return SSBEV_EINVAL;
diff --git a/stereoscene_amd/csrc/winograd_fused.hip b/stereoscene_amd/csrc/winograd_fused.hip
--- a/stereoscene_amd/csrc/winograd_fused.hip
+++ b/stereoscene_amd/csrc/winograd_fused.hip
@@ -424,7 +424,7 @@
 
 bool df_dims_ok(const ssbev_wino_dims* d, int N) {
   return d && d->B > 0 && d->C > 0 && d->D > 0 && d->H > 0 && d->W > 0 && d->H % 4 == 0 && d->W % 4 == 0 && d->D % 2 == 0 &&
-         d->C % DF_BK == 0 && N > 0 && N % 4 == 0;
+         d->C % DF_BK == 0 && N > 0 && N % 4 == 0 && d->dil <= 1;
 }
 
 int env_int(const char* name, int dflt) {
diff --git a/stereoscene_amd/functional.py b/stereoscene_amd/functional.py
--- a/stereoscene_amd/functional.py
+++ b/stereoscene_amd/functional.py
@@ -1022,6 +1022,22 @@
 POLYPHASE_MAX_PAD = float(os.environ.get("SSBEV_POLYPHASE_MAX_PAD", "1.35"))
 
 
+WINO_DILATED = os.environ.get("SSBEV_WINO_DILATED", "1") != "0"
+WINO_DILATED_MAX_TILES = float(os.environ.get("SSBEV_WINO_DILATED_MAX_TILES", str(POLYPHASE_MAX_PAD + 0.05)))
+WINO_DILATED_AXIS_CAP = 128
+
+
+def wino2d_axis_tiles(n, d):
+    return sum(-(-(-(-(n - ph) // d)) // 2) for ph in range(min(d, n)))
+
+
+def _wino_dilated_applicable(x, weight, d):
+    H, W = int(x.shape[-2]), int(x.shape[-1])
+    th, tw = wino2d_axis_tiles(H, d), wino2d_axis_tiles(W, d)
+    return (max(th, tw) <= WINO_DILATED_AXIS_CAP and weight.shape[1] % 4 == 0
+            and th * tw <= WINO_DILATED_MAX_TILES * (-(-H // 2)) * (-(-W // 2)))
+
+
 def _dilated_polyphase(x, weight, d):
     B, Cc, H, W = x.shape
     Hp, Wp = -(-H // (2 * d)) * 2 * d, -(-W // (2 * d)) * 2 * d
@@ -1054,6 +1070,11 @@
     if (GEMM_LAYERS and TILE_HINT == 0 and PRECISION == "fp32" and x.is_cuda and tuple(weight.shape[2:]) == (1, 1)
             and s == (1, 1) and p == (0, 0) and weight.shape[1] >= GEMM_MIN_CIN):
         return linear_cl(x, weight, bias)
+    if (WINO_DILATED and WINOGRAD and TILE_HINT == 0 and PRECISION == "fp32" and x.is_cuda and tuple(weight.shape[2:]) == (3, 3)
+            and s == (1, 1) and dl[0] == dl[1] and dl[0] > 1 and p == dl and min(weight.shape[0], weight.shape[1]) >= 64
+            and _wino_dilated_applicable(x, weight, dl[0])):
+        y = _WinoConv.apply(x.unsqueeze(2), weight.unsqueeze(2), _slot_of(x), dl[0]).squeeze(2)
+        return y if bias is None else y + bias.view(1, -1, 1, 1)
     if (DILATED_POLYPHASE and WINOGRAD and TILE_HINT == 0 and x.is_cuda and tuple(weight.shape[2:]) == (3, 3) and s == (1, 1)
             and dl[0] == dl[1] and dl[0] > 1 and p == dl and min(weight.shape[0], weight.shape[1]) >= 64):
         y = _dilated_polyphase(x, weight, dl[0])
@@ -1312,8 +1333,8 @@
 class _WinoConv(torch.autograd.Function):
 
     @staticmethod
-    def _plan(three_d, D, H, W, bf, cin=1 << 30):
-        f43 = WINO_F43 and (three_d or WINO_F43_2D or _F43_2D_SCOPE > 0) and not bf and H % 4 == 0 and W % 4 == 0 and \
+    def _plan(three_d, D, H, W, bf, cin=1 << 30, dil=1):
+        f43 = WINO_F43 and (three_d or WINO_F43_2D or _F43_2D_SCOPE > 0) and not bf and H % 4 == 0 and W % 4 == 0 and dil == 1 and \
             not (three_d and (WINO_DEPTH_FUSED or WINO_OWN_GEMM))
         if f43 and three_d and WINO_F444 and D % 4 == 0 and cin >= WINO_F444_MIN_CIN:
             return 4, "ssbev_wino444_", 216, 4, 8.0
@@ -1326,17 +1347,24 @@
         return (1 if f43 else 0), pre, nf, th, reduction
 
     @staticmethod
-    def forward(ctx, x, weight, slot=None):
+    def forward(ctx, x, weight, slot=None, dil=1):
         ctx.slot = slot
         if ctx.needs_input_grad[1]:
             streams.note_use(weight)
         bf = PRECISION != "fp32"
+        if dil > 1 and (bf or weight.shape[2] != 1):
+            raise capi.SsbevError("dilated Winograd: 2-D fp32 layers only")
         a16 = storage_bf16()
         xcl = to_cl(x if x.dtype == torch.bfloat16 else x.to(torch.bfloat16)) if a16 else to_cl(_f32(x, "wino_conv"))
         B, D, H, W, Cin = xcl.shape
         Cout, three_d = weight.shape[0], weight.shape[2] == 3
-        f43, pre, nf, th, red = _WinoConv._plan(three_d, D, H, W, bf, Cin)
+        f43, pre, nf, th, red = _WinoConv._plan(three_d, D, H, W, bf, Cin, dil)
         T = B * (D // (4 if f43 == 4 else 2) if three_d else D) * (H // th) * (W // th)
+        dtag = ""
+        if dil > 1:
+            T = B * D * wino2d_axis_tiles(H, dil) * wino2d_axis_tiles(W, dil)
+            red *= B * D * H * W / (4.0 * T)
+            dtag = f" d{dil}"
         lib = capi.load()
         w = weight.detach().contiguous()
         fl = 2.0 * B * D * H * W * Cin * Cout * (27 if three_d else 9)
@@ -1346,7 +1374,7 @@
         if not fused:
             U = torch.empty(nf, Cin, Cout, dtype=torch.float32, device=x.device)
             capi.check(wt(capi.ptr(w), capi.ptr(U), Cout, Cin, wdim, 0, capi.stream()), "ssbev_wino_weight_transform")
-        tag = f"wino{ {0: '', 1: '43', 4: '444'}[f43]} fwd {Cin}->{Cout} {D}x{H}x{W}"
+        tag = f"wino{ {0: '', 1: '43', 4: '444'}[f43]} fwd {Cin}->{Cout} {D}x{H}x{W}{dtag}"
         nby = 4.0 * (B * D * H * W * (Cin + Cout) + (27 if three_d else 9) * Cin * Cout)
         with _span("conv_winograd", fl, nby, tag, fl / red):
             if fused:
@@ -1354,22 +1382,23 @@
                 V = None
             elif bf:
                 sfx = "_bf16a" if a16 else "_bf16"
-                V = _wino_call(pre + "input_transform" + sfx, xcl, capi.WinoDims(B, D, H, W, Cin), (nf, T, Cin), torch.bfloat16)
+                V = _wino_call(pre + "input_transform" + sfx, xcl, capi.WinoDims(B, D, H, W, Cin, dil), (nf, T, Cin), torch.bfloat16)
                 M = _bmm16(V, U)
-                y = _wino_call(pre + "output_transform" + sfx, M, capi.WinoDims(B, D, H, W, Cout), (B, D, H, W, Cout),
+                y = _wino_call(pre + "output_transform" + sfx, M, capi.WinoDims(B, D, H, W, Cout, dil), (B, D, H, W, Cout),
                                torch.bfloat16 if a16 else torch.float32)
             else:
-                V = _wino_call(pre + "input_transform", xcl, capi.WinoDims(B, D, H, W, Cin), (nf, T, Cin))
+                V = _wino_call(pre + "input_transform", xcl, capi.WinoDims(B, D, H, W, Cin, dil), (nf, T, Cin))
                 M = _wino_bgemm(V, w, Cout, Cin, 0) if (three_d and WINO_OWN_GEMM and not f43) else (gemm_nn(V, U, tag=tag + " gemm") if own_gemm_site("wino") else torch.bmm(V, U))
-                y = _wino_call(pre + "output_transform", M, capi.WinoDims(B, D, H, W, Cout), (B, D, H, W, Cout))
+                y = _wino_call(pre + "output_transform", M, capi.WinoDims(B, D, H, W, Cout, dil), (B, D, H, W, Cout))
         ctx.save_for_backward(xcl if fused else V, weight)
-        ctx.geom = (B, D, H, W, Cin, Cout, T, three_d, fl, fused, bf, f43, pre, nf, red, a16)
+        ctx.geom = (B, D, H, W, Cin, Cout, T, three_d, fl, fused, bf, f43, pre, nf, red, a16, dil)
         return from_cl(y)
 
     @staticmethod
     def backward(ctx, gy):
         V, weight = ctx.saved_tensors
-        B, D, H, W, Cin, Cout, T, three_d, fl, fused, bf, f43, pre, nf, red, a16 = ctx.geom
+        B, D, H, W, Cin, Cout, T, three_d, fl, fused, bf, f43, pre, nf, red, a16, dil = ctx.geom
+        dtag = f" d{dil}" if dil > 1 else ""
         sfx, fdt = (("_bf16a" if a16 else "_bf16"), torch.bfloat16) if bf else ("", torch.float32)
         gcl = to_cl(gy)
         if a16 and gcl.dtype != torch.bfloat16:
@@ -1388,8 +1417,8 @@
             Ut = torch.empty(nf, Cout, Cin, dtype=torch.float32, device=gy.device)
             wt = lib.ssbev_wino43_weight_transform if f43 else lib.ssbev_wino_weight_transform
             capi.check(wt(capi.ptr(w), capi.ptr(Ut), Cout, Cin, nd, 1, capi.stream()), "ssbev_wino_weight_transform")
-            with _span("conv_winograd", fl, nby, f"wino{vtag} dgrad {Cin}->{Cout} {D}x{H}x{W}", fl / red):
-                Vg = _wino_call(pre + "input_transform" + sfx, gcl, capi.WinoDims(B, D, H, W, Cout), (nf, T, Cout), fdt)
+            with _span("conv_winograd", fl, nby, f"wino{vtag} dgrad {Cin}->{Cout} {D}x{H}x{W}{dtag}", fl / red):
+                Vg = _wino_call(pre + "input_transform" + sfx, gcl, capi.WinoDims(B, D, H, W, Cout, dil), (nf, T, Cout), fdt)
                 Mx = _wino_bgemm(Vg, w, Cout, Cin, 1) if (three_d and WINO_OWN_GEMM and not bf and not f43) \
                     else ((_bmm16(Vg, Ut) if fdt == torch.bfloat16 else torch.bmm(Vg, Ut.to(fdt))) if (bf or not own_gemm_site("wino")) else gemm_nn(Vg, Ut, tag="wino dgrad gemm"))
                 del Vg
@@ -1397,20 +1426,20 @@
                           "ssbev_wino43_2d_": "ssbev_wino43_2d_output_transform_acc"}.get(pre) if not bf else None
                 into = _slot_target(ctx.slot, torch.empty((B, D, H, W, Cin), device="meta")) if acc_fn else None
                 if into is not None:
-                    odims = capi.WinoDims(B, D, H, W, Cin)
+                    odims = capi.WinoDims(B, D, H, W, Cin, dil)
                     capi.check(getattr(lib, acc_fn)(capi.ptr(Mx), capi.ptr(into), C.byref(odims), capi.stream()), acc_fn)
                     gxcl = into
                 else:
-                    gxcl = _wino_call(pre + "output_transform" + sfx, Mx, capi.WinoDims(B, D, H, W, Cin), (B, D, H, W, Cin), adt)
+                    gxcl = _wino_call(pre + "output_transform" + sfx, Mx, capi.WinoDims(B, D, H, W, Cin, dil), (B, D, H, W, Cin), adt)
                 if ctx.slot is not None:
                     ctx.slot.buf = gxcl
             gx = from_cl(gxcl)
         if ctx.needs_input_grad[1]:
             def weight_gradient(V=V):
-                with _span("conv_winograd_wgrad", fl, nby, f"wino{vtag} wgrad {Cin}->{Cout} {D}x{H}x{W}", fl / red):
+                with _span("conv_winograd_wgrad", fl, nby, f"wino{vtag} wgrad {Cin}->{Cout} {D}x{H}x{W}{dtag}", fl / red):
                     if fused:
-                        V = _wino_call(pre + "input_transform", V, capi.WinoDims(B, D, H, W, Cin), (nf, T, Cin))
-                    Z = _wino_call(pre + "output_adjoint" + sfx, gcl, capi.WinoDims(B, D, H, W, Cout), (nf, T, Cout), fdt)
+                        V = _wino_call(pre + "input_transform", V, capi.WinoDims(B, D, H, W, Cin, dil), (nf, T, Cin))
+                    Z = _wino_call(pre + "output_adjoint" + sfx, gcl, capi.WinoDims(B, D, H, W, Cout, dil), (nf, T, Cout), fdt)
                     gU = _bmm16_tn(V, Z) if bf else (gemm_tn(V, Z, tag="wino wgrad gemm") if own_gemm_site("wino") else torch.bmm(V.transpose(1, 2), Z))
                 gwt = torch.empty_like(w)
                 wg = lib.ssbev_wino43_weight_grad if f43 else lib.ssbev_wino_weight_grad
@@ -1423,7 +1452,7 @@
                     side.publish(gw)
             else:
                 gw = weight_gradient()
-        return gx, gw, None
+        return gx, gw, None, None
 
 
 def conv_flops_3x3(B, D, H, W, Cin, Cout):
```

Measured after the change: 30.88 million voxels/s, median of 6. 1.9% higher.
